# uzh-rpg/dagr

Hardware: AMD Instinct MI355X
Metric: events_per_sec (higher is better)
Workload: dtype f32; 1 GPU; dagr-s + --use_image --img_net resnet50, 640x480 synthetic S-uniform, B=8 windows/step x 100000 events (50 ms each), r=7, K=16, events->graph->GNN(+image fusion)->decoded head outputs->confidence mask + NMS (device); image_branch=in-line, engines=3

## Files before the change

dagr_amd/_lib.py:

```python
import ctypes
import os

_HERE = os.path.dirname(os.path.abspath(__file__))
LIB_PATH = os.path.join(_HERE, "lib", "libdagr_hip.so")

c_void_p = ctypes.c_void_p
c_i32 = ctypes.c_int32
c_i64 = ctypes.c_int64
c_size_t = ctypes.c_size_t
c_float = ctypes.c_float


class PoolDesc(ctypes.Structure):
    _fields_ = [("batch_size", c_i32), ("channels", c_i32), ("gx", c_i32), ("gy", c_i32), ("vx", c_float),
                ("vy", c_float), ("inv_w", c_float), ("inv_h", c_float), ("two_max", c_float), ("r00", c_float),
                ("r02", c_float), ("r11", c_float), ("r12", c_float), ("rx", c_i32), ("ry", c_i32), ("aggr", c_i32),
                ("append_pos", c_i32), ("keep_order", c_i32)]


class GraphDesc(ctypes.Structure):
    _fields_ = [("width", c_i32), ("height", c_i32), ("batch_size", c_i32), ("max_neighbors", c_i32),
                ("queue_size", c_i32), ("radius", c_i32), ("delta_t_us", c_i32), ("time_window", c_i32),
                ("max_events", c_i64)]


class HeadScale(ctypes.Structure):
    _fields_ = [("n_ptr", c_void_p), ("n_max", c_i32), ("pred", c_void_p), ("ld", c_i32), ("pos", c_void_p),
                ("batch", c_void_p), ("vx", c_float), ("vy", c_float), ("stride", c_float), ("Hc", c_i32), ("Wc", c_i32),
                ("cnn", c_void_p * 3), ("cnn_stride", (c_i32 * 4) * 3), ("dense", c_void_p)]


class ConvJob(ctypes.Structure):
    _fields_ = [("n_nodes_ptr", c_void_p), ("n_nodes_max", c_i32), ("rowptr", c_void_p), ("col", c_void_p),
                ("code", c_void_p), ("x", c_void_p), ("ldx", c_i32), ("cin", c_i32), ("xskip", c_void_p),
                ("ldskip", c_i32), ("cskip", c_i32), ("rx", c_i32), ("ry", c_i32), ("den_x", c_float), ("den_y", c_float),
                ("Wq", c_void_p), ("bias", c_void_p), ("C", c_void_p), ("ldc", c_i32), ("N", c_i32), ("relu", c_i32)]


class L0Inputs(ctypes.Structure):
    _fields_ = [("feat", c_void_p), ("pos_nodes", c_void_p), ("batch_nodes", c_void_p), ("x0", c_void_p), ("ldx0", c_i32),
                ("col_feat", c_i32), ("col_pos", c_i32)]


class AsyncUpdateArgs(ctypes.Structure):
    _fields_ = [("gdesc", ctypes.POINTER(GraphDesc)), ("graph_ws", c_void_p), ("n_static", c_i64), ("first_id", c_i64),
                ("app_head", c_void_p), ("app_next", c_void_p), ("app_xytb", c_void_p), ("capacity", c_i64),
                ("pos", c_void_p), ("batch", c_void_p), ("batch_is_int64", c_i32), ("n_new", c_i64),
                ("nbr_src", c_void_p), ("nbr_code", c_void_p), ("deg", c_void_p), ("status", c_void_p),
                ("feat", c_void_p), ("pos_nodes", c_void_p), ("batch_nodes", c_void_p), ("batch_events", c_void_p),
                ("x0", c_void_p), ("ldx0", c_i32), ("col_feat", c_i32), ("col_pos", c_i32),
                ("win_x", c_i32), ("tx", c_i32), ("win_y", c_i32), ("ty", c_i32), ("rx", c_i32), ("ry", c_i32),
                ("den_x", c_float), ("den_y", c_float),
                ("cin1", c_i32), ("w1", c_void_p), ("s1", c_void_p), ("h1", c_void_p), ("ldh1", c_i32),
                ("w2", c_void_p), ("s2", c_void_p), ("hp0", c_void_p), ("ldhp0", c_i32),
                ("pdesc", ctypes.POINTER(PoolDesc)), ("pool_ws", c_void_p), ("xlo", c_void_p), ("ylo", c_void_p),
                ("x_out", c_void_p), ("ldo", c_i32), ("pos_out", c_void_p), ("batch_out", c_void_p), ("n_out", c_void_p),
                ("rowptr_out", c_void_p), ("col_out", c_void_p), ("code_out", c_void_p), ("e_out", c_void_p),
                ("e_cap", c_i32)]


SIGNATURES = {
    "dagr_last_error": (ctypes.c_char_p, []),
    "dagr_version": (ctypes.c_int, []),
    "dagr_device_count": (ctypes.c_int, []),
    "dagr_format_events": (ctypes.c_int, [c_void_p, c_void_p, c_void_p, c_i64, c_i32, c_i32, c_i32,
                                          c_void_p, c_void_p, c_void_p]),
    "dagr_fill_edges": (ctypes.c_int, [c_void_p, c_void_p, c_void_p, c_void_p, c_void_p, c_i32, c_float, c_float, c_void_p,
                                       c_i64, c_i32, c_i64, c_i32, c_i32, c_i32, c_i32, c_void_p]),
    "dagr_insert_in_queue": (ctypes.c_int, [c_void_p, c_void_p, c_void_p, c_i64, c_void_p, c_i32, c_i32, c_i32, c_i32,
                                            c_void_p]),
    "dagr_insert_in_queue_single": (ctypes.c_int, [c_void_p, c_void_p, c_void_p, c_i32, c_i32, c_i32, c_i32, c_void_p]),
    "dagr_graph_workspace_bytes": (c_size_t, [ctypes.POINTER(GraphDesc)]),
    "dagr_graph_workspace_init": (ctypes.c_int, [ctypes.POINTER(GraphDesc), c_void_p, c_size_t, c_void_p]),
    "dagr_graph_build_window": (ctypes.c_int, [ctypes.POINTER(GraphDesc), c_void_p, c_void_p, c_i32, c_void_p,
                                               c_i32, c_i64, c_void_p, c_void_p, c_void_p, c_void_p]),
    "dagr_graph_search_window": (ctypes.c_int, [ctypes.POINTER(GraphDesc), c_void_p, c_i64, c_void_p, c_void_p, c_void_p,
                                                c_void_p]),
    "dagr_graph_status": (ctypes.c_int, [ctypes.POINTER(GraphDesc), c_void_p, ctypes.POINTER(c_i64),
                                         ctypes.POINTER(c_i32), c_void_p]),
    "dagr_graph_counters": (ctypes.c_int, [ctypes.POINTER(GraphDesc), c_void_p, c_void_p, c_void_p]),
    "dagr_scan_scratch_elems": (c_size_t, [c_i64]),
    "dagr_graph_edge_index": (ctypes.c_int, [ctypes.POINTER(GraphDesc), c_void_p, c_void_p, c_void_p, c_i64, c_void_p,
                                             c_void_p, c_void_p, c_i64, c_void_p]),
    "dagr_graph_node_order": (ctypes.c_int, [ctypes.POINTER(GraphDesc), c_void_p, c_i64, c_void_p, c_void_p, c_void_p]),
    "dagr_graph_gather_inputs": (ctypes.c_int, [ctypes.POINTER(GraphDesc), c_void_p, c_void_p, c_void_p, c_i64,
                                                c_void_p, c_void_p, c_void_p, c_i32, c_i32, c_i32, c_void_p]),
    "dagr_spline_conv_l0_tiles": (ctypes.c_int, [c_i32, c_i32, c_i32, c_i32, c_i32, c_i32, c_i32, c_i32, c_i32, c_float,
                                                 c_float, c_i64, c_i32, c_void_p, c_void_p, c_void_p, c_void_p, c_i32,
                                                 c_void_p, c_i32, c_void_p, c_void_p, c_i32, c_void_p, c_i32, c_void_p,
                                                 c_void_p]),
    "dagr_graph_build_window_dev": (ctypes.c_int, [ctypes.POINTER(GraphDesc), c_void_p, c_void_p, c_i32, c_void_p,
                                                   c_i32, c_i64, c_void_p, c_void_p, c_void_p, c_void_p, c_void_p]),
    "dagr_graph_build_window_inputs": (ctypes.c_int, [ctypes.POINTER(GraphDesc), c_void_p, c_void_p, c_void_p, c_i32, c_i64,
                                                      c_void_p, c_void_p, c_void_p, c_void_p, c_void_p, c_void_p]),
    "dagr_graph_node_count_ptr": (c_void_p, [ctypes.POINTER(GraphDesc), c_void_p]),
    "dagr_graph_csr_codes": (ctypes.c_int, [ctypes.POINTER(GraphDesc), c_void_p, c_void_p, c_void_p, c_void_p, c_i64, c_i32,
                                            c_void_p, c_void_p, c_void_p, c_void_p, c_i64, c_void_p]),
    "dagr_stage_window": (ctypes.c_int, [ctypes.POINTER(GraphDesc), c_void_p, c_void_p, c_void_p, c_void_p, c_i32, c_i64,
                                         c_void_p, c_void_p, c_void_p, c_void_p, c_void_p]),
    "dagr_spiral_offsets": (ctypes.c_int, [c_i32, c_void_p, c_void_p]),
    "dagr_spline_tap_window": (ctypes.c_int, [c_i32, c_float, ctypes.POINTER(c_i32), ctypes.POINTER(c_i32)]),
    "dagr_spline_l0_table": (ctypes.c_int, [c_i32, c_i32, c_float, c_float, c_i32, c_i32, c_i32, c_i32, c_void_p,
                                            c_void_p, c_void_p]),
    "dagr_spline_conv_l0": (ctypes.c_int, [c_i32, c_i32, c_i32, c_i64, c_i32, c_i32, c_void_p, c_void_p, c_void_p,
                                           c_void_p, c_i32, c_void_p, c_i32, c_void_p, c_void_p, c_void_p, c_i32,
                                           c_void_p, c_i32, c_void_p]),
    "dagr_spline_tap_aggregate": (ctypes.c_int, [c_void_p, c_i32, c_void_p, c_void_p, c_void_p, c_void_p, c_i32,
                                                 c_i32, c_void_p, c_i32, c_i32, c_i32, c_i32, c_float, c_float,
                                                 c_void_p, c_i32, c_void_p]),
    "dagr_spline_tap_scatter_grad": (ctypes.c_int, [c_void_p, c_i32, c_void_p, c_void_p, c_void_p, c_void_p, c_i32, c_i32,
                                                    c_i32, c_i32, c_float, c_float, c_void_p, c_void_p, c_void_p, c_i32,
                                                    c_void_p]),
    "dagr_spline_tap_scatter_grad_w": (ctypes.c_int, [c_void_p, c_i32, c_void_p, c_void_p, c_void_p, c_void_p, c_i32, c_i32,
                                                      c_void_p, c_i32, c_i32, c_i32, c_i32, c_float, c_float, c_void_p,
                                                      c_void_p, c_void_p, c_i32, c_void_p]),
    "dagr_pool_workspace_bytes": (c_size_t, [ctypes.POINTER(PoolDesc)]),
    "dagr_pool_workspace_init": (ctypes.c_int, [ctypes.POINTER(PoolDesc), c_void_p, c_size_t, c_void_p]),
    "dagr_pool_l0": (ctypes.c_int, [ctypes.POINTER(PoolDesc), c_void_p, ctypes.POINTER(GraphDesc), c_void_p,
                                    c_void_p, c_void_p, c_void_p, c_i32, c_void_p, c_void_p, c_void_p, c_i32, c_i64,
                                    c_void_p, c_void_p,
                                    c_void_p, c_void_p, c_void_p, c_i32, c_i32, c_void_p, c_void_p, c_void_p,
                                    c_void_p, c_void_p, c_void_p, c_void_p, c_i32, c_void_p]),
    "dagr_pool_l0_accumulate": (ctypes.c_int, [ctypes.POINTER(PoolDesc), c_void_p, ctypes.POINTER(GraphDesc), c_void_p,
                                               c_void_p, c_void_p, c_void_p, c_i32, c_void_p, c_i64, c_void_p, c_void_p,
                                               c_void_p, c_void_p]),
    "dagr_pool_csr": (ctypes.c_int, [ctypes.POINTER(PoolDesc), c_void_p, c_void_p, c_i32, c_void_p, c_i32, c_void_p,
                                     c_void_p, c_void_p, c_void_p, c_void_p, c_void_p, c_i32, c_i32, c_void_p,
                                     c_void_p, c_void_p, c_void_p, c_void_p, c_void_p, c_void_p, c_i32, c_void_p]),
    "dagr_pool_recode": (ctypes.c_int, [c_void_p, c_i32, c_void_p, c_void_p, c_void_p, c_float, c_float, c_float, c_float,
                                        c_float, c_i32, c_i32, c_void_p, c_i32, c_void_p, c_void_p]),
    "dagr_pool_status": (ctypes.c_int, [ctypes.POINTER(PoolDesc), c_void_p, ctypes.POINTER(c_i32), c_void_p]),
    "dagr_pool_status_ptr": (c_void_p, [ctypes.POINTER(PoolDesc), c_void_p]),
    "dagr_pool_counters": (ctypes.c_int, [ctypes.POINTER(PoolDesc), c_void_p, c_void_p, c_void_p]),
    "dagr_to_dense": (ctypes.c_int, [c_void_p, c_i32, c_void_p, c_i32, c_i32, c_void_p, c_void_p, c_float, c_float,
                                     c_i32, c_i32, c_i32, c_void_p, c_void_p, c_void_p, c_void_p]),
    "dagr_pool_argmax": (ctypes.c_int, [c_void_p, c_i32, c_void_p, c_i32, c_i32, c_void_p, c_i32, c_i32, c_void_p, c_void_p]),
    "dagr_pool_grad": (ctypes.c_int, [c_void_p, c_i32, c_i32, c_i32, c_void_p, c_void_p, c_void_p, c_i32, c_void_p, c_i32,
                                      c_void_p]),
    "dagr_to_dense_grad": (ctypes.c_int, [c_i32, c_i32, c_void_p, c_void_p, c_float, c_float, c_i32, c_i32, c_i32, c_void_p,
                                          c_void_p, c_i32, c_void_p]),
    "dagr_sample_features": (ctypes.c_int, [c_void_p, c_i32, c_void_p, c_void_p, c_i32, c_void_p, c_i32, c_i32, c_i32,
                                            c_i32, c_i32, c_i32, c_void_p, c_i32, c_i32, c_void_p]),
    "dagr_nms_batched": (ctypes.c_int, [c_void_p, c_void_p, c_void_p, c_void_p, c_i32, c_i32, c_float, c_float, c_void_p,
                                        c_void_p, c_void_p, c_void_p]),
    "dagr_heads_finish": (ctypes.c_int, [ctypes.POINTER(HeadScale), ctypes.POINTER(HeadScale), c_i32, c_i32, c_void_p,
                                         c_void_p, c_void_p]),
    "dagr_heads_finish_detect": (ctypes.c_int, [ctypes.POINTER(HeadScale), ctypes.POINTER(HeadScale), c_i32, c_i32, c_void_p,
                                                c_void_p, c_float, c_float, c_float, c_void_p, c_void_p, c_void_p]),
    "dagr_decode_heads": (ctypes.c_int, [c_void_p, c_i32, c_i32, c_float, c_void_p, c_i32, c_i32, c_float, c_i32, c_i32,
                                         c_void_p, c_void_p]),
    "dagr_postprocess": (ctypes.c_int, [c_void_p, c_i32, c_i32, c_i32, c_float, c_float, c_float, c_void_p, c_void_p,
                                        c_void_p]),
    "dagr_masked_lin": (ctypes.c_int, [c_void_p, c_void_p, c_void_p, c_void_p, c_void_p, c_i32, c_i64, c_i32, c_i32, c_void_p]),
    "dagr_masked_lin_no_bias": (ctypes.c_int, [c_void_p, c_void_p, c_void_p, c_void_p, c_i32, c_i64, c_i32, c_i32, c_void_p]),
    "dagr_masked_isdiff": (ctypes.c_int, [c_void_p, c_void_p, c_void_p, c_float, c_float, c_i64, c_i32, c_void_p]),
    "dagr_masked_inplace_BN": (ctypes.c_int, [c_void_p, c_void_p, c_void_p, c_void_p, c_void_p, c_void_p, c_void_p, c_float,
                                              c_i64, c_i32, c_void_p]),
    "dagr_downsample_events": (ctypes.c_int, [c_void_p, c_void_p, c_void_p, c_i32, c_void_p, c_i32, c_i32, c_void_p,
                                              c_void_p, c_void_p]),
    "dagr_spline_conv_l0_tiles_rows": (ctypes.c_int, [c_i32, c_i32, c_i32, c_i32, c_i32, c_i32, c_i32, c_i32, c_i32, c_float,
                                                      c_float, c_i64, c_i64, c_i32, c_void_p, c_void_p, c_void_p, c_void_p,
                                                      c_i32, c_void_p, c_i32, c_void_p, c_void_p, c_i32, c_void_p, c_i32,
                                                      c_void_p, c_void_p]),
    "dagr_async_graph_append": (ctypes.c_int, [ctypes.POINTER(GraphDesc), c_void_p, c_i64, c_i64, c_void_p, c_void_p,
                                               c_void_p, c_i64, c_void_p, c_i32, c_void_p, c_i32, c_i64, c_void_p, c_void_p,
                                               c_void_p, c_void_p, c_void_p, c_void_p, c_void_p, c_void_p, c_void_p, c_i32,
                                               c_i32, c_i32, c_void_p]),
    "dagr_async_update": (ctypes.c_int, [ctypes.POINTER(AsyncUpdateArgs), c_void_p]),
    "dagr_pool_l0_stream": (ctypes.c_int, [ctypes.POINTER(PoolDesc), c_void_p, c_i32, ctypes.POINTER(GraphDesc), c_void_p,
                                           c_void_p, c_void_p, c_void_p, c_i32, c_void_p, c_void_p, c_i64, c_i64, c_i64,
                                           c_void_p, c_void_p, c_void_p, c_void_p, c_i32, c_i32, c_void_p, c_void_p,
                                           c_void_p, c_void_p, c_void_p, c_void_p, c_void_p, c_i32, c_void_p]),
    "dagr_spline_conv_fused_lds_bytes": (c_size_t, [c_i32, c_i32]),
    "dagr_spline_conv_fused_passes": (c_i32, [c_i32, c_i32]),
    "dagr_spline_conv_fused": (ctypes.c_int, [c_void_p, c_i32, c_void_p, c_void_p, c_void_p, c_void_p, c_i32, c_i32,
                                              c_void_p, c_i32, c_i32, c_i32, c_i32, c_float, c_float, c_void_p,
                                              c_void_p, c_void_p, c_i32, c_i32, c_i32, c_void_p]),
    "dagr_spline_conv_fused_pool": (ctypes.c_int, [c_void_p, c_i32, c_void_p, c_void_p, c_void_p, c_void_p, c_i32, c_i32,
                                                   c_void_p, c_i32, c_i32, c_i32, c_i32, c_float, c_float, c_void_p,
                                                   c_void_p, c_void_p, c_i32, c_i32, c_i32, ctypes.POINTER(PoolDesc),
                                                   c_void_p, c_void_p, c_void_p, c_void_p, c_void_p]),
    "dagr_spline_conv_fused_multi": (ctypes.c_int, [c_void_p, c_i32, c_void_p]),
    "dagr_spline_conv_fused_pair": (ctypes.c_int, [c_void_p, c_i32, c_void_p, c_void_p, c_void_p, c_i32, c_i32, c_i32, c_i32,
                                                   c_float, c_float, c_i32, c_i32, c_void_p, c_void_p, c_void_p, c_void_p,
                                                   c_i32, c_void_p, c_void_p, c_void_p, c_void_p, c_i32, c_void_p]),
    "dagr_gemm_epilogue_workspace_bytes": (c_size_t, []),
    "dagr_gemm_epilogue": (ctypes.c_int, [c_void_p, c_i64, c_i32, c_i64, c_void_p, c_i32, c_void_p, c_void_p, c_i64, c_i32,
                                          c_void_p, c_i64, c_void_p, c_size_t, c_void_p]),
    "dagr_add_relu": (ctypes.c_int, [c_void_p, c_void_p, c_i64, c_void_p]),
    "dagr_bias_relu": (ctypes.c_int, [c_void_p, c_void_p, c_i64, c_i32, c_void_p]),
    "dagr_bias_silu": (ctypes.c_int, [c_void_p, c_void_p, c_i64, c_i32, c_void_p]),
    "dagr_bn_relu_maxpool": (ctypes.c_int, [c_void_p, c_i32, c_i32, c_i32, c_i32, c_void_p, c_void_p, c_void_p, c_void_p]),
    "dagr_gemm_bias_act": (ctypes.c_int, [c_void_p, c_i32, c_void_p, c_i32, c_void_p, c_i32, c_void_p, c_void_p,
                                          c_i32, c_i32, c_i32, c_i32, c_void_p]),
    "dagr_async_flops": (ctypes.c_int, [c_void_p, c_i32, c_void_p, c_void_p, c_void_p, c_void_p, c_void_p, c_i32, c_void_p,
                                        c_void_p]),
    "dagr_viz_workspace_bytes": (c_size_t, [c_i32, c_i32, c_i32]),
    "dagr_viz_render": (ctypes.c_int, [c_void_p, c_i32, c_i32, c_i32, c_void_p, c_i32, c_void_p, c_void_p, c_void_p,
                                       c_void_p, c_i32, c_void_p, c_void_p, c_void_p, c_i32, c_i32, c_void_p, c_i32,
                                       c_void_p, c_void_p, c_void_p, c_size_t, c_void_p]),
    "dagr_augment_workspace_bytes": (c_size_t, [c_i64]),
    "dagr_augment_events": (ctypes.c_int, [c_void_p, c_i32, c_i32, c_i32, c_void_p, c_i32, c_void_p, c_i32, c_void_p, c_i32,
                                           c_void_p, c_i64, c_void_p, c_void_p, c_void_p, c_void_p, c_void_p, c_void_p,
                                           c_void_p, c_size_t, c_void_p]),
    "dagr_augment_status": (ctypes.c_int, [c_void_p, c_void_p]),
    "dagr_augment_frames": (ctypes.c_int, [c_void_p, c_i32, c_i32, c_i32, c_i32, c_i32, c_i32, c_void_p, c_void_p,
                                           c_void_p]),
    "dagr_augment_boxes": (ctypes.c_int, [c_void_p, c_i32, c_i32, c_i32, c_void_p, c_void_p, c_i32, c_i32, c_void_p,
                                          c_void_p]),
}

_lib = None


def lib():
    global _lib
    if _lib is None:
        if not os.path.exists(LIB_PATH):
            raise RuntimeError(
                f"dagr_amd: {LIB_PATH} not found -- build it with `make` (or __graft_entry__.build()). "
                "There is no CPU fallback for the event-graph hot path.")
        handle = ctypes.CDLL(LIB_PATH)
        for name, (res, args) in SIGNATURES.items():
            fn = getattr(handle, name)
            fn.restype = res
            fn.argtypes = args
        _lib = handle
    return _lib


def check(rc, what=""):
    if rc != 0:
        msg = lib().dagr_last_error().decode("utf-8", "replace")
        raise RuntimeError(f"libdagr_hip {what} failed (status {rc}): {msg}")


def ptr(t):
    return None if t is None else c_void_p(t.data_ptr())


def cur_stream(device=None):
    import torch
    return c_void_p(torch.cuda.current_stream(device).cuda_stream)
```

dagr_amd/csrc/pooling.hip:

```cpp
#include <climits>

#include "common.hpp"
#include "pool_common.hpp"

namespace dagr {
namespace {

constexpr int kMaxL0Channels = 512;

__device__ __forceinline__ float div_floor(float a, float b) {
    if (b == 0.0f) return a / b;
    const float mod = fmodf(a, b);
    float div = (a - mod) / b;
    if ((mod != 0.0f) && ((b < 0.0f) != (mod < 0.0f))) div -= 1.0f;
    float floordiv;
    if (div != 0.0f) {
        floordiv = floorf(div);
        if (div - floordiv > 0.5f) floordiv += 1.0f;
    } else {
        floordiv = copysignf(0.0f, a / b);
    }
    return floordiv;
}

__global__ __launch_bounds__(kBlock) void k_pool_accumulate(dagr_pool_desc d, const int32_t *__restrict__ n_ptr,
                                                           int n_max, const float *__restrict__ x, int ldx,
                                                           const float *__restrict__ pos,
                                                           const int32_t *__restrict__ batch,
                                                           const int32_t *__restrict__ rowptr,
                                                           const int32_t *__restrict__ col, PoolWs ws,
                                                           int32_t *__restrict__ cluster_raw_out) {
    const int n_nodes = n_ptr ? min(*n_ptr, n_max) : n_max;
    const int C = d.channels;
    const int64_t gid = (int64_t)blockIdx.x * kBlock + threadIdx.x;
    const int n = (int)(gid / C), ch = (int)(gid % C);
    if (n >= n_nodes) return;
    bool ok;
    const int raw = cluster_raw(pos[3 * n], pos[3 * n + 1], pos[3 * n + 2], batch[n], d, ok);
    if (!ok) {
        if (ch == 0) { atomicOr(&ws.status[0], 1); cluster_raw_out[n] = -1; }
        return;
    }
    const float v = x[(size_t)n * ldx + ch];
    if (d.aggr == 0)
        atomicMax(reinterpret_cast<int *>(ws.xacc + (size_t)raw * C + ch), enc_f(v));
    else
        atomicAdd(reinterpret_cast<unsigned long long *>(ws.xacc + (size_t)raw * C + ch),
                  (unsigned long long)(long long)llrint((double)v * kFeatScale));
    pool_merge_node(d, ws, n, raw, pos, batch, col, rowptr ? rowptr[n] : 0, rowptr ? rowptr[n + 1] : 0, ch, C, cluster_raw_out);
}

constexpr int kPoolL0Block = 1024;

template <int AGGR>
__host__ __device__ inline size_t pool_l0_lds_bytes(int VW, int C, int W, int H, bool ord = false) {
    size_t b = ((size_t)VW * C * (AGGR == 0 ? 4 : 8) + 7) / 8 * 8;
    b += (size_t)VW * (24 + 4 + 4 + 4);
    b += (kPoolL0Block / 64) * 64 * 2;
    b += ((size_t)(W + H) * 2 + 7) / 8 * 8;
    if (ord) b += (size_t)VW * 4;
    return b + 64;
}

template <int AGGR, int VEC, bool ORD>
__device__ __forceinline__ void pool_l0_slots_body(dagr_pool_desc d, int W, int H, int n_cap, int VW,
                                                               const int32_t *__restrict__ n_ptr,
                                                               const int32_t *__restrict__ xlo,
                                                               const int32_t *__restrict__ ylo,
                                                               const int32_t *__restrict__ start, int row_keys,
                                                               const int2 *__restrict__ slot_it,
                                                               const int32_t *__restrict__ slot_xyb,
                                                               const float *__restrict__ x, int ldx,
                                                               const float *__restrict__ pos, PoolWs ws,
                                                               const int16_t *__restrict__ nbr_code,
                                                               const int32_t *__restrict__ nbr_src,
                                                               const int32_t *__restrict__ deg, int K, int r) {
    extern __shared__ __align__(16) unsigned char lds_raw[];
    constexpr int NW = kPoolL0Block / 64;
    const int n = min(*n_ptr, n_cap);
    const int per_block = max(64 * NW, (int)(((long long)n + gridDim.x - 1) / gridDim.x + 63) / 64 * 64);
    const int s_begin = blockIdx.x * per_block;
    if (s_begin >= n) return;
    const int s_end = min(n, s_begin + per_block);
    const int C = d.channels;
    const int lane = threadIdx.x & 63, wv = threadIdx.x >> 6;
    int *l_acc; unsigned long long *l_ps; int *l_cnt, *l_perm; unsigned *l_nbm; short *l_sv; unsigned short *l_xlut, *l_ylut;
    int *l_tmax = nullptr;
    {
        unsigned char *p = lds_raw;
        l_acc = reinterpret_cast<int *>(p); p += ((size_t)VW * C * (AGGR == 0 ? 4 : 8) + 7) / 8 * 8;
        l_ps = reinterpret_cast<unsigned long long *>(p); p += (size_t)VW * 24;
        l_cnt = reinterpret_cast<int *>(p); p += (size_t)VW * 4;
        l_perm = reinterpret_cast<int *>(p); p += (size_t)VW * 4;
        l_nbm = reinterpret_cast<unsigned *>(p); p += (size_t)VW * 4;
        l_sv = reinterpret_cast<short *>(p); p += NW * 64 * 2;
        l_xlut = reinterpret_cast<unsigned short *>(p); p += (size_t)W * 2;
        l_ylut = reinterpret_cast<unsigned short *>(p);
        if (ORD) l_tmax = reinterpret_cast<int *>(l_xlut + ((size_t)(W + H) * 2 + 7) / 8 * 4);
    }
    auto arm_window = [&]() {
        for (int i = threadIdx.x; i < VW * C; i += kPoolL0Block) {
            if (AGGR == 0) l_acc[i] = kEncMin;
            else reinterpret_cast<unsigned long long *>(l_acc)[i] = 0ull;
        }
        for (int i = threadIdx.x; i < VW; i += kPoolL0Block) {
            l_cnt[i] = 0; l_perm[i] = -1; l_nbm[i] = 0u;
            if (ORD) l_tmax[i] = kEncMin;
            l_ps[3 * i] = 0ull; l_ps[3 * i + 1] = 0ull; l_ps[3 * i + 2] = 0ull;
        }
    };
    arm_window();
    for (int c = threadIdx.x; c < d.gx; c += kPoolL0Block)
        for (int px = xlo[c]; px < min(xlo[c + 1], W); px++) l_xlut[px] = (unsigned short)c;
    for (int c = threadIdx.x; c < d.gy; c += kPoolL0Block)
        for (int py = ylo[c]; py < min(ylo[c + 1], H); py++) l_ylut[py] = (unsigned short)c;
    __syncthreads();
    const int cells = d.gx * d.gy;
    const int pair = ws_pair(ws);
    long long *w_possum = ws_possum(ws, pair);
    int32_t *w_cnt = ws_cnt(ws, pair);
    const int side = 2 * r + 1;
    const int side_magic = (65536 + side - 1) / side;
    const int PPN = C / VEC;
    const unsigned ppn_magic = PPN > 1 ? (unsigned)((0x100000000ull + (unsigned)PPN - 1) / (unsigned)PPN) : 0u;
    constexpr int kBig = 1 << 28;
    int n_slow = 0;
    const int T = ws.T;
    const int WB = VW / d.gx;
    for (int seg_begin = s_begin; seg_begin < s_end;) {
    int raw0, seg_end = s_end;
    {
        const int c0 = slot_xyb[seg_begin];
        const int q0 = (int)l_ylut[(c0 >> 12) & 4095] + d.gy * ((c0 >> 24) & 127);
        raw0 = d.gx * q0;
        const int qe = q0 + WB;
        if (qe < d.gy * d.batch_size) {
            const int be = qe / d.gy, cye = qe - be * d.gy;
            seg_end = min(s_end, max(seg_begin + 1, start[row_keys * (min(ylo[cye], H) + H * be)]));
        }
    }
    for (int cs = seg_begin + 64 * wv; cs < seg_end; cs += 64 * NW) {
        const int s = cs + lane;
        const bool live = s < seg_end;
        int c = 0, id = 0, dg = 0;
        float px = 0.f, py = 0.f, pt = 0.f;
        int4 lo4 = make_int4(0, 0, 0, 0), hi4 = lo4;
        if (live) {
            c = slot_xyb[s];
            px = pos[3 * (size_t)s]; py = pos[3 * (size_t)s + 1]; pt = pos[3 * (size_t)s + 2];
            id = slot_it[s].x;
            if (nbr_code) {
                dg = min(deg[s], K);
                if (K == 16) {
                    lo4 = *reinterpret_cast<const int4 *>(nbr_code + (size_t)s * 16);
                    hi4 = *reinterpret_cast<const int4 *>(nbr_code + (size_t)s * 16 + 8);
                }
            }
        }
        const float *xrow = x + (size_t)cs * ldx;
        const int n_live = min(64, seg_end - cs);
        constexpr int U = 4;
        float val[U][VEC];
        int who[U];
        auto request = [&](int f0) {
#pragma unroll
            for (int u = 0; u < U; u++) {
                const int f = f0 + 64 * u + lane;
                who[u] = -1;
                if (f < n_live * PPN) {
                    const int k = PPN > 1 ? (int)__umulhi((unsigned)f, ppn_magic) : f, p = f - k * PPN;
                    who[u] = (k << 16) | p;
                    if constexpr (VEC == 4) {
                        const float4 qv = *reinterpret_cast<const float4 *>(xrow + (size_t)k * ldx + 4 * p);
                        val[u][0] = qv.x; val[u][1] = qv.y; val[u][2] = qv.z; val[u][3] = qv.w;
                    } else {
                        val[u][0] = xrow[(size_t)k * ldx + p];
                    }
                }
            }
        };
        request(0);
        int vloc = -1;
        if (live) {
            const int xp = c & 4095, yp = (c >> 12) & 4095, b = (c >> 24) & 127;
            const int cx = l_xlut[xp], cy = l_ylut[yp];
            const bool leak = pt >= 1.0f;
            const int raw = cx + d.gx * (cy + d.gy * b);
            const int rel = raw - raw0;
            const bool inwin = !leak && rel >= 0 && rel < VW;
            const unsigned long long q0 = (unsigned long long)(long long)llrint((double)px * kPosScale);
            const unsigned long long q1 = (unsigned long long)(long long)llrint((double)py * kPosScale);
            const unsigned long long q2 = (unsigned long long)(long long)llrint((double)pt * kPosScale);
            if (ORD) {
                if (inwin) atomicMax(&l_tmax[rel], enc_f(pt));
                else atomicMax(&ws.tmax[leak ? raw + cells : raw], enc_f(pt));
            }
            unsigned nbm = 0, nbm_up = 0, nbm_low = 0;
            if (nbr_code) {
                int tx[4], ty[4];
#pragma unroll
                for (int k = 0; k < 4; k++) {
                    const int qx = cx - 1 + k, qy = cy - 1 + k;
                    tx[k] = (qx <= 0 ? -kBig : (qx >= d.gx ? kBig : xlo[qx])) - xp + r;
                    ty[k] = (qy <= 0 ? -kBig : (qy >= d.gy ? kBig : ylo[qy])) - yp + r;
                }
                int codes[16];
                if (K == 16) {
                    const int w8[8] = {lo4.x, lo4.y, lo4.z, lo4.w, hi4.x, hi4.y, hi4.z, hi4.w};
#pragma unroll
                    for (int j = 0; j < 8; j++) { codes[2 * j] = (short)(w8[j] & 0xffff); codes[2 * j + 1] = w8[j] >> 16; }
                } else {
#pragma unroll
                    for (int j = 0; j < 16; j++) codes[j] = j < dg ? (int)nbr_code[(size_t)s * K + j] : 0;
                }
#pragma unroll
                for (int j = 0; j < 16; j++) {
                    if (j < dg) {
                        const int code = codes[j];
                        const int ox = (code * side_magic) >> 16, oy = code - ox * side;
                        const int dcx = (ox >= tx[0]) + (ox >= tx[1]) + (ox >= tx[2]) + (ox >= tx[3]);
                        const int dcy = (oy >= ty[0]) + (oy >= ty[1]) + (oy >= ty[2]) + (oy >= ty[3]);
                        const unsigned bit = 1u << (dcy * 5 + dcx);
                        if (!leak) {
                            nbm |= bit;
                        } else {
                            const int src = nbr_src[(size_t)s * K + j];
                            if (pos[3 * (size_t)src + 2] >= 1.0f) nbm_up |= bit;
                            else nbm_low |= bit;
                        }
                    }
                }
                nbm &= ~(1u << 12);
                nbm_up &= ~(1u << 12);
            }
            if (inwin) {
                vloc = rel;
                atomicAdd(&l_cnt[rel], 1);
                atomicMax(&l_perm[rel], id);
                atomicAdd(&l_ps[3 * rel], q0);
                atomicAdd(&l_ps[3 * rel + 1], q1);
                atomicAdd(&l_ps[3 * rel + 2], q2);
                if (nbm) atomicOr(&l_nbm[rel], nbm);
            } else {
                const int rl = leak ? raw + cells : raw;
                n_slow++;
                for (int ch = 0; ch < C; ch++) {
                    const float v = x[(size_t)s * ldx + ch];
                    if (AGGR == 0)
                        atomicMax(reinterpret_cast<int *>(ws.xacc + (size_t)rl * C + ch), enc_f(v));
                    else
                        atomicAdd(reinterpret_cast<unsigned long long *>(ws.xacc + (size_t)rl * C + ch),
                                  (unsigned long long)(long long)llrint((double)v * kFeatScale));
                }
                ws.occupied[rl] = 1;
                atomicAdd(&w_cnt[rl], 1);
                atomicMax(&ws.perm[rl], id);
                atomicAdd(reinterpret_cast<unsigned long long *>(w_possum + (size_t)rl * 3 + 0), q0);
                atomicAdd(reinterpret_cast<unsigned long long *>(w_possum + (size_t)rl * 3 + 1), q1);
                atomicAdd(reinterpret_cast<unsigned long long *>(w_possum + (size_t)rl * 3 + 2), q2);
                if (!leak) {
                    if (nbm) atomicOr(&ws.nbmask[rl], (unsigned long long)nbm);
                } else if (nbm_up | nbm_low) {
                    atomicOr(&ws.nbmask[rl], ((unsigned long long)nbm_low << 32) | nbm_up);
                }
            }
        }
        l_sv[wv * 64 + lane] = (short)vloc;
        __builtin_amdgcn_wave_barrier();
        for (int f0 = 0; f0 < n_live * PPN; f0 += 64 * U) {
            float cur[U][VEC];
            int tgt[U];
#pragma unroll
            for (int u = 0; u < U; u++) {
                tgt[u] = -1;
                if (who[u] >= 0) {
                    const int v = l_sv[wv * 64 + (who[u] >> 16)];
                    if (v >= 0) tgt[u] = v * C + (who[u] & 0xffff) * VEC;
                }
#pragma unroll
                for (int j = 0; j < VEC; j++) cur[u][j] = val[u][j];
            }
            if (f0 + 64 * U < n_live * PPN) request(f0 + 64 * U);
#pragma unroll
            for (int u = 0; u < U; u++) {
                if (tgt[u] >= 0) {
#pragma unroll
                    for (int j = 0; j < VEC; j++) {
                        if (AGGR == 0)
                            atomicMax(&l_acc[tgt[u] + j], enc_f(cur[u][j]));
                        else
                            atomicAdd(reinterpret_cast<unsigned long long *>(l_acc) + tgt[u] + j,
                                      (unsigned long long)(long long)llrint((double)cur[u][j] * kFeatScale));
                    }
                }
            }
        }
        __builtin_amdgcn_wave_barrier();
    }
    __syncthreads();
    for (int i = threadIdx.x; i < VW * C; i += kPoolL0Block) {
        const int v = i / C;
        if (l_cnt[v] > 0 && raw0 + v < T) {
            const size_t o = (size_t)(raw0 + v) * C + (i - v * C);
            if (AGGR == 0) atomicMax(reinterpret_cast<int *>(ws.xacc + o), l_acc[i]);
            else atomicAdd(reinterpret_cast<unsigned long long *>(ws.xacc + o),
                           reinterpret_cast<unsigned long long *>(l_acc)[i]);
        }
    }
    for (int v = threadIdx.x; v < VW; v += kPoolL0Block) {
        const int cn = l_cnt[v];
        if (cn > 0 && raw0 + v < T) {
            const int raw = raw0 + v;
            ws.occupied[raw] = 1;
            atomicAdd(&w_cnt[raw], cn);
            atomicMax(&ws.perm[raw], l_perm[v]);
            atomicAdd(reinterpret_cast<unsigned long long *>(w_possum + (size_t)raw * 3 + 0), l_ps[3 * v]);
            atomicAdd(reinterpret_cast<unsigned long long *>(w_possum + (size_t)raw * 3 + 1), l_ps[3 * v + 1]);
            atomicAdd(reinterpret_cast<unsigned long long *>(w_possum + (size_t)raw * 3 + 2), l_ps[3 * v + 2]);
            if (l_nbm[v]) atomicOr(&ws.nbmask[raw], (unsigned long long)l_nbm[v]);
            if (ORD) atomicMax(&ws.tmax[raw], l_tmax[v]);
        }
    }
    seg_begin = seg_end;
    if (seg_begin < s_end) {
        __syncthreads();
        arm_window();
        __syncthreads();
    }
    }
    {
        int tot = n_slow;
#pragma unroll
        for (int off = 1; off < 64; off <<= 1) tot += __shfl_xor(tot, off, 64);
        if (lane == 0 && tot) atomicAdd(&ws.status[5], tot);
    }
}

#define DAGR_POOL_L0_SLOTS_KERNEL(NAME, ORD)                                                                          \
    template <int AGGR, int VEC>                                                                                       \
    __global__ __launch_bounds__(kPoolL0Block) void NAME(                                                              \
        dagr_pool_desc d, int W, int H, int n_cap, int VW, const int32_t *__restrict__ n_ptr,                          \
        const int32_t *__restrict__ xlo, const int32_t *__restrict__ ylo, const int32_t *__restrict__ start, int row_keys, \
        const int2 *__restrict__ slot_it, const int32_t *__restrict__ slot_xyb, const float *__restrict__ x, int ldx,   \
        const float *__restrict__ pos, PoolWs ws, const int16_t *__restrict__ nbr_code,                                \
        const int32_t *__restrict__ nbr_src, const int32_t *__restrict__ deg, int K, int r) {                          \
        pool_l0_slots_body<AGGR, VEC, ORD>(d, W, H, n_cap, VW, n_ptr, xlo, ylo, start, row_keys, slot_it, slot_xyb, x, \
                                           ldx, pos, ws, nbr_code, nbr_src, deg, K, r);                                \
    }
DAGR_POOL_L0_SLOTS_KERNEL(k_pool_l0_slots, false)
DAGR_POOL_L0_SLOTS_KERNEL(k_pool_l0_slots_ord, true)
#undef DAGR_POOL_L0_SLOTS_KERNEL

__global__ __launch_bounds__(kBlock) void k_pool_l0_event_cluster(dagr_pool_desc d, int N,
                                                                 const float *__restrict__ pos,
                                                                 const int32_t *__restrict__ batch32,
                                                                 const int64_t *__restrict__ batch64,
                                                                 int32_t *__restrict__ cluster_raw_out,
                                                                 int32_t *__restrict__ status) {
    const int n = blockIdx.x * kBlock + threadIdx.x;
    if (n >= N) return;
    bool ok;
    const int b = batch32 ? batch32[n] : (int)batch64[n];
    const int raw = cluster_raw(pos[3 * (size_t)n], pos[3 * (size_t)n + 1], pos[3 * (size_t)n + 2], b, d, ok);
    if (!ok) atomicOr(status, 1);
    cluster_raw_out[n] = ok ? raw : -1;
}

__device__ __forceinline__ void cluster_pos(const PoolWs &ws, int pair, int raw, int cnt, const dagr_pool_desc &d,
                                            float (&p)[3]) {
    const long long *ps = ws_possum(ws, pair) + (size_t)raw * 3;
#pragma unroll
    for (int k = 0; k < 3; k++) p[k] = (float)(((double)ps[k] / kPosScale) / (double)cnt);
    p[0] = div_floor(p[0] + 1e-5f, d.inv_w) * d.inv_w;
    p[1] = div_floor(p[1] + 1e-5f, d.inv_h) * d.inv_h;
}

__global__ __launch_bounds__(kBlock) void k_pool_finalize(dagr_pool_desc d, PoolWs ws,
                                                         const int32_t *__restrict__ batch32,
                                                         const int64_t *__restrict__ batch64,
                                                         float *__restrict__ x_out, int ldo, int xoff,
                                                         float *__restrict__ pos_out, int32_t *__restrict__ batch_out,
                                                         int32_t *__restrict__ n_out) {
    const int T = d.gx * d.gy * (d.batch_size + 1);
    const int C = d.channels;
    const int64_t gid = (int64_t)blockIdx.x * kBlock + threadIdx.x;
    const int raw = (int)(gid / C), ch = (int)(gid % C);
    if (raw >= T) return;
    if (gid == 0) *n_out = ws.newid[T];
    const int pair = ws_pair(ws);
    const int cnt = ws_cnt(ws, pair)[raw];
    long long *acc = ws.xacc + (size_t)raw * C + ch;
    if (cnt > 0) {
        const int c = ws.newid[raw];
        float v;
        if (d.aggr == 0) v = dec_f((int)(*acc));
        else v = (float)(((double)(*acc) / kFeatScale) / (double)cnt);
        x_out[(size_t)c * ldo + xoff + ch] = v;
        if (ch == 0) {
            float p[3];
            cluster_pos(ws, pair, raw, cnt, d, p);
            pos_out[3 * c] = p[0]; pos_out[3 * c + 1] = p[1]; pos_out[3 * c + 2] = p[2];
            const int pm = ws.perm[raw];
            batch_out[c] = batch32 ? batch32[pm] : (int)batch64[pm];
            if (d.append_pos) {
                x_out[(size_t)c * ldo + xoff + C] = p[0];
                x_out[(size_t)c * ldo + xoff + C + 1] = p[1];
            }
        }
    }
    *acc = 0ll;
    if (d.aggr == 0) *reinterpret_cast<int *>(acc) = kEncMin;
    if (ch == 0) {
        long long *ps = ws_possum(ws, pair) + (size_t)raw * 3;
        ps[0] = 0; ps[1] = 0; ps[2] = 0;
    }
}

__global__ void k_fill_enc_min(long long *p, size_t n) {
    const size_t i = (size_t)blockIdx.x * blockDim.x + threadIdx.x;
    if (i < n) { p[i] = 0ll; *reinterpret_cast<int *>(p + i) = kEncMin; }
}

__global__ __launch_bounds__(kBlock) void k_pool_rearm(int T, PoolWs ws) {
    const int raw = blockIdx.x * kBlock + threadIdx.x;
    if (raw >= T) return;
    ws_cnt(ws, ws_pair(ws))[raw] = 0;
    ws.perm[raw] = -1;
    ws.nbmask[raw] = 0ull;
    if (ws.tmax) ws.tmax[raw] = kEncMin;
}

__global__ __launch_bounds__(kBlock) void k_coarse_edges_ell(int N, int K, const int32_t *__restrict__ nbr_src,
                                                            const int32_t *__restrict__ deg,
                                                            const int32_t *__restrict__ cluster_raw_in,
                                                            const int32_t *__restrict__ newid, int32_t *rows,
                                                            int32_t *status, const int32_t *__restrict__ tmax) {
    __shared__ unsigned long long seen[256];
    seen[threadIdx.x] = ~0ull;
    __syncthreads();
    const int lane = threadIdx.x & 63;
    const int per_iter = kBlock / K;
    const int G = gridDim.x, nx = (G % 8 == 0) ? 8 : 1;
    const int xcd = blockIdx.x % nx, lb = blockIdx.x / nx, bpx = G / nx;
    const int chunk = (N + nx - 1) / nx;
    const int per_block = (chunk + bpx - 1) / bpx;
    const int n_begin = xcd * chunk + lb * per_block;
    const int n_end = min(min(N, (xcd + 1) * chunk), n_begin + per_block);
    const int sub = threadIdx.x / K, j = threadIdx.x % K;
    for (int n0 = n_begin; n0 < n_end; n0 += per_iter) {
        const int n = n0 + sub;
        int rd = -1, rs = -1;
        if (sub < per_iter && n < n_end && j < deg[n]) {
            rd = cluster_raw_in[n];
            rs = cluster_raw_in[nbr_src[(size_t)n * K + j]];
        }
        bool has = (rd != rs) && rd >= 0 && rs >= 0;
        if (tmax && has && !(tmax[rs] < tmax[rd])) has = false;
        const unsigned long long key = ((unsigned long long)(unsigned)rd << 32) | (unsigned)rs;
        const unsigned h = (unsigned)((key * 0x9E3779B97F4A7C15ull) >> 56);
        if (has && seen[h] == key) has = false;
        unsigned long long pending = __ballot(has);
        while (pending) {
            const int leader = __ffsll((long long)pending) - 1;
            const int prd = __shfl(rd, leader, 64), prs = __shfl(rs, leader, 64);
            if (lane == leader) {
                row_insert(rows, newid[prd], newid[prs], status);
                seen[h] = key;
            }
            const bool same = has && rd == prd && rs == prs;
            pending &= ~__ballot(same);
            if (same) has = false;
        }
    }
}

__global__ __launch_bounds__(kBlock) void k_rows_sort(int T, const int32_t *__restrict__ newid, int32_t *rows,
                                                     int32_t *__restrict__ rowcnt) {
    const int lane = threadIdx.x & 63;
    const int c = blockIdx.x * (kBlock / 64) + (threadIdx.x >> 6);
    if (c > T) return;
    const int nc = newid[T];
    if (c >= nc) {
        if (lane == 0 && c <= T) rowcnt[c] = 0;
        return;
    }
    int32_t *row = rows + (size_t)c * kRowSlots;
    const int v = row[lane];
    const bool valid = v >= 0;
    int rank = 0;
    for (int k = 0; k < 64; k++) {
        const int o = __shfl(v, k, 64);
        rank += (o >= 0 && o < v) ? 1 : 0;
    }
    const int count = __popcll(__ballot(valid));
    row[lane] = -1;
    __builtin_amdgcn_wave_barrier();
    if (valid) row[rank] = v;
    if (lane == 0) rowcnt[c] = count;
}

__global__ __launch_bounds__(kBlock) void k_rows_emit(dagr_pool_desc d, int T, const int32_t *__restrict__ newid,
                                                     int32_t *rows, const int32_t *__restrict__ rowptr,
                                                     const float *__restrict__ pos_out, int32_t *__restrict__ col,
                                                     int32_t *__restrict__ code, int32_t *__restrict__ e_out,
// ... 222 lines not shown
        for (int k = 0; k < 64; k++) {
            const int o = __shfl(v, k, 64);
            rank += (o >= 0 && o < v) ? 1 : 0;
        }
    }
    if (v < 0) return;
    const int o = rowptr_out[c] + rank;
    if (o >= e_cap) { atomicOr(ws.status, 4); return; }
    float q[3];
    cluster_pos(ws, pair, v, ws_cnt(ws, pair)[v], d, q);
    const float ax = (q[0] - p[0]) / d.two_max + 0.5f;
    const float ay = (q[1] - p[1]) / d.two_max + 0.5f;
    const int ix = (int)((ax * d.r00 + d.r02) + 1e-3f);
    const int iy = (int)((ay * d.r11 + d.r12) + 1e-3f);
    if (ix < 0 || ix > 2 * d.rx || iy < 0 || iy > 2 * d.ry) atomicOr(ws.status, 8);
    col[o] = ws.newid[v];
    code[o] = (ix & 0xffff) | (iy << 16);
}

template <bool KEEP>
__global__ __launch_bounds__(kBlock) void k_pool_order_masks(dagr_pool_desc d, PoolWs ws) {
    const int raw = blockIdx.x * kBlock + threadIdx.x;
    if (raw >= ws.T) return;
    const unsigned long long m = ws.nbmask[raw];
    unsigned long long f = 0ull;
    if (m) {
        if (!KEEP) ws.nbmask[raw] = 0ull;
        const int td = ws.tmax[raw];
        const int cells = d.gx * d.gy;
        for (unsigned long long r = m; r; r &= r - 1ull) {
            const int bit = __ffsll((long long)r) - 1;
            const int k = bit & 31;
            const int v = raw + (k % 5 - 2) + d.gx * (k / 5 - 2) - (bit >= 32 ? cells : 0);
            if (v >= 0 && v < ws.T && ws.tmax[v] < td) f |= 1ull << bit;
        }
    }
    ws.nbmask_f[raw] = f;
}

__global__ __launch_bounds__(kBlock) void k_pool_order_rows(PoolWs ws) {
    const int lane = threadIdx.x & 63;
    const int raw = blockIdx.x * (kBlock / 64) + (threadIdx.x >> 6);
    if (raw >= ws.T || ws.rowcnt[raw] == 0) return;
    int32_t *row = ws.rows + (size_t)raw * kRowSlots;
    const int v = row[lane];
    bool keep = v >= 0;
    if (keep && !(ws.tmax[v] < ws.tmax[raw])) {
        row[lane] = -1;
        keep = false;
    }
    const int n = __popcll(__ballot(keep));
    if (lane == 0) ws.rowcnt[raw] = n;
}

__global__ __launch_bounds__(kBlock) void k_pool_l0_add_rows(dagr_pool_desc d, int W, int H, int first_row, int n_rows,
                                                            const int32_t *__restrict__ xlo,
                                                            const int32_t *__restrict__ ylo,
                                                            const float *__restrict__ x, int ldx,
                                                            const float *__restrict__ pos,
                                                            const int32_t *__restrict__ batch_events, PoolWs ws,
                                                            const int16_t *__restrict__ nbr_code,
                                                            const int32_t *__restrict__ nbr_src,
                                                            const int32_t *__restrict__ deg, int K, int r) {
    const int l = threadIdx.x & 15;
    const int i = (blockIdx.x * kBlock + threadIdx.x) >> 4;
    if (i >= n_rows) return;
    const int s = first_row + i;
    const float px = pos[3 * (size_t)s], py = pos[3 * (size_t)s + 1], pt = pos[3 * (size_t)s + 2];
    const int b = batch_events[s];
    bool ok;
    const int raw = cluster_raw(px, py, pt, b, d, ok);
    if (!ok) {
        if (l == 0) atomicOr(&ws.status[0], 1);
        return;
    }
    const bool leak = pt >= 1.0f;
    const int cells = d.gx * d.gy;
    const int C = d.channels;
    const int pair = ws_pair(ws);
    for (int ch = l; ch < C; ch += 16) {
        const float v = x[(size_t)s * ldx + ch];
        if (d.aggr == 0) atomicMax(reinterpret_cast<int *>(ws.xacc + (size_t)raw * C + ch), enc_f(v));
        else atomicAdd(reinterpret_cast<unsigned long long *>(ws.xacc + (size_t)raw * C + ch),
                       (unsigned long long)(long long)llrint((double)v * kFeatScale));
    }
    if (l == 0) {
        ws.occupied[raw] = 1;
        atomicAdd(&ws_cnt(ws, pair)[raw], 1);
        atomicMax(&ws.perm[raw], ((b + 1) << 26) | s);
        if (ws.tmax) atomicMax(&ws.tmax[raw], enc_f(pt));
        atomicAdd(reinterpret_cast<unsigned long long *>(ws_possum(ws, pair) + (size_t)raw * 3 + 0),
                  (unsigned long long)(long long)llrint((double)px * kPosScale));
        atomicAdd(reinterpret_cast<unsigned long long *>(ws_possum(ws, pair) + (size_t)raw * 3 + 1),
                  (unsigned long long)(long long)llrint((double)py * kPosScale));
        atomicAdd(reinterpret_cast<unsigned long long *>(ws_possum(ws, pair) + (size_t)raw * 3 + 2),
                  (unsigned long long)(long long)llrint((double)pt * kPosScale));
    }
    if (nbr_code && l < deg[s]) {
        const int xpix = (int)((float)W * px + 1e-3f), ypix = (int)((float)H * py + 1e-3f);
        const int cx = (raw % cells) % d.gx, cy = (raw % cells) / d.gx;
        const int side = 2 * r + 1;
        const int code = nbr_code[(size_t)s * K + l];
        const int ox = code / side, oy = code - ox * side;
        const int xs = xpix + ox - r, ys = ypix + oy - r;
        int dcx = 0, dcy = 0;
#pragma unroll
        for (int q = 0; q < 4; q++) {
            const int qx = cx - 1 + q, qy = cy - 1 + q;
            const int bxq = qx <= 0 ? INT_MIN : (qx >= d.gx ? INT_MAX : xlo[qx]);
            const int byq = qy <= 0 ? INT_MIN : (qy >= d.gy ? INT_MAX : ylo[qy]);
            dcx += xs >= bxq;
            dcy += ys >= byq;
        }
        const int bit = dcy * 5 + dcx;
        if (!leak) {
            if (bit != 12) atomicOr(&ws.nbmask[raw], 1ull << bit);
        } else {
            const int src = nbr_src[(size_t)s * K + l];
            if (pos[3 * (size_t)src + 2] >= 1.0f) {
                if (bit != 12) atomicOr(&ws.nbmask[raw], 1ull << bit);
            } else {
                atomicOr(&ws.nbmask[raw], 1ull << (32 + bit));
            }
        }
    }
}

__global__ __launch_bounds__(kBlock) void k_pool_perm_keys(int T, const int32_t *__restrict__ batch_events, PoolWs ws) {
    const int raw = blockIdx.x * kBlock + threadIdx.x;
    if (raw >= T) return;
    const int pm = ws.perm[raw];
    if (pm >= 0) ws.perm[raw] = ((batch_events[pm] + 1) << 26) | pm;
}

}
}

using namespace dagr;

namespace {
int validate_pool(const dagr_pool_desc *d) {
    DAGR_CHECK_ARG(d != nullptr, "desc is NULL");
    DAGR_CHECK_ARG(d->gx > 0 && d->gy > 0 && d->batch_size > 0 && d->channels > 0, "bad sizes");
    DAGR_CHECK_ARG((int64_t)d->gx * d->gy * (d->batch_size + 1) < (1 << 22), "voxel table too large");
    DAGR_CHECK_ARG(d->keep_order == 0 || d->keep_order == 1, "keep_order must be 0 or 1");
    DAGR_CHECK_ARG(d->aggr == 0 || d->aggr == 1, "aggr must be 0 (max) or 1 (mean)");
    DAGR_CHECK_ARG(d->vx > 0 && d->vy > 0 && d->two_max > 0, "bad voxel size / cartesian max");
    return DAGR_OK;
}

int launch_pool_l0_slots(const dagr_pool_desc *desc, const dagr_graph_desc *gdesc, void *graph_ws, const int32_t *xlo,
                         const int32_t *ylo, const float *x, int ldx, const float *pos, const PoolWs &ws,
                         const int16_t *nbr_code, const int32_t *nbr_src, const int32_t *deg, int64_t n_cap,
                         hipStream_t stream) {
    PixelIndex ix;
    graph_ws_index(gdesc, graph_ws, &ix);
    const int32_t *start = ix.start; const int2 *slot_it = ix.slot_it;
    const int32_t *slot_xyb = ix.slot_xyb;
    const int32_t *n_ptr = ix.n_nodes;
    const int row_keys = ix.W;
    const int C = desc->channels, W = gdesc->width, H = gdesc->height, K = gdesc->max_neighbors;
    const bool vec4 = C % 4 == 0 && ldx % 4 == 0 && ((uintptr_t)x & 15) == 0;
    const bool ord = desc->keep_order != 0;
    const size_t per_slot = (size_t)C * (desc->aggr == 0 ? 4 : 8) + 36 + (ord ? 4 : 0);
    const size_t budget = (size_t)60 * 1024 - (size_t)(W + H) * 2 - 2048 - 1024;
    int VW = (int)std::min<size_t>(1024, budget / per_slot);
    VW = std::max(VW, desc->gx) / 2 * 2 + 2;
    const size_t lds = desc->aggr == 0 ? pool_l0_lds_bytes<0>(VW, C, W, H, ord) : pool_l0_lds_bytes<1>(VW, C, W, H, ord);
    DAGR_CHECK_ARG(lds <= 64 * 1024, "level-0 pooling: one voxel row of accumulators does not fit the LDS window");
    DAGR_CHECK_ARG(desc->gx < 65536 && desc->gy < 65536 && VW < 32768, "voxel grid too large for the level-0 pooling kernel");
    const int gmult = C > 32 ? 2 : 1;
    const unsigned grid = (unsigned)std::max<int64_t>(1, std::min<int64_t>((int64_t)gmult * device_cu_count(),
                                                                          ceil_div(n_cap, kPoolL0Block)));
#define DAGR_POOL_L0_LAUNCH(AG, VEC)                                                                                  \
    if (ord) DAGR_POOL_L0_LAUNCH_ORD(k_pool_l0_slots_ord, AG, VEC); else DAGR_POOL_L0_LAUNCH_ORD(k_pool_l0_slots, AG, VEC)
#define DAGR_POOL_L0_LAUNCH_ORD(KERNEL, AG, VEC)                                                                      \
    KERNEL<AG, VEC><<<grid, kPoolL0Block, lds, stream>>>(*desc, W, H, (int)n_cap, VW, n_ptr, xlo, ylo, start, row_keys, slot_it, \
                                                                   slot_xyb, x, ldx, pos, ws, nbr_code, nbr_src, deg, K, \
                                                                   gdesc->radius)
    if (desc->aggr == 0) { if (vec4) DAGR_POOL_L0_LAUNCH(0, 4); else DAGR_POOL_L0_LAUNCH(0, 1); }
    else                 { if (vec4) DAGR_POOL_L0_LAUNCH(1, 4); else DAGR_POOL_L0_LAUNCH(1, 1); }
#undef DAGR_POOL_L0_LAUNCH
#undef DAGR_POOL_L0_LAUNCH_ORD
    DAGR_CHECK_LAUNCH();
    return DAGR_OK;
}
template <bool KEEP>
int pool_order_masks(const dagr_pool_desc *d, const PoolWs &ws, PoolWs *view, hipStream_t stream) {
    *view = ws;
    if (!d->keep_order) return DAGR_OK;
    k_pool_order_masks<KEEP><<<(unsigned)ceil_div(ws.T, kBlock), kBlock, 0, stream>>>(*d, ws);
    DAGR_CHECK_LAUNCH();
    view->nbmask = ws.nbmask_f;
    return DAGR_OK;
}
}

extern "C" {

size_t dagr_pool_workspace_bytes(const dagr_pool_desc *desc) {
    if (validate_pool(desc) != DAGR_OK) return 0;
    return pool_carve(*desc, nullptr, nullptr);
}

int dagr_pool_workspace_init(const dagr_pool_desc *desc, void *workspace, size_t bytes, void *stream_) {
    int rc = validate_pool(desc);
    if (rc != DAGR_OK) return rc;
    DAGR_CHECK_ARG(workspace, "workspace is NULL");
    PoolWs ws;
    if (pool_carve(*desc, (char *)workspace, &ws) > bytes) {
        set_error("dagr_pool_workspace_init: workspace too small");
        return DAGR_ERR_WORKSPACE;
    }
    hipStream_t stream = (hipStream_t)stream_;
    const int64_t T = (int64_t)desc->gx * desc->gy * (desc->batch_size + 1);
    DAGR_CHECK_HIP(hipMemsetAsync(ws.occupied, 0, (T + 32) * 4, stream));
    DAGR_CHECK_HIP(hipMemsetAsync(ws.newid, 0, (T + 32) * 4, stream));
    DAGR_CHECK_HIP(hipMemsetAsync(ws.possum, 0, 2 * T * 3 * 8, stream));
    DAGR_CHECK_HIP(hipMemsetAsync(ws.cnt, 0, 2 * T * 4, stream));
    DAGR_CHECK_HIP(hipMemsetAsync(ws.perm, 0xff, T * 4, stream));
    DAGR_CHECK_HIP(hipMemsetAsync(ws.rows, 0xff, T * (size_t)kRowSlots * 4, stream));
    DAGR_CHECK_HIP(hipMemsetAsync(ws.rowcnt, 0, (T + 32) * 4, stream));
    DAGR_CHECK_HIP(hipMemsetAsync(ws.status, 0, 32, stream));
    DAGR_CHECK_HIP(hipMemsetAsync(ws.tile_state, 0, ((T + 1 + kPoolScanTile - 1) / kPoolScanTile + 8) * 8, stream));
    DAGR_CHECK_HIP(hipMemsetAsync(ws.nbmask, 0, (T + 9) * 8, stream));
    if (desc->keep_order) {
        DAGR_CHECK_HIP(hipMemsetD32Async((hipDeviceptr_t)ws.tmax, kEncMin, (size_t)T + 32, stream));
        DAGR_CHECK_HIP(hipMemsetAsync(ws.nbmask_f, 0, (T + 9) * 8, stream));
    }
    {
        const size_t n = T * (size_t)desc->channels;
        if (desc->aggr == 0) {
            k_fill_enc_min<<<(unsigned)ceil_div(n, 256), 256, 0, stream>>>(ws.xacc, n);
            DAGR_CHECK_LAUNCH();
        } else {
            DAGR_CHECK_HIP(hipMemsetAsync(ws.xacc, 0, n * 8, stream));
        }
    }
    return DAGR_OK;
}


#define DAGR_POOL_SCAN(MASKS, KEEP, WS)                                                                               \
    k_pool_scan_chained<MASKS, KEEP><<<(unsigned)ceil_div(T + 1, kPoolScanTile), kBlock, 0, stream>>>(WS, n_out, rowptr_out, e_out)


static int pool_tail(const dagr_pool_desc *d, PoolWs &ws, const int32_t *batch32, const int64_t *batch64,
                     float *x_out, int ldo, int xoff, float *pos_out, int32_t *batch_out, int32_t *n_out,
                     int32_t *rowptr_out, int32_t *col_out, int32_t *code_out, int32_t *e_out, int e_cap,
                     hipStream_t stream) {
    const int T = d->gx * d->gy * (d->batch_size + 1);
    const int wpb = kBlock / 64;
    k_rows_sort<<<(unsigned)ceil_div(T + 1, wpb), kBlock, 0, stream>>>(T, ws.newid, ws.rows, ws.rowcnt);
    DAGR_CHECK_LAUNCH();
    DAGR_CHECK_HIP(exclusive_scan_i32(ws.rowcnt, rowptr_out, T + 1, ws.scan_tmp, false, stream));
    k_rows_emit<<<(unsigned)ceil_div(T, wpb), kBlock, 0, stream>>>(*d, T, ws.newid, ws.rows, rowptr_out, pos_out,
                                                                  col_out, code_out, e_out, e_cap, ws.status);
    DAGR_CHECK_LAUNCH();
    k_pool_rearm<<<(unsigned)ceil_div(T, kBlock), kBlock, 0, stream>>>(T, ws);
    DAGR_CHECK_LAUNCH();
    (void)batch32; (void)batch64; (void)x_out; (void)ldo; (void)xoff; (void)batch_out; (void)n_out;
    return DAGR_OK;
}

int dagr_pool_l0(const dagr_pool_desc *desc, void *pool_ws, const dagr_graph_desc *gdesc, void *graph_ws,
                 const int32_t *xlo, const int32_t *ylo, const float *x, int32_t ldx, const float *pos,
                 const int32_t *batch_nodes, const void *batch, int32_t batch_is_int64, int64_t N,
                 const int32_t *nbr_src, const int16_t *nbr_code, const int32_t *deg,
                 int32_t *cluster_scratch, float *x_out, int32_t ldo, int32_t xoff, float *pos_out,
                 int32_t *batch_out, int32_t *n_out, int32_t *rowptr_out, int32_t *col_out, int32_t *code_out,
                 int32_t *e_out, int32_t e_cap, void *stream_) {
    int rc = validate_pool(desc);
    if (rc != DAGR_OK) return rc;
    DAGR_CHECK_ARG(pool_ws && gdesc && graph_ws, "NULL workspace/desc");
    DAGR_CHECK_ARG(desc->channels <= kMaxL0Channels, "too many channels for the level-0 pooling kernel");
    DAGR_CHECK_ARG(desc->batch_size == gdesc->batch_size, "batch_size mismatch");
    DAGR_CHECK_ARG(n_out && rowptr_out && e_out, "NULL output");
    hipStream_t stream = (hipStream_t)stream_;
    PoolWs ws;
    pool_carve(*desc, (char *)pool_ws, &ws);
    const int T = desc->gx * desc->gy * (desc->batch_size + 1);
    const int32_t *b32 = batch_is_int64 ? nullptr : (const int32_t *)batch;
    const int64_t *b64 = batch_is_int64 ? (const int64_t *)batch : nullptr;
    const int K = gdesc->max_neighbors;
    const int cell_w = (int)floorf(desc->vx * (float)gdesc->width), cell_h = (int)floorf(desc->vy * (float)gdesc->height);
    const bool fast_edges = nbr_code != nullptr && K <= 16 && gdesc->radius <= 2 * std::min(cell_w, cell_h) &&
                            gdesc->width <= 4096;
    if (N > 0) {
        DAGR_CHECK_ARG(xlo && ylo && x && pos && batch_nodes && batch && nbr_src && deg && cluster_scratch, "NULL input");
        rc = launch_pool_l0_slots(desc, gdesc, graph_ws, xlo, ylo, x, ldx, pos, ws, fast_edges ? nbr_code : nullptr, nbr_src,
                                  deg, N, stream);
        if (rc != DAGR_OK) return rc;
    }
    if (fast_edges) {
        PoolWs wv;
        rc = pool_order_masks<false>(desc, ws, &wv, stream);
        if (rc != DAGR_OK) return rc;
        DAGR_POOL_SCAN(true, false, wv);
        DAGR_CHECK_LAUNCH();
        k_pool_emit<true><<<(unsigned)ceil_div(T, kBlock / 64), kBlock, 0, stream>>>(
            *desc, wv, b32, b64, x_out, ldo, xoff, pos_out, batch_out, rowptr_out, col_out, code_out, e_cap);
        DAGR_CHECK_LAUNCH();
        return DAGR_OK;
    }
    DAGR_CHECK_HIP(exclusive_scan_i32(ws.occupied, ws.newid, T + 1, ws.scan_tmp, true, stream));
    k_pool_finalize<<<(unsigned)ceil_div((int64_t)T * desc->channels, kBlock), kBlock, 0, stream>>>(
        *desc, ws, b32, b64, x_out, ldo, xoff, pos_out, batch_out, n_out);
    DAGR_CHECK_LAUNCH();
    if (N > 0) {
        k_pool_l0_event_cluster<<<(unsigned)ceil_div(N, kBlock), kBlock, 0, stream>>>(
            *desc, (int)N, pos, batch_nodes, nullptr, cluster_scratch, ws.status);
        DAGR_CHECK_LAUNCH();
        DAGR_CHECK_ARG(K <= kBlock, "max_neighbors too large");
        const unsigned gE = round_grid8(std::min<int64_t>(ceil_div(N, kBlock / K), 256 * 8));
        k_coarse_edges_ell<<<gE, kBlock, 0, stream>>>((int)N, K, nbr_src, deg, cluster_scratch, ws.newid, ws.rows,
                                                      ws.status, ws.tmax);
        DAGR_CHECK_LAUNCH();
    }
    return pool_tail(desc, ws, b32, b64, x_out, ldo, xoff, pos_out, batch_out, n_out, rowptr_out, col_out, code_out,
                     e_out, e_cap, stream);
}

int dagr_pool_l0_accumulate(const dagr_pool_desc *desc, void *pool_ws, const dagr_graph_desc *gdesc, void *graph_ws,
                            const int32_t *xlo, const int32_t *ylo, const float *x, int32_t ldx, const float *pos,
                            int64_t N, const int32_t *nbr_src, const int16_t *nbr_code, const int32_t *deg,
                            void *stream_) {
    int rc = validate_pool(desc);
    if (rc != DAGR_OK) return rc;
    DAGR_CHECK_ARG(pool_ws && gdesc && graph_ws && xlo && ylo && x && pos && nbr_src && deg && N > 0, "bad arguments");
    DAGR_CHECK_ARG(desc->channels <= kMaxL0Channels && desc->batch_size == gdesc->batch_size, "bad descriptors");
    PoolWs ws;
    pool_carve(*desc, (char *)pool_ws, &ws);
    const int K = gdesc->max_neighbors;
    const int cell_w = (int)floorf(desc->vx * (float)gdesc->width), cell_h = (int)floorf(desc->vy * (float)gdesc->height);
    const bool fast_edges = nbr_code != nullptr && K <= 16 && gdesc->radius <= 2 * std::min(cell_w, cell_h) &&
                            gdesc->width <= 4096;
    return launch_pool_l0_slots(desc, gdesc, graph_ws, xlo, ylo, x, ldx, pos, ws, fast_edges ? nbr_code : nullptr, nbr_src,
                                deg, N, (hipStream_t)stream_);
}

int dagr_pool_l0_stream(const dagr_pool_desc *desc, void *pool_ws, int32_t rebuild, const dagr_graph_desc *gdesc,
                        void *graph_ws, const int32_t *xlo, const int32_t *ylo, const float *x, int32_t ldx, const float *pos,
                        const int32_t *batch_events, int64_t n_window, int64_t first_row, int64_t n_rows,
                        const int32_t *nbr_src, const int16_t *nbr_code, const int32_t *deg, float *x_out, int32_t ldo,
                        int32_t xoff, float *pos_out, int32_t *batch_out, int32_t *n_out, int32_t *rowptr_out,
                        int32_t *col_out, int32_t *code_out, int32_t *e_out, int32_t e_cap, void *stream_) {
    int rc = validate_pool(desc);
    if (rc != DAGR_OK) return rc;
    DAGR_CHECK_ARG(pool_ws && gdesc && graph_ws, "NULL workspace/desc");
    DAGR_CHECK_ARG(desc->channels <= kMaxL0Channels, "too many channels for the level-0 pooling kernel");
    DAGR_CHECK_ARG(desc->batch_size == gdesc->batch_size, "batch_size mismatch");
    DAGR_CHECK_ARG(n_out && rowptr_out && e_out && xlo && ylo && x && pos && batch_events && nbr_src && nbr_code && deg,
                   "NULL pointer");
    DAGR_CHECK_ARG(n_window >= 0 && first_row >= n_window && n_rows >= 0 && first_row + n_rows < (1 << 26) &&
                       desc->batch_size < 30, "bad row ranges");
    hipStream_t stream = (hipStream_t)stream_;
    PoolWs ws;
    pool_carve(*desc, (char *)pool_ws, &ws);
    const int T = desc->gx * desc->gy * (desc->batch_size + 1);
    const int K = gdesc->max_neighbors;
    const int cell_w = (int)floorf(desc->vx * (float)gdesc->width), cell_h = (int)floorf(desc->vy * (float)gdesc->height);
    DAGR_CHECK_ARG(K <= 16 && gdesc->radius <= 2 * std::min(cell_w, cell_h) && gdesc->width <= 4096,
                   "asynchronous pooling keeps its coarse edges as cell bitmaps: the search radius must span at most two cells");
    if (rebuild) {
        rc = dagr_pool_workspace_init(desc, pool_ws, pool_carve(*desc, nullptr, nullptr), stream_);
        if (rc != DAGR_OK) return rc;
        if (n_window > 0) {
            rc = launch_pool_l0_slots(desc, gdesc, graph_ws, xlo, ylo, x, ldx, pos, ws, nbr_code, nbr_src, deg, n_window,
                                      stream);
            if (rc != DAGR_OK) return rc;
            k_pool_perm_keys<<<(unsigned)ceil_div(T, kBlock), kBlock, 0, stream>>>(T, batch_events, ws);
            DAGR_CHECK_LAUNCH();
        }
    }
    if (n_rows > 0) {
        k_pool_l0_add_rows<<<(unsigned)ceil_div(n_rows * 16, kBlock), kBlock, 0, stream>>>(
            *desc, gdesc->width, gdesc->height, (int)first_row, (int)n_rows, xlo, ylo, x, ldx, pos, batch_events, ws, nbr_code,
            nbr_src, deg, K, gdesc->radius);
        DAGR_CHECK_LAUNCH();
    }
    PoolWs wv;
    rc = pool_order_masks<true>(desc, ws, &wv, stream);
    if (rc != DAGR_OK) return rc;
    DAGR_POOL_SCAN(true, true, wv);
    DAGR_CHECK_LAUNCH();
    k_pool_emit<true, true><<<(unsigned)ceil_div(T, kBlock / 64), kBlock, 0, stream>>>(
        *desc, wv, batch_events, nullptr, x_out, ldo, xoff, pos_out, batch_out, rowptr_out, col_out, code_out, e_cap);
    DAGR_CHECK_LAUNCH();
    return DAGR_OK;
}

int dagr_pool_csr(const dagr_pool_desc *desc, void *pool_ws, const int32_t *n_ptr, int32_t n_max, const float *x,
                  int32_t ldx, const float *pos, const int32_t *batch, const int32_t *rowptr, const int32_t *col,
                  int32_t *cluster_scratch, float *x_out, int32_t ldo, int32_t xoff, float *pos_out,
                  int32_t *batch_out, int32_t *n_out, int32_t *rowptr_out, int32_t *col_out, int32_t *code_out,
                  int32_t *e_out, int32_t e_cap, void *stream_) {
    int rc = validate_pool(desc);
    if (rc != DAGR_OK) return rc;
    DAGR_CHECK_ARG(pool_ws, "NULL workspace");
    DAGR_CHECK_ARG(n_out && rowptr_out && e_out, "NULL output");
    hipStream_t stream = (hipStream_t)stream_;
    PoolWs ws;
    pool_carve(*desc, (char *)pool_ws, &ws);
    const int T = desc->gx * desc->gy * (desc->batch_size + 1);
    if (n_max > 0) {
        DAGR_CHECK_ARG(x && pos && batch && rowptr && col && cluster_scratch, "NULL input");
        k_pool_accumulate<<<(unsigned)ceil_div((int64_t)n_max * desc->channels, kBlock), kBlock, 0, stream>>>(
            *desc, n_ptr, n_max, x, ldx, pos, batch, rowptr, col, ws, cluster_scratch);
        DAGR_CHECK_LAUNCH();
    }
    if (desc->keep_order) {
        k_pool_order_rows<<<(unsigned)ceil_div(T, kBlock / 64), kBlock, 0, stream>>>(ws);
        DAGR_CHECK_LAUNCH();
    }
    DAGR_POOL_SCAN(false, false, ws);
    DAGR_CHECK_LAUNCH();
    k_pool_emit<false><<<(unsigned)ceil_div(T, kBlock / 64), kBlock, 0, stream>>>(
        *desc, ws, batch, nullptr, x_out, ldo, xoff, pos_out, batch_out, rowptr_out, col_out, code_out, e_cap);
    DAGR_CHECK_LAUNCH();
    return DAGR_OK;
}

int dagr_pool_status(const dagr_pool_desc *desc, void *pool_ws, int32_t *flags_host, void *stream) {
    int rc = validate_pool(desc);
    if (rc != DAGR_OK) return rc;
    DAGR_CHECK_ARG(pool_ws && flags_host, "NULL pointer");
    PoolWs ws;
    pool_carve(*desc, (char *)pool_ws, &ws);
    DAGR_CHECK_HIP(hipMemcpyAsync(flags_host, ws.status, 4, hipMemcpyDeviceToHost, (hipStream_t)stream));
    DAGR_CHECK_HIP(hipStreamSynchronize((hipStream_t)stream));
    return DAGR_OK;
}

const int32_t *dagr_pool_status_ptr(const dagr_pool_desc *desc, void *pool_ws) {
    if (validate_pool(desc) != DAGR_OK || !pool_ws) return nullptr;
    PoolWs ws;
    pool_carve(*desc, (char *)pool_ws, &ws);
    return ws.status;
}

int dagr_pool_counters(const dagr_pool_desc *desc, void *pool_ws, int32_t *out8_host, void *stream) {
    int rc = validate_pool(desc);
    if (rc != DAGR_OK) return rc;
    DAGR_CHECK_ARG(pool_ws && out8_host, "NULL pointer");
    PoolWs ws;
    pool_carve(*desc, (char *)pool_ws, &ws);
    DAGR_CHECK_HIP(hipMemcpyAsync(out8_host, ws.status, 32, hipMemcpyDeviceToHost, (hipStream_t)stream));
    DAGR_CHECK_HIP(hipStreamSynchronize((hipStream_t)stream));
    return DAGR_OK;
}

int dagr_pool_recode(const int32_t *n_ptr, int32_t n_max, const int32_t *rowptr, const int32_t *col, const float *pos,
                     float two_max, float r00, float r02, float r11, float r12, int32_t rx, int32_t ry,
                     int32_t *code_out, int32_t e_cap, int32_t *status, void *stream) {
    DAGR_CHECK_ARG(n_max >= 0 && e_cap >= 0, "bad sizes");
    if (n_max == 0) return DAGR_OK;
    DAGR_CHECK_ARG(n_ptr && rowptr && col && pos && code_out && status, "NULL pointer");
    DAGR_CHECK_ARG(two_max > 0 && rx >= 0 && ry >= 0, "bad domain");
    k_recode<<<(unsigned)ceil_div(n_max, kBlock / 64), kBlock, 0, (hipStream_t)stream>>>(
        n_ptr, n_max, rowptr, col, pos, two_max, r00, r02, r11, r12, rx, ry, code_out, e_cap, status);
    DAGR_CHECK_LAUNCH();
    return DAGR_OK;
}

}
```

dagr_amd/csrc/sample.hip:

```cpp
#include "common.hpp"

namespace dagr {
namespace {

template <typename BatchT, int V, bool ALIGNED>
__global__ __launch_bounds__(kBlock) void k_sample_features(const int32_t *__restrict__ n_ptr, int n_max,
                                                           const float *__restrict__ pos,
                                                           const BatchT *__restrict__ batch,
                                                           const float *__restrict__ feat, int B, int h, int w,
                                                           int C, float fW, float fH, float fWm1, float fHm1,
                                                           float fBm1, float *__restrict__ out, int ldo, int coff) {
    const int n_nodes = n_ptr ? min(*n_ptr, n_max) : n_max;
    const int CV = C / V;
    const int64_t gid = (int64_t)blockIdx.x * kBlock + threadIdx.x;
    const int n = (int)(gid / CV), c = (int)(gid % CV) * V;
    if (n >= n_nodes) return;
    float gx = pos[3 * (size_t)n] * fW;
    float gy = pos[3 * (size_t)n + 1] * fH;
    float gb = (float)batch[n];
    gx = (2.0f * gx) / fWm1 - 1.0f;
    gy = (2.0f * gy) / fHm1 - 1.0f;
    gb = (2.0f * gb) / fBm1 - 1.0f;
    const float ix = ((gx + 1.0f) / 2.0f) * (float)(w - 1);
    const float iy = ((gy + 1.0f) / 2.0f) * (float)(h - 1);
    const float iz = ((gb + 1.0f) / 2.0f) * (float)(B - 1);
    const float x0f = floorf(ix), y0f = floorf(iy), z0f = floorf(iz);
    const int x0 = (int)x0f, y0 = (int)y0f, z0 = (int)z0f;
    const int x1 = x0 + 1, y1 = y0 + 1, z1 = z0 + 1;
    const float wx0 = (x0f + 1.0f) - ix, wx1 = ix - x0f;
    const float wy0 = (y0f + 1.0f) - iy, wy1 = iy - y0f;
    const float wz0 = (z0f + 1.0f) - iz, wz1 = iz - z0f;
    float acc[V];
#pragma unroll
    for (int v = 0; v < V; v++) acc[v] = 0.0f;
    auto tap = [&](int z, int y, int x, float wgt) {
        if (wgt == 0.0f || z < 0 || z >= B || y < 0 || y >= h || x < 0 || x >= w) return;
        const float *src = feat + (((size_t)z * h + y) * w + x) * C + c;
        if (V == 4 && ALIGNED) {
            const float4 f = *reinterpret_cast<const float4 *>(src);
            acc[0] += f.x * wgt; acc[1 % V] += f.y * wgt; acc[2 % V] += f.z * wgt; acc[3 % V] += f.w * wgt;
        } else {
#pragma unroll
            for (int v = 0; v < V; v++) acc[v] += src[v] * wgt;
        }
    };
    tap(z0, y0, x0, (wx0 * wy0) * wz0);
    tap(z0, y0, x1, (wx1 * wy0) * wz0);
    tap(z0, y1, x0, (wx0 * wy1) * wz0);
    tap(z0, y1, x1, (wx1 * wy1) * wz0);
    tap(z1, y0, x0, (wx0 * wy0) * wz1);
    tap(z1, y0, x1, (wx1 * wy0) * wz1);
    tap(z1, y1, x0, (wx0 * wy1) * wz1);
    tap(z1, y1, x1, (wx1 * wy1) * wz1);
    float *dst = out + (size_t)n * ldo + coff + c;
    if (V == 4 && ALIGNED) {
        *reinterpret_cast<float4 *>(dst) = make_float4(acc[0], acc[1 % V], acc[2 % V], acc[3 % V]);
    } else {
#pragma unroll
        for (int v = 0; v < V; v++) dst[v] = acc[v];
    }
}

}
}

using namespace dagr;

extern "C" int dagr_sample_features(const int32_t *n_ptr, int32_t n_max, const float *pos, const void *batch,
                                    int32_t batch_is_int64, const float *feat_nhwc, int32_t B, int32_t h, int32_t w,
                                    int32_t C, int32_t width, int32_t height, float *out, int32_t ldo, int32_t coff,
                                    void *stream_) {
    DAGR_CHECK_ARG(n_max >= 0 && B >= 1 && h >= 1 && w >= 1 && C >= 1 && width > 1 && height > 1, "bad sizes");
    if (n_max == 0) return DAGR_OK;
    DAGR_CHECK_ARG(pos && batch && feat_nhwc && out, "NULL pointer");
    hipStream_t stream = (hipStream_t)stream_;
    const float fBm1 = (float)((B > 1 ? B : 2) - 1);
    const bool four = (C % 4 == 0) && ((uintptr_t)feat_nhwc % 16 == 0);
    const bool aligned = four && (ldo % 4 == 0) && (coff % 4 == 0) && ((uintptr_t)out % 16 == 0);
    const unsigned grid = (unsigned)ceil_div((int64_t)n_max * (four ? C / 4 : C), kBlock);
#define DAGR_SAMPLE(BT, V, A)                                                                                           \
    k_sample_features<BT, V, A><<<grid, kBlock, 0, stream>>>(n_ptr, n_max, pos, (const BT *)batch, feat_nhwc, B, h, w, C, \
                                                             (float)width, (float)height, (float)(width - 1),          \
                                                             (float)(height - 1), fBm1, out, ldo, coff)
#define DAGR_SAMPLE_BT(BT)                                 \
    do {                                                   \
        if (aligned) DAGR_SAMPLE(BT, 4, true);             \
        else if (four) DAGR_SAMPLE(BT, 4, false);          \
        else DAGR_SAMPLE(BT, 1, false);                    \
    } while (0)
    if (batch_is_int64) DAGR_SAMPLE_BT(int64_t);
    else DAGR_SAMPLE_BT(int32_t);
#undef DAGR_SAMPLE_BT
#undef DAGR_SAMPLE
    DAGR_CHECK_LAUNCH();
    return DAGR_OK;
}
```

dagr_amd/engine.py:

```python
import contextlib
import ctypes
import gc
import types

import numpy as np
import torch

from . import _lib
from .graph.ev_graph import WindowGraphBuilder

FUSED_PASSES_MAX_NODES = 1600


def _f32(v):
    return float(torch.as_tensor(v, dtype=torch.float32))


def _same_domain(a, b):
    return (a["rx"], a["ry"], a["den_x"], a["den_y"]) == (b["rx"], b["ry"], b["den_x"], b["den_y"]) \
        and torch.equal(a["remap"], b["remap"])


def _bn_affine(bn):
    m = bn.module
# ... 137 lines not shown
    if y.is_cuda and y.dtype == torch.float32 and z.dtype == torch.float32 and y.shape == z.shape \
            and y.stride() == z.stride() and y.data_ptr() % 16 == 0 and z.data_ptr() % 16 == 0 \
            and (y.is_contiguous() or y.is_contiguous(memory_format=torch.channels_last)):
        _lib.check(_lib.lib().dagr_add_relu(_lib.ptr(y), _lib.ptr(z), y.numel(), _lib.cur_stream(y.device)), "add_relu")
        return y
    return torch.relu_(y.add_(z))


def _bias_relu_(y, bias):
    C = y.shape[1]
    if y.is_cuda and y.dtype == torch.float32 and C % 4 == 0 and y.is_contiguous(memory_format=torch.channels_last) \
            and y.data_ptr() % 16 == 0 and bias.data_ptr() % 16 == 0:
        _lib.check(_lib.lib().dagr_bias_relu(_lib.ptr(y), _lib.ptr(bias), y.numel(), C, _lib.cur_stream(y.device)),
                   "bias_relu")
        return y
    return torch.relu_(y.add_(bias.view(1, -1, 1, 1)))


def _baseconv_forward(m, x):
    y = m.conv(x)
    b = m._bias
    C = y.shape[1]
    if y.is_cuda and y.dtype == torch.float32 and C % 4 == 0 and y.is_contiguous(memory_format=torch.channels_last) \
            and y.data_ptr() % 16 == 0 and b.data_ptr() % 16 == 0:
        _lib.check(_lib.lib().dagr_bias_silu(_lib.ptr(y), _lib.ptr(b), y.numel(), C, _lib.cur_stream(y.device)),
                   "bias_silu")
        return y
    return torch.nn.functional.silu(y.add_(b.view(1, -1, 1, 1)), inplace=True)


def _conv_bias_relu(blk, name, x):
    conv = getattr(blk, name)
    b = getattr(blk, "_" + name + "_bias", None)
    out = conv(x)
    if b is not None:
        return _bias_relu_(out, b)
    if getattr(conv, "relu", False):
        return out
    return blk.relu(out)


def _bottleneck_forward(blk, x):
    identity = x if blk.downsample is None else blk.downsample(x)
    out = _conv_bias_relu(blk, "conv1", x)
    out = _conv_bias_relu(blk, "conv2", out)
    if isinstance(blk.conv3, _Conv1x1Gemm):
        return blk.conv3(out, residual=identity)
    return _add_relu_(blk.conv3(out), identity)


def _resnet_features_forward(net, x, emit=None):
    emit = emit or (lambda name, t: None)
    c1 = net.conv1(x)
    emit("conv1", c1)
    mp = net.maxpool
    ok = (c1.is_cuda and c1.dtype == torch.float32 and c1.is_contiguous(memory_format=torch.channels_last)
          and c1.shape[1] % 4 == 0 and mp.kernel_size == 3 and mp.stride == 2 and mp.padding == 1
          and mp.dilation == 1 and not mp.ceil_mode)
    if ok:
        B, C, H, W = c1.shape
        scale, shift = net._stem_affine
        y = torch.empty((B, C, (H - 1) // 2 + 1, (W - 1) // 2 + 1), dtype=c1.dtype, device=c1.device,
                        memory_format=torch.channels_last)
        _lib.check(_lib.lib().dagr_bn_relu_maxpool(_lib.ptr(c1), B, H, W, C, _lib.ptr(scale), _lib.ptr(shift), _lib.ptr(y),
                                                   _lib.cur_stream(c1.device)), "bn_relu_maxpool")
    else:
        y = net.maxpool(net.relu(net.bn1(c1)))
    l1 = net.layer1(y)
    emit("layer1", l1)
    l2 = net.layer2(l1)
    emit("layer2", l2)
    l3 = net.layer3(l2)
    emit("layer3", l3)
    l4 = net.layer4(l3)
    emit("layer4", l4)
    return dict(conv1=c1, layer1=l1, layer2=l2, layer3=l3, layer4=l4)


def _basicblock_forward(blk, x):
    identity = x if blk.downsample is None else blk.downsample(x)
    out = _conv_bias_relu(blk, "conv1", x)
    return _add_relu_(blk.conv2(out), identity)


class _Level:

    def __init__(self, T, cin, cout, device, cf_next=0):
        self.T = T
        self.e_cap = T * 64
        i32 = dict(dtype=torch.int32, device=device)
        f32 = dict(dtype=torch.float32, device=device)
        self.x = torch.zeros((T, (cin + 3) // 4 * 4), **f32)
        self.pos = torch.zeros((T, 3), **f32)
        self.batch = torch.zeros((T,), **i32)
        self.rowptr = torch.zeros((T + 2,), **i32)
        self.col = torch.zeros((self.e_cap,), **i32)
        self.code = torch.zeros((self.e_cap,), **i32)
        self.counts = torch.zeros((2,), **i32)
        self.cluster = torch.zeros((T,), **i32)
        self.h1 = torch.zeros((T, cout), **f32)
        self.hp = torch.zeros((T, cout + cf_next), **f32)
        self.cout = cout


class WindowEngine:
    def __init__(self, model, max_events=1 << 17, device="cuda"):
        self.model = model
        self.device = torch.device(device)
        args = model.args
        bb, head = model.backbone, model.head
        self.args = args
        self.B = int(args.batch_size)
        self.W, self.H = int(model.width), int(model.height)
        self.time_window = int(getattr(args, "time_window_us", 1000000))
        self.num_classes = bb.num_classes
        self.num_scales = int(args.num_scales)
        self.use_image = bool(args.use_image)
        self.no_events = bool(getattr(args, "no_events", False))
        self.feat_ch = list(bb.net.feature_channels) if self.use_image else [0] * 5
        if self.use_image:
            bb.net.to(memory_format=torch.channels_last)
            head.cnn_head.to(memory_format=torch.channels_last)
        if bb.conv_block1.conv_block1.conv.lut_domain is None:
            model.cache_luts(width=self.W, height=self.H, radius=args.radius)
            model._engine = self
        self.L = _lib.lib()
        if self.L.dagr_device_count() < 1:
            raise RuntimeError("dagr_amd: no HIP device visible; the event-graph path has no CPU fallback")
        self._keep = []
        self._cnn_out = None
        self._img_stream = None
        self._feat_ready = None
        self._post_key = None
        self._det = self._n_keep = None
        self._wg_post = self._graph_post = (None, None)
        self._post_fresh = False
        self._cnn_ready = None
        self._net_f = self._cnn_f = None
        self._tail_jobs = None
        self._inputs_gathered = False
        self.fast_coarse_edges = True
        self._pool_accumulated = [False] * 4
        self.set_low_latency(True)
        self._head_stream = self._head_join = self._graph = self._graph_out = None
        self._graph_warm = 0
        self._wg = self._wg_out = None
        self._wg_warm = 0
        self._dev_mode = False
        self.in_image = None
        self._async_on = False
        self._app = None
        self._n_rows = 0
        self._N = 0
        self._prepare(bb, head)
        self.max_events = 0
        self._alloc_events(int(max_events))

    def _prepare(self, bb, head):
        dev = self.device
        L = self.L
        stream = _lib.cur_stream(dev)
        layers = [bb.conv_block1, bb.layer2, bb.layer3, bb.layer4, bb.layer5]
        pools = [bb.pool1, bb.pool2, bb.pool3, bb.pool4]
        self.dom = [layer.conv_block1.conv.lut_domain for layer in layers]
        d0 = self.dom[0]
        if d0["rx"] != d0["ry"]:
            raise NotImplementedError("level 0 expects a square search radius (ev_tgn.py:29 derives it from the width)")
        win = []
        for r, den in ((d0["rx"], d0["den_x"]), (d0["ry"], d0["den_y"])):
            lo, cnt = ctypes.c_int32(0), ctypes.c_int32(0)
            _lib.check(L.dagr_spline_tap_window(r, den, ctypes.byref(lo), ctypes.byref(cnt)), "tap_window")
            if cnt.value <= 3:
                win += [min(lo.value, 2), 3]
            else:
                win += [0, 5]
        self.win0 = tuple(win)
        self.ntaps0 = win[1] * win[3]
        ntp = (self.ntaps0 + 3) // 4 * 4
        self.ncodes0 = (2 * d0["rx"] + 1) * (2 * d0["ry"] + 1)
        self.tab0 = torch.zeros((self.ncodes0, ntp), dtype=torch.float32, device=dev)
        bad = torch.zeros((1,), dtype=torch.int32, device=dev)
        _lib.check(L.dagr_spline_l0_table(d0["rx"], d0["ry"], d0["den_x"], d0["den_y"], win[0], win[1], win[2], win[3],
                                          _lib.ptr(self.tab0), _lib.ptr(bad), stream), "l0_table")
        if int(bad.item()) != 0:
            raise RuntimeError("level-0 offset table: an offset needs a kernel tap outside the chosen window")
        l0 = layers[0]
        c0 = 1 + self.feat_ch[0] + 2
        self.l0_tiles = ((win[1], win[3]) in ((3, 3), (3, 5), (5, 3)) and int(self.args.max_neighbors) == 16
                         and self.feat_ch[0] in (0, 16))
        if self.l0_tiles:
            nf = self.feat_ch[0]
            self.x0_cols = list(range(1, 1 + nf)) + [0, 1 + nf, 2 + nf]
            self.x0_ld = (c0 + 3) // 4 * 4
            self.x0_feat_col, self.x0_img_col, self.x0_pos_col = nf, 0, nf + 1
        else:
            self.x0_cols = list(range(c0))
            self.x0_ld = c0
            self.x0_feat_col, self.x0_img_col, self.x0_pos_col = 0, 1, c0 - 2
        self.l0_conv1 = _pack_l0(l0.conv_block1.conv, l0.conv_block1.norm, self.win0, device=dev, cols_in=self.x0_cols)
        self.l0_conv2 = _pack_l0(l0.conv_block2.conv, l0.conv_block2.norm, self.win0,
                                 skip=(l0.conv_block2.lin, l0.conv_block2.norm_skip), device=dev,
                                 cols_skip=self.x0_cols)
        self.packs = []
        for layer in layers[1:]:
            c1 = _pack_generic([layer.conv_block1.conv], [layer.conv_block1.norm], device=dev)
            c2 = _pack_generic([layer.conv_block2.conv], [layer.conv_block2.norm],
                               skip=(layer.conv_block2.lin, layer.conv_block2.norm_skip), device=dev)
            self.packs.append((c1, c2))
        self.pool_desc, self.pool_ws, self.levels = [], [], []
        B = self.B
        chans = [l.out_channel for l in layers]
        fch = self.feat_ch
        for k, pool in enumerate(pools):
            vs = pool.voxel_size.detach().float().cpu()
            end = torch.Tensor([0.9999999, 0.9999999])
            g = ((end - 0) / vs[:2]).to(torch.int64) + 1
            nd = self.dom[k + 1]
            remap = nd["remap"]
            desc = _lib.PoolDesc(batch_size=B, channels=chans[k] + fch[k + 1], gx=int(g[0]), gy=int(g[1]), vx=float(vs[0]),
                                 vy=float(vs[1]), inv_w=float(pool.wh_inv[0, 0]), inv_h=float(pool.wh_inv[0, 1]),
                                 two_max=_f32(2 * pool.transform.max), r00=float(remap[0, 0]),
                                 r02=float(remap[0, 2]), r11=float(remap[1, 1]), r12=float(remap[1, 2]),
                                 rx=nd["rx"], ry=nd["ry"], aggr=0 if pool.aggr == "max" else 1, append_pos=1,
                                 keep_order=1 if getattr(pool, "keep_temporal_ordering", False) else 0)
            nbytes = L.dagr_pool_workspace_bytes(ctypes.byref(desc))
            if nbytes == 0:
                raise RuntimeError("libdagr_hip: " + L.dagr_last_error().decode())
            ws = torch.empty(nbytes, dtype=torch.uint8, device=dev)
            _lib.check(L.dagr_pool_workspace_init(ctypes.byref(desc), _lib.ptr(ws), nbytes, stream), "pool_ws_init")
            self.pool_desc.append(desc)
            self.pool_ws.append(ws)
            T = int(g[0]) * int(g[1]) * (B + 1)
            self.levels.append(_Level(T, chans[k] + fch[k + 1] + 2, chans[k + 1], dev,
                                      cf_next=fch[k + 2] if k + 2 < 5 else 0))
        vs = pools[0].voxel_size.detach().float().cpu()
        d = self.pool_desc[0]
        cellx = ((torch.arange(self.W).float() / self.W) / vs[0]).to(torch.int64)
        celly = ((torch.arange(self.H).float() / self.H) / vs[1]).to(torch.int64)
        self.xlo = torch.searchsorted(cellx, torch.arange(d.gx + 1)).to(torch.int32).to(dev)
        self.ylo = torch.searchsorted(celly, torch.arange(d.gy + 1)).to(torch.int32).to(dev)
        self.head_packs, self.head_dom = [], []
        first_level = 5 - self.num_scales
        self.head_levels = list(range(first_level, 5))
        for s in range(1, self.num_scales + 1):
            g = lambda n: getattr(head, n + str(s))
            stem = _pack_generic([g("stem").conv], [g("stem").norm], device=dev)
            cr = _pack_generic([g("cls_conv").conv, g("reg_conv").conv], [g("cls_conv").norm, g("reg_conv").norm],
                               device=dev)
            cls = _pack_generic([g("cls_pred")], [None], relu=False, device=dev)
            ro = _pack_generic([g("reg_pred"), g("obj_pred")], [None, None], relu=False, device=dev)
            self.head_packs.append((stem, cr, cls, ro))
            hd = g("stem").conv.lut_domain
            for n in ("cls_conv", "reg_conv"):
                assert _same_domain(getattr(head, n + str(s)).conv.lut_domain, hd)
            for n in ("cls_pred", "reg_pred", "obj_pred"):
                assert _same_domain(getattr(head, n + str(s)).lut_domain, hd)
            self.head_dom.append(hd)
        self.n_reg = head.stem1.conv.out_channels
        osz = bb.get_output_sizes()[-self.num_scales:]
        self.out_sizes = osz
        self.strides = list(bb.strides)
        self.head_vox = [pools[2].voxel_size[:2].detach().float().cpu(), pools[3].voxel_size[:2].detach().float().cpu()][-self.num_scales:]
        lda_max = 0
        for k, (c1, c2) in enumerate(self.packs):
            lda_max = max(lda_max, self.levels[k].T * (max(c1.K, c2.K) + 3))
        for i, lvl in enumerate(self.head_levels):
            for p in self.head_packs[i]:
                lda_max = max(lda_max, self.levels[lvl - 1].T * (p.K + 3))
        self.A = torch.zeros((lda_max,), dtype=torch.float32, device=dev)
        lda2 = max([self.levels[self.head_levels[0] - 1].T * (p.K + 3) for p in self.head_packs[0]])
        self.A2 = torch.zeros((lda2 if self.num_scales > 1 else 1,), dtype=torch.float32, device=dev)
        self.head_buf = []
        for i, lvl in enumerate(self.head_levels):
            T = self.levels[lvl - 1].T
            Hc, Wc = self.out_sizes[i]
            self.head_buf.append(dict(
                stem=torch.zeros((T, self.n_reg), dtype=torch.float32, device=dev),
                cr=torch.zeros((T, 2 * self.n_reg), dtype=torch.float32, device=dev),
                pred=torch.zeros((T, 5 + self.num_classes), dtype=torch.float32, device=dev),
                dense=torch.zeros((self.B, 5 + self.num_classes, Hc, Wc), dtype=torch.float32, device=dev)))
        self.status = torch.zeros((4,), dtype=torch.int32, device=dev)
        self.head_code = []
        for i, lvl in enumerate(self.head_levels):
            same = _same_domain(self.head_dom[i], self.dom[lvl])
            self.head_code.append(None if same else torch.zeros_like(self.levels[lvl - 1].code))
        grids, strides = [], []
        for (hs, ws_), stride in zip(self.out_sizes, self.strides):
            yv, xv = torch.meshgrid(torch.arange(hs), torch.arange(ws_), indexing="ij")
            grid = torch.stack((xv, yv), 2).view(1, -1, 2)
            grids.append(grid)
            strides.append(torch.full((1, grid.shape[1], 1), stride))
        self.grid_cache = torch.cat(grids, dim=1).float().to(dev)
        self.stride_cache = torch.cat(strides, dim=1).float().to(dev)

    def set_low_latency(self, on):
        self.overlap_heads = self.tail_graph = bool(on)
        self.window_graph = bool(on)
        return self

    def _alloc_events(self, n):
        if n <= self.max_events:
            return
        dev = self.device
        n = max(n, 1024)
        self.max_events = n
        bb = self.model.backbone
        tgn = bb.events_to_graph
        self.graph = tgn.window_builder(self.W, self.H, self.time_window, self.B, dev, max_events=n)
        K = self.graph.K
        self.nbr_src = torch.zeros((n, K), dtype=torch.int32, device=dev)
        self.nbr_code = torch.zeros((n, K), dtype=torch.int16, device=dev)
        self.deg = torch.zeros((n,), dtype=torch.int32, device=dev)
        self.h1 = torch.zeros((n, 16), dtype=torch.float32, device=dev)
        self.hp0 = torch.zeros((n, 16 + self.feat_ch[1]), dtype=torch.float32, device=dev)
        self.x0buf = torch.zeros((n, self.x0_ld), dtype=torch.float32, device=dev)
        self.cluster0 = torch.zeros((n,), dtype=torch.int32, device=dev)
        self.pos_n = torch.zeros((n, 3), dtype=torch.float32, device=dev)
        self.batch_n = torch.zeros((n,), dtype=torch.int32, device=dev)
        self.in_pos = torch.zeros((n, 3), dtype=torch.float32, device=dev)
        self.in_feat = torch.zeros((n,), dtype=torch.float32, device=dev)
        self.in_batch = torch.zeros((n,), dtype=torch.int32, device=dev)
        self.n_dev = torch.zeros((1,), dtype=torch.int32, device=dev)
        self._wg = self._wg_out = None
        self._wg_warm = 0
        self.rows_cap = n
        self._async_on = False
        self._app = None

    _ROW_ARRAYS = ("nbr_src", "nbr_code", "deg", "h1", "hp0", "x0buf", "cluster0", "pos_n", "batch_n")

    def _grow_rows(self, rows):
        if rows <= self.rows_cap:
            return
        cap = max(rows, self.rows_cap + self.rows_cap // 2)
        for name in self._ROW_ARRAYS:
            old = getattr(self, name)
            new = torch.zeros((cap,) + tuple(old.shape[1:]), dtype=old.dtype, device=old.device)
            new[:old.shape[0]] = old
            setattr(self, name, new)
        if self._app is not None:
            for name in ("next", "xytb", "batch_ev"):
                old = self._app[name]
                new = torch.zeros((cap,) + tuple(old.shape[1:]), dtype=old.dtype, device=old.device)
                new[:old.shape[0]] = old
                self._app[name] = new
        self.rows_cap = cap

    def can_append(self):
        if not self.l0_tiles or self.no_events or self._N <= 0 or self.B >= 30:
            return False
        d, g = self.pool_desc[0], self.graph.params
        cell_w, cell_h = int(np.floor(np.float32(d.vx) * np.float32(g["width"]))), int(np.floor(np.float32(d.vy) * np.float32(g["height"])))
        return g["max_neighbors"] <= 16 and g["radius"] <= 2 * min(cell_w, cell_h) and g["width"] <= 4096

    def async_begin(self):
        L, P = self.L, _lib.ptr
        dev = self.device
        n0 = self._N
        if n0 == 0:
            raise RuntimeError("asynchronous update without a window: call forward_raw (reset=True) first")
        self._grow_rows(n0 + max(4096, n0 // 4))
        npix = self.B * self.H * self.W
        if self._app is None or self._app["head"].shape[0] != npix:
            nbytes = L.dagr_pool_workspace_bytes(ctypes.byref(self.pool_desc[0]))
            self._app = dict(head=torch.empty((npix,), dtype=torch.int32, device=dev),
                             next=torch.zeros((self.rows_cap,), dtype=torch.int32, device=dev),
                             xytb=torch.zeros((self.rows_cap, 4), dtype=torch.int32, device=dev),
                             batch_ev=torch.zeros((self.rows_cap,), dtype=torch.int32, device=dev),
                             status=torch.zeros((4,), dtype=torch.int32, device=dev),
                             pool_ws=torch.empty(nbytes, dtype=torch.uint8, device=dev))
        a = self._app
        for name in ("next", "xytb", "batch_ev"):
            if a[name].shape[0] < self.rows_cap:
                a[name] = torch.zeros((self.rows_cap,) + tuple(a[name].shape[1:]), dtype=a[name].dtype, device=dev)
        a.pop("args", None)
        a["head"].fill_(-1)
        a["status"].zero_()
        a["batch_ev"][:n0] = self._batch.to(torch.int32)
        self._n_rows = n0
        self._async_on = True
        self._pool1_stream(rebuild=True, first=n0, n=0)

    def _pool1_stream(self, rebuild, first, n):
        L, P = self.L, _lib.ptr
        g, a, l1, d = self.graph, self._app, self.levels[0], self.pool_desc[0]
        _lib.check(L.dagr_pool_l0_stream(ctypes.byref(d), P(a["pool_ws"]), 1 if rebuild else 0, ctypes.byref(g.desc),
                                         P(g.workspace), P(self.xlo), P(self.ylo), P(self.hp0), self.hp0.shape[1],
                                         P(self.pos_n), P(a["batch_ev"]), self._N, first, n, P(self.nbr_src),
                                         P(self.nbr_code), P(self.deg), P(l1.x), l1.x.shape[1], 0, P(l1.pos), P(l1.batch),
                                         P(l1.counts), P(l1.rowptr), P(l1.col), P(l1.code),
                                         ctypes.c_void_p(l1.counts.data_ptr() + 4), l1.e_cap,
                                         _lib.cur_stream(self.device)), "pool_l0_stream")

    def _conv_l0_rows(self, pack, first, n, x, ldx, xskip, ldskip, out, ldo):
        L, P = self.L, _lib.ptr
        cin, cskip, w, s = pack
        d0 = self.dom[0]
        wx, tx, wy, ty = self.win0
        cm = 16 if cin >= 16 else 0
        _lib.check(L.dagr_spline_conv_l0_tiles_rows(cm, cin - cm, cskip, wx, tx, wy, ty, d0["rx"], d0["ry"], d0["den_x"],
                                                    d0["den_y"], first, n, self.graph.K, P(self.nbr_src), P(self.nbr_code),
                                                    P(self.deg), x, ldx, xskip, ldskip, P(w), P(s), 1, out, ldo, None,
                                                    _lib.cur_stream(self.device)), "conv_l0_tiles_rows")

    def _async_call(self, a, first, n, pos, feat, batch, stream):
        P = lambda t: None if t is None else t.data_ptr()
        u = a.get("args")
        g, l1, d0 = self.graph, self.levels[0], self.dom[0]
        if u is None or a.get("args_rows_cap") != self.rows_cap:
            u = _lib.AsyncUpdateArgs()
            u.gdesc, u.graph_ws = ctypes.pointer(g.desc), P(g.workspace)
            u.app_head, u.app_next, u.app_xytb = P(a["head"]), P(a["next"]), P(a["xytb"])
            u.capacity = a["next"].shape[0]
            u.nbr_src, u.nbr_code, u.deg, u.status = P(self.nbr_src), P(self.nbr_code), P(self.deg), P(a["status"])
            u.pos_nodes, u.batch_nodes, u.batch_events = P(self.pos_n), P(self.batch_n), P(a["batch_ev"])
            u.x0, u.ldx0, u.col_feat, u.col_pos = P(self.x0buf), self.x0_ld, self.x0_feat_col, self.x0_pos_col
            u.win_x, u.tx, u.win_y, u.ty = self.win0
            u.rx, u.ry, u.den_x, u.den_y = d0["rx"], d0["ry"], d0["den_x"], d0["den_y"]
            cin1, _, w1, s1 = self.l0_conv1
            _, _, w2, s2 = self.l0_conv2
            u.cin1, u.w1, u.s1, u.h1, u.ldh1 = cin1, P(w1), P(s1), P(self.h1), 16
            u.w2, u.s2, u.hp0, u.ldhp0 = P(w2), P(s2), P(self.hp0), self.hp0.shape[1]
            u.pdesc, u.pool_ws, u.xlo, u.ylo = ctypes.pointer(self.pool_desc[0]), P(a["pool_ws"]), P(self.xlo), P(self.ylo)
            u.x_out, u.ldo, u.pos_out, u.batch_out = P(l1.x), l1.x.shape[1], P(l1.pos), P(l1.batch)
            u.n_out, u.rowptr_out, u.col_out, u.code_out = P(l1.counts), P(l1.rowptr), P(l1.col), P(l1.code)
            u.e_out, u.e_cap = l1.counts.data_ptr() + 4, l1.e_cap
            a["args"], a["args_rows_cap"] = u, self.rows_cap
        u.n_static, u.first_id, u.n_new = self._N, first, n
        u.pos, u.feat, u.batch = P(pos), P(feat), P(batch)
        u.batch_is_int64 = 1 if (batch is not None and batch.dtype == torch.int64) else 0
        _lib.check(self.L.dagr_async_update(ctypes.byref(u), stream), "async_update")

    def forward_append(self, pos, feat, batch, static_out=False):
        if not self.l0_tiles:
            raise NotImplementedError("asynchronous updates run on the tiled level-0 conv (16 neighbours, 3x3/3x5 tap window)")
        L, P = self.L, _lib.ptr
        if not self._async_on:
            self.async_begin()
        n = int(pos.shape[0])
        a = self._app
        first = self._n_rows
        stream = _lib.cur_stream(self.device)
        if n:
            self._grow_rows(first + n)
            a = self._app
            pos = pos.float().contiguous()
            feat = feat.float().reshape(-1).contiguous()
            batch = batch.contiguous()
        if not self.use_image:
            self._async_call(a, first, n, pos if n else None, feat if n else None, batch if n else None, stream)
            self._n_rows = first + n
        else:
            if n:
                b64 = 1 if batch.dtype == torch.int64 else 0
                g = self.graph
                _lib.check(L.dagr_async_graph_append(ctypes.byref(g.desc), P(g.workspace), self._N, first, P(a["head"]),
                                                     P(a["next"]), P(a["xytb"]), a["next"].shape[0], P(pos), 0, P(batch), b64,
                                                     n, P(self.nbr_src), P(self.nbr_code), P(self.deg), P(a["status"]), P(feat),
                                                     P(self.pos_n), P(self.batch_n), P(a["batch_ev"]), P(self.x0buf),
                                                     self.x0_ld, self.x0_feat_col, self.x0_pos_col, stream),
                           "async_graph_append")
                rows = slice(first, first + n)
                self._sample(None, n, self.pos_n[rows], self.batch_n[rows], 0, self._img_feats[0], self.x0buf[rows],
                             self.x0_img_col)
                self._conv_l0_rows(self.l0_conv1, first, n, P(self.x0buf), self.x0_ld, None, 0, P(self.h1), 16)
                self._conv_l0_rows(self.l0_conv2, first, n, P(self.h1), 16, P(self.x0buf), self.x0_ld, P(self.hp0),
                                   self.hp0.shape[1])
                self._sample(None, n, self.pos_n[rows], self.batch_n[rows], 0, self._img_feats[1], self.hp0[rows], 16)
                self._n_rows = first + n
            self._pool1_stream(rebuild=False, first=first, n=n)
        if self.tail_graph and not self.use_image:
            return self._replay_tail(static_out)
        return self._tail_and_head()

    def _conv_generic(self, lvl, pack, x, ldx, xskip, ldskip, out, ldo, dom, stream, code=None, scratch=None):
        L = self.L
        P = _lib.ptr
        code = lvl.code if code is None else code
        scratch = self.A if scratch is None else scratch
        passes = L.dagr_spline_conv_fused_passes(pack.cin, pack.cskip)
        if passes == 1 or (passes > 1 and lvl.T <= FUSED_PASSES_MAX_NODES):
            _lib.check(L.dagr_spline_conv_fused(P(lvl.counts), lvl.T, P(lvl.rowptr), P(lvl.col), P(code), x, ldx,
                                                pack.cin, xskip, ldskip, pack.cskip, dom["rx"], dom["ry"], dom["den_x"],
                                                dom["den_y"], P(pack.Wq), P(pack.bias), out, ldo, pack.N,
                                                1 if pack.relu else 0, stream), "spline_conv_fused")
            return
        lda = (pack.K + 3) // 4 * 4
        _lib.check(L.dagr_spline_tap_aggregate(P(lvl.counts), lvl.T, P(lvl.rowptr), P(lvl.col), P(code),
                                               x, ldx, pack.cin, xskip, ldskip, pack.cskip, dom["rx"], dom["ry"],
                                               dom["den_x"], dom["den_y"], P(scratch), lda, stream), "tap_aggregate")
        _lib.check(L.dagr_gemm_bias_act(P(lvl.counts), lvl.T, P(scratch), lda, P(pack.Wm), pack.ldw, P(pack.bias),
                                        out, ldo, pack.K, pack.N, 1 if pack.relu else 0, stream), "gemm")

    def stage_graph(self, pos, batch, feat=None):
        N = int(pos.shape[0])
        self._alloc_events(N)
        self._N = N
        self._pos, self._batch = pos, batch
        self._nbr = (self.nbr_src[:N], self.nbr_code[:N], self.deg[:N])
        inputs = None
        if feat is not None and pos.dtype == torch.float32:
            self._feat_flat = feat.float().reshape(-1).contiguous()
            inputs = _lib.L0Inputs(feat=self._feat_flat.data_ptr(), pos_nodes=self.pos_n.data_ptr(),
                                   batch_nodes=self.batch_n.data_ptr(), x0=self.x0buf.data_ptr(), ldx0=self.x0_ld,
                                   col_feat=self.x0_feat_col, col_pos=self.x0_pos_col)
        self.graph.build(pos, batch, out=self._nbr, n_dev=self.n_dev if self._dev_mode else None, inputs=inputs)
        self._inputs_gathered = inputs is not None
        self._n_rows = N
        self._async_on = False

    def _nptr(self):
        return self.graph.node_count_ptr() if self._dev_mode else None

    def _sample(self, n_ptr, n_max, pos, batch, b64, fmap, out, coff):
        if self._feat_ready is not None:
            ready = self._feat_ready.get(id(fmap))
            if ready is None:
                raise RuntimeError("pipelined window: a sampled feature map has no ready-event (the image branch did not "
                                   "announce it) -- reading it would race with the image stream")
            torch.cuda.current_stream(self.device).wait_event(ready)
        Bf, C, h, w = fmap.shape
        nhwc = fmap.permute(0, 2, 3, 1)
        if not nhwc.is_contiguous():
            nhwc = nhwc.contiguous()
        self._keep.append(nhwc)
        _lib.check(self.L.dagr_sample_features(n_ptr, n_max, _lib.ptr(pos), _lib.ptr(batch), b64, _lib.ptr(nhwc), Bf, h,
                                               w, C, self.W, self.H, _lib.ptr(out), out.shape[1], coff,
                                               _lib.cur_stream(self.device)), "sample_features")

    def _fold_image_branch(self):
        import copy
        from torch.nn.utils.fusion import fuse_conv_bn_eval
        bb, head = self.model.backbone, self.model.head
        net = copy.deepcopy(bb.net).eval()
        cnn = copy.deepcopy(head.cnn_head).eval()

        def fold_block(blk):
            for ci, bi in (("conv1", "bn1"), ("conv2", "bn2"), ("conv3", "bn3")):
                if hasattr(blk, ci):
                    setattr(blk, ci, fuse_conv_bn_eval(getattr(blk, ci), getattr(blk, bi)))
                    setattr(blk, bi, torch.nn.Identity())
            if blk.downsample is not None:
                blk.downsample = torch.nn.Sequential(fuse_conv_bn_eval(blk.downsample[0], blk.downsample[1]))
        for name in ("layer1", "layer2", "layer3", "layer4"):
            for blk in getattr(net.module, name):
                fold_block(blk)
        for m in cnn.modules():
            if hasattr(m, "conv") and hasattr(m, "bn") and isinstance(m.bn, torch.nn.BatchNorm2d):
                m.conv = fuse_conv_bn_eval(m.conv, m.bn)
                m.bn = torch.nn.Identity()
                if isinstance(getattr(m, "act", None), torch.nn.SiLU) and m.conv.bias is not None:
                    m._bias = m.conv.bias.detach().clone().contiguous()
                    m.conv.bias = None
                    m.forward = types.MethodType(_baseconv_forward, m)
        net = net.to(memory_format=torch.channels_last)
        cnn = cnn.to(memory_format=torch.channels_last)
        for blkname in ("layer1", "layer2", "layer3", "layer4"):
            _gemmify_1x1(getattr(net.module, blkname))
            for blk in getattr(net.module, blkname):
                relu_convs = ("conv1", "conv2") if hasattr(blk, "conv3") else ("conv1",)
                for cname in relu_convs:
                    conv = getattr(blk, cname)
                    if isinstance(conv, _Conv1x1Gemm):
                        conv.relu = True
                    elif isinstance(conv, torch.nn.Conv2d) and conv.bias is not None:
                        setattr(blk, "_" + cname + "_bias", conv.bias.detach().clone().contiguous())
                        conv.bias = None
                blk.forward = types.MethodType(_bottleneck_forward if hasattr(blk, "conv3") else _basicblock_forward,
                                               blk)
        bn = net.module.bn1
        scale = (bn.weight.detach().float() / torch.sqrt(bn.running_var.detach().float() + bn.eps)).contiguous()
        shift = (bn.bias.detach().float() - bn.running_mean.detach().float() * scale).contiguous()
        net.module._stem_affine = (scale, shift)
        net.module.forward_features = types.MethodType(_resnet_features_forward, net.module)
        _gemmify_1x1(net.feature_dconv)
        _gemmify_1x1(net.output_dconv)
        self._net_f, self._cnn_f = net, cnn

    def _image_branch(self, image, on_feature=None):
        if self._net_f is None:
            self._fold_image_branch()
        bb, head = types.SimpleNamespace(net=self._net_f), types.SimpleNamespace(cnn_head=self._cnn_f)
        x = image.contiguous(memory_format=torch.channels_last)
        net = self._net_f
        if on_feature is not None:
            feats = [None] * len(net.feature_layers)

            def emit(name, t):
                if name in net.feature_layers:
                    j = net.feature_layers.index(name)
                    feats[j] = net.feature_dconv[j](t) if len(net.feature_dconv) > 0 else t
                    on_feature(j, feats[j])
            d = _resnet_features_forward(net.module, x, emit)
            outs = [d[l] for l in net.output_layers]
            if len(net.output_dconv) > 0:
                outs = [dconv(o) for o, dconv in zip(outs, net.output_dconv)]
        else:
            feats, outs = bb.net(x)
        outs = outs[-self.num_scales:]
        resized = [torch.nn.functional.interpolate(f, o) for f, o in zip(outs, self.out_sizes)]
        return feats, head.cnn_head(resized)

    def stage_image(self, image):
        self._keep = []
        self._img_feats, self._cnn_out = self._image_branch(image)

    def image_async(self, image, stream=None):
        cur = torch.cuda.current_stream(self.device)
        if stream is not None:
            self._img_stream = stream
        if self._img_stream is None:
            self._img_stream = torch.cuda.Stream(self.device)
        s = self._img_stream
        s.wait_stream(cur)
        with torch.cuda.stream(s):
            feats, cnn_out = self._image_branch(image)
            ev = torch.cuda.Event()
            ev.record(s)
        return feats, cnn_out, ev

    def _consume_image_handle(self, handle):
        feats, cnn_out, ev = handle
        cur = torch.cuda.current_stream(self.device)
        cur.wait_event(ev)
        for t in list(feats) + [o for v in cnn_out.values() for o in v]:
            t.record_stream(cur)
        self._keep = []
        self._img_feats, self._cnn_out = feats, cnn_out

    def stage_l0_input(self, feat):
        N = self._N
        x0 = self.x0buf[:N]
        g = self.graph
        if not self._inputs_gathered:
            f = feat.float().reshape(-1).contiguous()
            _lib.check(self.L.dagr_graph_gather_inputs(ctypes.byref(g.desc), _lib.ptr(g.workspace), _lib.ptr(self._pos),
                                                       _lib.ptr(f), N, _lib.ptr(self.pos_n), _lib.ptr(self.batch_n),
                                                       _lib.ptr(x0), self.x0_ld, self.x0_feat_col, self.x0_pos_col,
                                                       _lib.cur_stream(self.device)), "graph_gather_inputs")
        if self.use_image:
            self._sample(self._nptr(), N, self.pos_n, self.batch_n, 0, self._img_feats[0], x0, self.x0_img_col)
        self._x0 = x0

    def _conv_l0(self, pack, x, ldx, xskip, ldskip, out, ldo):
        L, P = self.L, _lib.ptr
        nbr_src, nbr_code, deg = self._nbr
        cin, cskip, w, s = pack
        d0 = self.dom[0]
        wx, tx, wy, ty = self.win0
        stream = _lib.cur_stream(self.device)
        if self.l0_tiles:
            cm = 16 if cin >= 16 else 0
            _lib.check(L.dagr_spline_conv_l0_tiles(cm, cin - cm, cskip, wx, tx, wy, ty, d0["rx"], d0["ry"], d0["den_x"],
                                                   d0["den_y"], self._N, self.graph.K, P(nbr_src), P(nbr_code), P(deg),
                                                   x, ldx, xskip, ldskip, P(w), P(s), 1, out, ldo, self._nptr(), stream),
                       "conv_l0_tiles")
        else:
            _lib.check(L.dagr_spline_conv_l0(cin, cskip, self.ntaps0, self._N, self.graph.K, self.ncodes0, P(nbr_src),
                                             P(nbr_code), P(deg), x, ldx, xskip, ldskip, P(self.tab0), P(w), P(s), 1,
                                             out, ldo, stream), "conv_l0")

    def stage_l0_conv1(self):
        P = _lib.ptr
        assert self.l0_conv1[0] == len(self.x0_cols)
        self._conv_l0(self.l0_conv1, P(self._x0), self.x0_ld, None, 0, P(self.h1), 16)

    def stage_l0_conv2(self, sample=True):
        P = _lib.ptr
        self._conv_l0(self.l0_conv2, P(self.h1), 16, P(self._x0), self.x0_ld, P(self.hp0), self.hp0.shape[1])
        if self.use_image and sample:
            self._sample(self._nptr(), self._N, self.pos_n, self.batch_n, 0, self._img_feats[1], self.hp0[:self._N], 16)

    def stage_l0_sample1(self):
        self._sample(None, self._N, self.pos_n, self.batch_n, 0, self._img_feats[1], self.hp0[:self._N], 16)

    def stage_pool1(self):
        L, P = self.L, _lib.ptr
        g = self.graph
        nbr_src, nbr_code, deg = self._nbr
        l1 = self.levels[0]
        d = self.pool_desc[0]
        b64 = 1 if self._batch.dtype == torch.int64 else 0
        _lib.check(L.dagr_pool_l0(ctypes.byref(d), P(self.pool_ws[0]), ctypes.byref(g.desc), P(g.workspace),
                                  P(self.xlo), P(self.ylo), P(self.hp0), self.hp0.shape[1], P(self.pos_n),
                                  P(self.batch_n), P(self._batch), b64, self._N, P(nbr_src),
                                  P(nbr_code) if self.fast_coarse_edges else None, P(deg), P(self.cluster0), P(l1.x),
                                  l1.x.shape[1], 0, P(l1.pos), P(l1.batch), P(l1.counts), P(l1.rowptr), P(l1.col),
                                  P(l1.code), ctypes.c_void_p(l1.counts.data_ptr() + 4), l1.e_cap,
                                  _lib.cur_stream(self.device)), "pool_l0")

    def pool1_accumulate_again(self):
        L, P = self.L, _lib.ptr
        g = self.graph
        nbr_src, nbr_code, deg = self._nbr
        _lib.check(L.dagr_pool_l0_accumulate(ctypes.byref(self.pool_desc[0]), P(self.pool_ws[0]), ctypes.byref(g.desc),
                                             P(g.workspace), P(self.xlo), P(self.ylo), P(self.hp0), self.hp0.shape[1],
                                             P(self.pos_n), self._N, P(nbr_src),
                                             P(nbr_code) if self.fast_coarse_edges else None, P(deg),
                                             _lib.cur_stream(self.device)), "pool_l0_accumulate")

    def _stage_level(self, k, trace=None):
        L, P = self.L, _lib.ptr
        stream = _lib.cur_stream(self.device)
        lvl = self.levels[k]
        c1, c2 = self.packs[k]
        dom = self.dom[k + 1]
        ldx = lvl.x.shape[1]
        self._conv_generic(lvl, c1, P(lvl.x), ldx, None, 0, P(lvl.h1), c1.N, dom, stream)
        ldh = lvl.hp.shape[1]
        fuse_pool = (k < 3 and not self.use_image and L.dagr_spline_conv_fused_passes(c2.cin, c2.cskip) == 1
                     and self.pool_desc[k + 1].channels == c2.N)
        self._pool_accumulated[k] = fuse_pool
        if fuse_pool:
            d = self.pool_desc[k + 1]
            _lib.check(L.dagr_spline_conv_fused_pool(P(lvl.counts), lvl.T, P(lvl.rowptr), P(lvl.col), P(lvl.code), P(lvl.h1),
                                                     c1.N, c2.cin, P(lvl.x), ldx, c2.cskip, dom["rx"], dom["ry"],
                                                     dom["den_x"], dom["den_y"], P(c2.Wq), P(c2.bias), P(lvl.hp), ldh, c2.N,
                                                     1 if c2.relu else 0, ctypes.byref(d), P(self.pool_ws[k + 1]), P(lvl.pos),
                                                     P(lvl.batch), P(lvl.cluster), stream), "spline_conv_fused_pool")
        else:
            self._conv_generic(lvl, c2, P(lvl.h1), c1.N, P(lvl.x), ldx, P(lvl.hp), ldh, dom, stream)
        if trace is not None:
            trace[f"pool{k + 1}"] = self._level_snapshot(lvl, lvl.x)
            trace[f"layer{k + 2}"] = self._level_snapshot(lvl, lvl.hp[:, :lvl.cout])

    def _stage_pool(self, k):
        L, P = self.L, _lib.ptr
        stream = _lib.cur_stream(self.device)
        lvl, nxt = self.levels[k], self.levels[k + 1]
        ldh = lvl.hp.shape[1]
        if self.use_image:
            self._sample(P(lvl.counts), lvl.T, lvl.pos, lvl.batch, 0, self._img_feats[k + 2], lvl.hp, lvl.cout)
        d = self.pool_desc[k + 1]
        _lib.check(L.dagr_pool_csr(ctypes.byref(d), P(self.pool_ws[k + 1]), P(lvl.counts),
                                   0 if self._pool_accumulated[k] else lvl.T, P(lvl.hp),
                                   ldh, P(lvl.pos), P(lvl.batch), P(lvl.rowptr), P(lvl.col),
                                   P(lvl.cluster), P(nxt.x), nxt.x.shape[1], 0, P(nxt.pos), P(nxt.batch),
                                   P(nxt.counts), P(nxt.rowptr), P(nxt.col), P(nxt.code),
                                   ctypes.c_void_p(nxt.counts.data_ptr() + 4), nxt.e_cap, stream), "pool_csr")

    def stage_tail(self, trace=None):
        for k in range(4):
            self._stage_level(k, trace)
            if k < 3:
                self._stage_pool(k)

    def _head_recode(self, i):
        code = self.head_code[i]
        if code is None:
            return
        L, P = self.L, _lib.ptr
        lvln = self.head_levels[i]
        lvl = self.levels[lvln - 1]
        dom = self.head_dom[i]
        rm = dom["remap"]
        _lib.check(L.dagr_pool_recode(P(lvl.counts), lvl.T, P(lvl.rowptr), P(lvl.col), P(lvl.pos),
                                      self.pool_desc[lvln - 1].two_max, float(rm[0, 0]), float(rm[0, 2]),
                                      float(rm[1, 1]), float(rm[1, 2]), dom["rx"], dom["ry"], P(code),
                                      lvl.e_cap, ctypes.c_void_p(self.status.data_ptr() + 4), _lib.cur_stream(self.device)),
                   "pool_recode")

    def _conv_job(self, lvl, pack, x, ldx, xskip, ldskip, out, ldo, dom, code=None):
        code = lvl.code if code is None else code
        return _lib.ConvJob(n_nodes_ptr=lvl.counts.data_ptr(), n_nodes_max=lvl.T, rowptr=lvl.rowptr.data_ptr(),
                            col=lvl.col.data_ptr(), code=code.data_ptr(), x=x, ldx=ldx, cin=pack.cin, xskip=xskip,
                            ldskip=ldskip, cskip=pack.cskip, rx=dom["rx"], ry=dom["ry"], den_x=dom["den_x"],
                            den_y=dom["den_y"], Wq=pack.Wq.data_ptr(), bias=pack.bias.data_ptr(), C=out, ldc=ldo, N=pack.N,
                            relu=1 if pack.relu else 0)

    def _build_tail_jobs(self):
        L = self.L
        if not (len(self.head_levels) == 2 and self.head_levels[0] == 3):
            return None
        c1, c2 = self.packs[3]
        packs = [c1, c2] + [p for hp in self.head_packs for p in hp]
        if any(L.dagr_spline_conv_fused_passes(p.cin, p.cskip) != 1 for p in packs):
            return None
        nr = self.n_reg
        lvl4 = self.levels[3]
        dom4 = self.dom[4]
        ldx4, ldh4 = lvl4.x.shape[1], lvl4.hp.shape[1]
        layer5 = [self._conv_job(lvl4, c1, lvl4.x.data_ptr(), ldx4, None, 0, lvl4.h1.data_ptr(), c1.N, dom4),
                  self._conv_job(lvl4, c2, lvl4.h1.data_ptr(), c1.N, lvl4.x.data_ptr(), ldx4, lvl4.hp.data_ptr(), ldh4, dom4)]
        heads = []
        for i in range(2):
            lvl = self.levels[self.head_levels[i] - 1]
            stem, cr, cls, ro = self.head_packs[i]
            hb, dom, code = self.head_buf[i], self.head_dom[i], self.head_code[i]
            pred = hb["pred"]
            npred = pred.shape[1]
            heads.append([
                [self._conv_job(lvl, stem, lvl.hp.data_ptr(), lvl.hp.shape[1], None, 0, hb["stem"].data_ptr(), nr, dom, code)],
                [self._conv_job(lvl, cr, hb["stem"].data_ptr(), nr, None, 0, hb["cr"].data_ptr(), 2 * nr, dom, code)],
                [self._conv_job(lvl, ro, hb["cr"].data_ptr() + 4 * nr, 2 * nr, None, 0, pred.data_ptr(), npred, dom, code),
                 self._conv_job(lvl, cls, hb["cr"].data_ptr(), 2 * nr, None, 0, pred.data_ptr() + 4 * 5, npred, dom, code)]])
        plan = [[layer5[0]] + heads[0][0], [layer5[1]] + heads[0][1], heads[1][0] + heads[0][2], heads[1][1], heads[1][2]]
        return [((_lib.ConvJob * len(jobs))(*jobs), len(jobs)) for jobs in plan]

    def _stage_level5_and_heads(self):
        stream = _lib.cur_stream(self.device)
        self._pool_accumulated[3] = False
        for i in range(2):
            self._head_recode(i)
        for arr, count in self._tail_jobs:
            _lib.check(self.L.dagr_spline_conv_fused_multi(arr, count, stream), "spline_conv_fused_multi")

    def _stage_head_scale(self, i, scratch=None):
        L, P = self.L, _lib.ptr
        stream = _lib.cur_stream(self.device)
        lvln = self.head_levels[i]
        lvl = self.levels[lvln - 1]
        stem, cr, cls, ro = self.head_packs[i]
        hb = self.head_buf[i]
        dom = self.head_dom[i]
        code = self.head_code[i]
        self._head_recode(i)
        nr = self.n_reg
        self._conv_generic(lvl, stem, P(lvl.hp), lvl.hp.shape[1], None, 0, P(hb["stem"]), nr, dom, stream, code, scratch)
        self._conv_generic(lvl, cr, P(hb["stem"]), nr, None, 0, P(hb["cr"]), 2 * nr, dom, stream, code, scratch)
        pred = hb["pred"]
        npred = pred.shape[1]
        x_reg, x_cls = ctypes.c_void_p(hb["cr"].data_ptr() + 4 * nr), P(hb["cr"])
        o_reg, o_cls = P(pred), ctypes.c_void_p(pred.data_ptr() + 4 * 5)
        if L.dagr_spline_conv_fused_passes(ro.cin, 0) >= 1 and \
                (L.dagr_spline_conv_fused_passes(ro.cin, 0) == 1 or lvl.T <= FUSED_PASSES_MAX_NODES):
            kcode = lvl.code if code is None else code
            _lib.check(L.dagr_spline_conv_fused_pair(P(lvl.counts), lvl.T, P(lvl.rowptr), P(lvl.col), P(kcode), 2 * nr, ro.cin,
                                                     dom["rx"], dom["ry"], dom["den_x"], dom["den_y"], npred, 0, x_reg,
                                                     P(ro.Wq), P(ro.bias), o_reg, ro.N, x_cls, P(cls.Wq), P(cls.bias), o_cls,
                                                     cls.N, stream), "spline_conv_fused_pair")
        else:
            self._conv_generic(lvl, ro, x_reg, 2 * nr, None, 0, o_reg, npred, dom, stream, code, scratch)
            self._conv_generic(lvl, cls, x_cls, 2 * nr, None, 0, o_cls, npred, dom, stream, code, scratch)
        return pred

    def _heads_finish(self):
        P = _lib.ptr
        if self._cnn_ready is not None:
            torch.cuda.current_stream(self.device).wait_event(self._cnn_ready)
            self._cnn_ready = None
            self._feat_ready = None
        scales = []
        for i, lvln in enumerate(self.head_levels):
            lvl, hb = self.levels[lvln - 1], self.head_buf[i]
            Hc, Wc = self.out_sizes[i]
            vox = self.head_vox[i]
            hs = _lib.HeadScale(n_ptr=lvl.counts.data_ptr(), n_max=lvl.T, pred=hb["pred"].data_ptr(), ld=hb["pred"].shape[1],
                                pos=lvl.pos.data_ptr(), batch=lvl.batch.data_ptr(), vx=float(vox[0]), vy=float(vox[1]),
                                stride=float(self.strides[i]), Hc=int(Hc), Wc=int(Wc), dense=hb["dense"].data_ptr())
            if self._cnn_out is not None:
                for k, name in enumerate(("reg_output", "obj_output", "cls_output")):
                    t = self._cnn_out[name][i]
                    hs.cnn[k] = t.data_ptr()
                    for j in range(4):
                        hs.cnn_stride[k][j] = int(t.stride(j))
            scales.append(hs)
        A = sum(int(h) * int(w) for h, w in self.out_sizes)
        CH = 5 + self.num_classes
        out = torch.empty((self.B, A, CH), dtype=torch.float32, device=self.device)
        s0, s1 = ctypes.byref(scales[0]), ctypes.byref(scales[1]) if len(scales) > 1 else None
        if self._post_key is not None:
            self._det = torch.empty((self.B, A, 6), dtype=torch.float32, device=self.device)
            self._n_keep = torch.empty((self.B,), dtype=torch.int32, device=self.device)
            conf, nms = self._post_key
            _lib.check(self.L.dagr_heads_finish_detect(s0, s1, self.B, CH, P(out), P(self.status), conf, nms,
                                                       float(max(self.W, self.H) + 1), P(self._det), P(self._n_keep),
                                                       _lib.cur_stream(self.device)), "heads_finish_detect")
            self._post_fresh = True
        else:
            _lib.check(self.L.dagr_heads_finish(s0, s1, self.B, CH, P(out), P(self.status), _lib.cur_stream(self.device)),
                       "heads_finish")
        self._fused_dense = [hb["dense"] for hb in self.head_buf]
        return out

    def stage_head(self):
        for i in range(len(self.head_levels)):
            self._stage_head_scale(i)
        return self._heads_finish()

    def _tail_and_head(self, trace=None):
        first = self.head_levels[0]
        if trace is None:
            if self._tail_jobs is None:
                self._tail_jobs = self._build_tail_jobs() or False
            if self._tail_jobs:
                for k in range(3):
                    self._stage_level(k)
                    self._stage_pool(k)
                self._stage_level5_and_heads()
                return self._heads_finish()
        done = [False] * len(self.head_levels)
        cur = torch.cuda.current_stream(self.device)
        forked = False
        for k in range(4):
            self._stage_level(k, trace)
            if k + 1 == first and first == 3 and trace is None and self.overlap_heads:
                if self._head_stream is None:
                    self._head_stream = torch.cuda.Stream(self.device)
                ev = torch.cuda.Event()
                ev.record(cur)
                self._head_stream.wait_event(ev)
                with torch.cuda.stream(self._head_stream):
                    self._stage_head_scale(0, scratch=self.A2)
                    done[0] = True
                    self._head_join = torch.cuda.Event()
                    self._head_join.record(self._head_stream)
                forked = True
            if k < 3:
                self._stage_pool(k)
        for i in range(len(self.head_levels)):
            if not done[i]:
                self._stage_head_scale(i)
        if forked:
            cur.wait_event(self._head_join)
        return self._heads_finish()

    def _post_launch(self, out):
        if self._post_key is None or self._post_fresh:
            return
        B, A, C = out.shape
        self._det = torch.empty((B, A, 6), dtype=torch.float32, device=self.device)
        self._n_keep = torch.empty((B,), dtype=torch.int32, device=self.device)
        conf, nms = self._post_key
        _lib.check(self.L.dagr_postprocess(_lib.ptr(out), B, A, int(self.num_classes), conf, nms,
                                           float(max(self.W, self.H) + 1), _lib.ptr(self._det), _lib.ptr(self._n_keep),
                                           _lib.cur_stream(self.device)), "postprocess")
        self._post_fresh = True

    def forward_detections(self, pos, feat, batch, image=None, append=False):
        from .model.utils import postprocess_device
        key = (float(self.model.conf_threshold), float(self.model.nms_threshold))
        if key != self._post_key:
            self._post_key = key
            self._wg = None
            self._wg_warm = 0
            self._graph = None
            self._graph_warm = 0
        self._post_fresh = False
        if append:
            out = self.forward_append(pos, feat, batch, static_out=True)
        else:
            out = self.forward_raw(pos, feat, batch, image=image, static_out=True)
        if self._post_fresh:
            return self._det, self._n_keep
        return postprocess_device(out, self.num_classes, key[0], key[1], self.H, self.W)

    def forward_raw(self, pos, feat, batch, image=None, trace=None, image_handle=None, static_out=False):
        if trace is None and image_handle is None and self.window_graph and self.l0_tiles and not self.no_events \
                and (image is not None or not self.use_image):
            return self._forward_window_graph(pos, feat, batch, image, static_out)
        self._cnn_out = None
        if self.use_image:
            if image_handle is not None:
                self._consume_image_handle(image_handle)
            elif image is None:
                raise RuntimeError("model was built with --use_image: an image batch is required")
            else:
                self.stage_image(image)
        if self.no_events:
            c = self._cnn_out
            return self._decode_maps([torch.cat([c["reg_output"][k], c["obj_output"][k], c["cls_output"][k]], 1)
                                      for k in range(self.num_scales)])
        self.stage_graph(pos.contiguous(), batch.contiguous(), feat)
        self.stage_l0_input(feat)
        self.stage_l0_conv1()
        self.stage_l0_conv2()
        if trace is not None:
            trace["nbr"] = tuple(t.clone() for t in self._nbr)
            _, ev_slot = self.graph.node_order(self._N)
            ev_slot = ev_slot.long()
            trace["layer1"] = self.hp0[:self._N, :16][ev_slot].clone()
            if self.use_image:
                back = [self.x0_cols.index(k) for k in range(len(self.x0_cols))]
                trace["x0"] = self._x0[ev_slot][:, back].clone()
        self.stage_pool1()
        if trace is None and self.tail_graph and not self.use_image:
            return self._replay_tail(static_out)
        out = self._tail_and_head(trace)
        if trace is not None:
            trace["head_dense"] = [o.clone() for o in self._fused_dense]
        return out

    def _forward_static(self):
        self._dev_mode = True
        try:
            self._cnn_out = None
            if self.use_image:
                cur = torch.cuda.current_stream(self.device)
                if self._head_stream is None:
                    self._head_stream = torch.cuda.Stream(self.device)
                fork = torch.cuda.Event()
                fork.record(cur)
                self._head_stream.wait_event(fork)
                with torch.cuda.stream(self._head_stream):
                    self.stage_graph(self.in_pos, self.in_batch, self.in_feat)
                    join = torch.cuda.Event()
                    join.record(self._head_stream)
                if self._img_stream is None:
                    self._img_stream = torch.cuda.Stream(self.device)
                s_img = self._img_stream
                s_img.wait_event(fork)
                self._feat_ready = {}
                self._keep = []
                with torch.cuda.stream(s_img):
                    def on_feature(j, fmap):
                        ev = torch.cuda.Event()
                        ev.record(s_img)
                        self._feat_ready[id(fmap)] = ev
                        fmap.record_stream(cur)
                    self._img_feats, self._cnn_out = self._image_branch(self.in_image, on_feature)
                    for v in self._cnn_out.values():
                        for o in v:
                            o.record_stream(cur)
                    self._cnn_ready = torch.cuda.Event()
                    self._cnn_ready.record(s_img)
                cur.wait_event(join)
            else:
                self.stage_graph(self.in_pos, self.in_batch, self.in_feat)
            self.stage_l0_input(self.in_feat)
            self.stage_l0_conv1()
            self.stage_l0_conv2()
            self.stage_pool1()
            out = self._tail_and_head()
            self._post_launch(out)
            return out
        finally:
            self._dev_mode = False

    def _forward_window_graph(self, pos, feat, batch, image, static_out=False):
        L, P = self.L, _lib.ptr
        N = int(pos.shape[0])
        if N > self.max_events:
            self._alloc_events(max(N, 2 * self.max_events))
        pos = pos.float().contiguous()
        feat = feat.float().reshape(-1).contiguous()
        batch = batch.contiguous()
        g = self.graph
        _lib.check(L.dagr_stage_window(ctypes.byref(g.desc), P(g.workspace), P(pos), P(feat), P(batch),
                                       1 if batch.dtype == torch.int64 else 0, N, P(self.in_pos), P(self.in_feat),
                                       P(self.in_batch), P(self.n_dev), _lib.cur_stream(self.device)), "stage_window")
        if self.use_image:
            if self.in_image is None or self.in_image.shape != image.shape:
                self.in_image = torch.empty(tuple(image.shape), dtype=torch.float32, device=self.device)
                self._wg = None
                self._wg_warm = 0
            self.in_image.copy_(image)
        if self._wg is None:
            if self._wg_warm < 2:
                self._wg_warm += 1
                out = self._forward_static()
            else:
                g = torch.cuda.CUDAGraph()
                with _capture(g):
                    out = self._forward_static()
                self._wg, self._wg_out, self._wg_post = g, out, (self._det, self._n_keep)
                g.replay()
        else:
            self._wg.replay()
            out = self._wg_out
            self._det, self._n_keep = self._wg_post
            self._post_fresh = self._post_key is not None
        self._N = N
        self._n_rows = N
        self._async_on = False
        self._pos, self._batch = self.in_pos[:N], self.in_batch[:N]
        self._nbr = (self.nbr_src[:N], self.nbr_code[:N], self.deg[:N])
        self._x0 = self.x0buf[:N]
        return out if static_out else out.clone()

    def _replay_tail(self, static_out=False):
        if self._graph is None:
            if self._graph_warm < 2:
                self._graph_warm += 1
                out = self._tail_and_head()
                self._post_launch(out)
                return out
            g = torch.cuda.CUDAGraph()
            with _capture(g):
                out = self._tail_and_head()
                self._post_launch(out)
            self._graph, self._graph_out, self._graph_post = g, out, (self._det, self._n_keep)
        self._graph.replay()
        self._det, self._n_keep = self._graph_post
        self._post_fresh = self._post_key is not None
        return self._graph_out if static_out else self._graph_out.clone()

    def _decode_maps(self, dense_maps):
        P = _lib.ptr
        d = [m.contiguous() for m in dense_maps]
        self._keep_maps = d
        CH = d[0].shape[1]
        A = sum(m.shape[2] * m.shape[3] for m in d)
        out = torch.empty((self.B, A, CH), dtype=torch.float32, device=self.device)
        second = d[1] if len(d) > 1 else None
        _lib.check(self.L.dagr_decode_heads(P(d[0]), d[0].shape[2], d[0].shape[3], float(self.strides[0]), P(second),
                                            second.shape[2] if second is not None else 0,
                                            second.shape[3] if second is not None else 0,
                                            float(self.strides[1]) if second is not None else 0.0, self.B, CH, P(out),
                                            _lib.cur_stream(self.device)), "decode_heads")
        return out

    def _level_snapshot(self, lvl, x):
        n, e = [int(v) for v in lvl.counts.tolist()]
        return dict(x=x[:n].clone(), pos=lvl.pos[:n].clone(), batch=lvl.batch[:n].clone(),
                    rowptr=lvl.rowptr[:n + 1].clone(), col=lvl.col[:e].clone(), code=lvl.code[:e].clone())

    def l0_kernel_names(self):
        c0 = 3 + self.feat_ch[0]
        nt = self.ntaps0
        if self.l0_tiles:
            tx, ty = self.win0[1], self.win0[3]
            cm = 16 if c0 >= 16 else 0
            return {"l0_conv1": f"k_conv_l0_tiles<{cm}, {c0 - cm}, 0, {tx}, {ty}>",
                    "l0_conv2": f"k_conv_l0_tiles<16, 0, {c0}, {tx}, {ty}>"}
        return {"l0_conv1": f"k_conv_l0<{c0}, 0, {nt}>", "l0_conv2": f"k_conv_l0<16, {c0}, {nt}>"}

    def check_status(self):
        ne, fl = self.graph.status()
        if fl:
            raise RuntimeError(f"graph builder flagged {fl:#x} (events outside the sensor / batch range)")
        for k, (d, ws) in enumerate(zip(self.pool_desc, self.pool_ws)):
            f = ctypes.c_int32(0)
            _lib.check(self.L.dagr_pool_status(ctypes.byref(d), _lib.ptr(ws), ctypes.byref(f),
                                               _lib.cur_stream(self.device)), "pool_status")
            if f.value:
                raise RuntimeError(f"pool{k + 1} flagged {f.value:#x}")
        if self._async_on:
            if int(self._app["status"][0]):
                raise RuntimeError("asynchronous update: event outside the sensor / batch range")
            f = ctypes.c_int32(0)
            _lib.check(self.L.dagr_pool_status(ctypes.byref(self.pool_desc[0]), _lib.ptr(self._app["pool_ws"]),
                                               ctypes.byref(f), _lib.cur_stream(self.device)), "pool_status")
            if f.value:
                raise RuntimeError(f"pool1 (asynchronous accumulators) flagged {f.value:#x}")
        st = self.status.tolist()
        if st[0]:
            raise RuntimeError("to_dense: node outside the output map")
        if st[1]:
            raise RuntimeError("head: LUT coordinate outside the head's table (dagr_pool_recode)")

    def check_batch(self, data):
        ng = getattr(data, "num_graphs", None)
        if ng is not None and int(ng) > self.B:
            raise RuntimeError(f"batch of {int(ng)} windows, but the model was built with batch_size = {self.B}")
        geo = getattr(data, "_geometry", None)
        for k, (name, want) in enumerate((("width", self.W), ("height", self.H), ("time_window", self.time_window))):
            v = geo[k] if geo is not None else getattr(data, name, None)
            if v is not None and not (torch.is_tensor(v) and v.is_cuda):
                v = int(v[0]) if hasattr(v, "__len__") else int(v)
                if v != want:
                    raise RuntimeError(f"data.{name} = {v}, but the model was built for {want}")

    def forward_detections_data(self, data):
        batch = data.batch if getattr(data, "batch", None) is not None else \
            torch.zeros(data.pos.shape[0], dtype=torch.int64, device=data.pos.device)
        self.check_batch(data)
        return self.forward_detections(data.pos.float(), data.x.float(), batch, image=getattr(data, "image", None))

    def forward_data(self, data, static_out=False):
        batch = data.batch if getattr(data, "batch", None) is not None else \
            torch.zeros(data.pos.shape[0], dtype=torch.int64, device=data.pos.device)
        self.check_batch(data)
        return self.forward_raw(data.pos.float(), data.x.float(), batch, image=getattr(data, "image", None),
                                static_out=static_out)
```

include/dagr_hip.h:

```cpp
#ifndef DAGR_HIP_H
#define DAGR_HIP_H

#include <stddef.h>
#include <stdint.h>

#ifdef __cplusplus
extern "C" {
#endif

typedef enum {
    DAGR_OK = 0,
    DAGR_ERR_INVALID_ARG = -1,
    DAGR_ERR_HIP = -2,
    DAGR_ERR_WORKSPACE = -3,
    DAGR_ERR_UNSUPPORTED = -4
} dagr_status;

const char *dagr_last_error(void);
int dagr_version(void);
int dagr_device_count(void);

int dagr_format_events(const int16_t *xy , const int32_t *t , const int8_t *p ,
                       int64_t N, int32_t width, int32_t height, int32_t time_window,
                       float *pos_out , float *feat_out , void *stream);
// ... 6 lines not shown
int dagr_insert_in_queue(const int32_t *indices , const int32_t *unique_coords ,
                         const int32_t *cumsum_counts , int64_t num_pixels, int32_t *queue,
                         int32_t B, int32_t Q, int32_t H, int32_t W, void *stream);
int dagr_insert_in_queue_single(const int32_t *indices , const int32_t *event_xy ,
                                int32_t *queue, int32_t B, int32_t Q, int32_t H, int32_t W, void *stream);

typedef struct {
    int32_t width;
    int32_t height;
    int32_t batch_size;
    int32_t max_neighbors;
    int32_t queue_size;
    int32_t radius;
    int32_t delta_t_us;
    int32_t time_window;
    int64_t max_events;
} dagr_graph_desc;

size_t dagr_graph_workspace_bytes(const dagr_graph_desc *desc);
int dagr_graph_workspace_init(const dagr_graph_desc *desc, void *workspace, size_t workspace_bytes, void *stream);

int dagr_graph_build_window(const dagr_graph_desc *desc, void *workspace,
                            const void *pos, int32_t pos_is_int32,
                            const void *batch, int32_t batch_is_int64, int64_t N,
                            int32_t *nbr_src, int16_t *nbr_code, int32_t *deg, void *stream);

int dagr_graph_build_window_dev(const dagr_graph_desc *desc, void *workspace, const void *pos, int32_t pos_is_int32,
                                const void *batch, int32_t batch_is_int64, int64_t n_cap, const int32_t *n_dev,
                                int32_t *nbr_src, int16_t *nbr_code, int32_t *deg, void *stream);
const int32_t *dagr_graph_node_count_ptr(const dagr_graph_desc *desc, void *workspace);
int dagr_stage_window(const dagr_graph_desc *desc, void *workspace, const float *pos, const float *feat, const void *batch,
                      int32_t batch_is_int64, int64_t N, float *pos_out, float *feat_out, int32_t *batch_out,
                      int32_t *n_dev, void *stream);

int dagr_graph_search_window(const dagr_graph_desc *desc, void *workspace, int64_t N,
                             int32_t *nbr_src, int16_t *nbr_code, int32_t *deg, void *stream);

int dagr_graph_status(const dagr_graph_desc *desc, void *workspace, int64_t *num_edges ,
                      int32_t *flags , void *stream);
int dagr_graph_counters(const dagr_graph_desc *desc, void *workspace, int32_t *out8_host, void *stream);

size_t dagr_scan_scratch_elems(int64_t n);
int dagr_graph_edge_index(const dagr_graph_desc *desc, void *workspace, const int32_t *nbr_src, const int32_t *deg,
                          int64_t N, int32_t *rowptr, int32_t *scan_scratch,
                          int64_t *edge_index, int64_t row_stride, void *stream);
int dagr_graph_csr_codes(const dagr_graph_desc *desc, void *workspace, const int32_t *nbr_src, const int16_t *nbr_code,
                         const int32_t *deg, int64_t N, int32_t code_bias, int32_t *rowptr, int32_t *scan_scratch,
                         int32_t *col, int32_t *code, int64_t e_cap, void *stream);
int dagr_graph_node_order(const dagr_graph_desc *desc, void *workspace, int64_t N, int32_t *slot_event,
                          int32_t *event_slot, void *stream);
int dagr_graph_gather_inputs(const dagr_graph_desc *desc, void *workspace, const float *pos, const float *feat,
                             int64_t N, float *pos_nodes, int32_t *batch_nodes, float *x0, int32_t ldx0,
                             int32_t col_feat, int32_t col_pos, void *stream);

typedef struct dagr_l0_inputs {
    const float *feat;
    float *pos_nodes;
    int32_t *batch_nodes;
    float *x0;
    int32_t ldx0, col_feat, col_pos;
} dagr_l0_inputs;
int dagr_graph_build_window_inputs(const dagr_graph_desc *desc, void *workspace, const float *pos, const void *batch,
                                   int32_t batch_is_int64, int64_t N, const int32_t *n_dev, int32_t *nbr_src,
                                   int16_t *nbr_code, int32_t *deg, const dagr_l0_inputs *inputs, void *stream);

int dagr_spline_tap_window(int32_t r, float den, int32_t *first_tap_host, int32_t *num_taps_host);
int dagr_spline_l0_table(int32_t rx, int32_t ry, float den_x, float den_y, int32_t win_x, int32_t tx,
                         int32_t win_y, int32_t ty, float *tab, int32_t *bad_flag, void *stream);
int dagr_spline_conv_l0(int32_t cin, int32_t cskip, int32_t ntaps ,
                        int64_t N, int32_t K, int32_t ncodes,
                        const int32_t *nbr_src, const int16_t *nbr_code, const int32_t *deg,
                        const float *x, int32_t ldx, const float *xskip, int32_t ldskip,
                        const float *tab, const float *wpack, const float *shift, int32_t relu,
                        float *out, int32_t ldo, void *stream);
int dagr_spline_conv_l0_tiles(int32_t cmain, int32_t cextra, int32_t cskip, int32_t win_x, int32_t tx, int32_t win_y,
                              int32_t ty, int32_t rx, int32_t ry, float den_x, float den_y, int64_t N, int32_t K,
                              const int32_t *nbr_src, const int16_t *nbr_code, const int32_t *deg, const float *x,
                              int32_t ldx, const float *xskip, int32_t ldskip, const float *wpack, const float *shift,
                              int32_t relu, float *out, int32_t ldo, const int32_t *n_ptr, void *stream);
int dagr_spline_conv_l0_tiles_rows(int32_t cmain, int32_t cextra, int32_t cskip, int32_t win_x, int32_t tx, int32_t win_y,
                                   int32_t ty, int32_t rx, int32_t ry, float den_x, float den_y, int64_t first_node,
                                   int64_t N, int32_t K, const int32_t *nbr_src, const int16_t *nbr_code,
                                   const int32_t *deg, const float *x, int32_t ldx, const float *xskip, int32_t ldskip,
                                   const float *wpack, const float *shift, int32_t relu, float *out, int32_t ldo,
                                   const int32_t *n_ptr, void *stream);
int dagr_spline_tap_aggregate(const int32_t *n_nodes_ptr, int32_t n_nodes_max, const int32_t *rowptr,
                              const int32_t *col, const int32_t *code, const float *x, int32_t ldx,
                              int32_t cin, const float *xskip, int32_t ldskip, int32_t cskip,
                              int32_t rx, int32_t ry, float den_x, float den_y,
                              float *A, int32_t lda, void *stream);
int dagr_spline_tap_scatter_grad(const int32_t *n_nodes_ptr, int32_t n_nodes_max, const int32_t *rowptr,
                                 const int32_t *col, const int32_t *code, const float *grad_A, int32_t lda, int32_t cin,
                                 int32_t rx, int32_t ry, float den_x, float den_y, const float *grad_A_absmax,
                                 int64_t *acc, float *grad_x, int32_t ldg, void *stream);
int dagr_spline_tap_scatter_grad_w(const int32_t *n_nodes_ptr, int32_t n_nodes_max, const int32_t *rowptr,
                                   const int32_t *col, const int32_t *code, const float *grad_out, int32_t ldg, int32_t cout,
                                   const float *Wm, int32_t ldw, int32_t cin, int32_t rx, int32_t ry, float den_x,
                                   float den_y, const float *grad_A_bound, int64_t *acc, float *grad_x, int32_t ldgx,
                                   void *stream);
size_t dagr_spline_conv_fused_lds_bytes(int32_t cin, int32_t cskip);
int32_t dagr_spline_conv_fused_passes(int32_t cin, int32_t cskip);
int dagr_spline_conv_fused(const int32_t *n_nodes_ptr, int32_t n_nodes_max, const int32_t *rowptr,
                           const int32_t *col, const int32_t *code, const float *x, int32_t ldx, int32_t cin,
                           const float *xskip, int32_t ldskip, int32_t cskip, int32_t rx, int32_t ry,
                           float den_x, float den_y, const float *Wq, const float *bias, float *C, int32_t ldc,
                           int32_t N, int32_t relu, void *stream);
int dagr_spline_conv_fused_pair(const int32_t *n_nodes_ptr, int32_t n_nodes_max, const int32_t *rowptr,
                                const int32_t *col, const int32_t *code, int32_t ldx, int32_t cin, int32_t rx, int32_t ry,
                                float den_x, float den_y, int32_t ldc, int32_t relu, const float *x_a, const float *Wq_a,
                                const float *bias_a, float *C_a, int32_t N_a, const float *x_b, const float *Wq_b,
                                const float *bias_b, float *C_b, int32_t N_b, void *stream);
typedef struct dagr_conv_job {
    const int32_t *n_nodes_ptr;
    int32_t n_nodes_max;
    const int32_t *rowptr, *col, *code;
    const float *x;
    int32_t ldx, cin;
    const float *xskip;
    int32_t ldskip, cskip, rx, ry;
    float den_x, den_y;
    const float *Wq, *bias;
    float *C;
    int32_t ldc, N, relu;
} dagr_conv_job;
int dagr_spline_conv_fused_multi(const dagr_conv_job *jobs, int32_t count, void *stream);
int dagr_gemm_bias_act(const int32_t *m_ptr, int32_t m_max, const float *A, int32_t lda,
                       const float *Wm, int32_t ldw, const float *bias, float *C, int32_t ldc,
                       int32_t K, int32_t N, int32_t relu, void *stream);

typedef struct {
    int32_t batch_size;
    int32_t channels;
    int32_t gx, gy;
    float vx, vy;
    float inv_w, inv_h;
    float two_max;
    float r00, r02, r11, r12;
    int32_t rx, ry;
    int32_t aggr;
    int32_t append_pos;
    int32_t keep_order;
} dagr_pool_desc;

size_t dagr_pool_workspace_bytes(const dagr_pool_desc *desc);
int dagr_pool_workspace_init(const dagr_pool_desc *desc, void *workspace, size_t workspace_bytes, void *stream);
int dagr_pool_l0(const dagr_pool_desc *desc, void *pool_ws, const dagr_graph_desc *gdesc, void *graph_ws,
                 const int32_t *xlo, const int32_t *ylo, const float *x, int32_t ldx,
                 const float *pos_nodes, const int32_t *batch_nodes ,
                 const void *batch, int32_t batch_is_int64 , int64_t N,
                 const int32_t *nbr_src, const int16_t *nbr_code , const int32_t *deg,
                 int32_t *cluster_scratch , float *x_out, int32_t ldo, int32_t xoff, float *pos_out,
                 int32_t *batch_out, int32_t *n_out, int32_t *rowptr_out, int32_t *col_out, int32_t *code_out,
                 int32_t *e_out, int32_t e_cap, void *stream);
int dagr_async_graph_append(const dagr_graph_desc *desc, void *graph_ws, int64_t n_static, int64_t first_id,
                            int32_t *app_head, int32_t *app_next, int32_t *app_xytb, int64_t capacity,
                            const void *pos , int32_t pos_is_int32,
                            const void *batch, int32_t batch_is_int64, int64_t n_new,
                            int32_t *nbr_src, int16_t *nbr_code, int32_t *deg ,
                            int32_t *status,
                            const float *feat, float *pos_nodes, int32_t *batch_nodes, int32_t *batch_events, float *x0,
                            int32_t ldx0, int32_t col_feat, int32_t col_pos, void *stream);
typedef struct dagr_async_update_args {
    const dagr_graph_desc *gdesc; void *graph_ws; int64_t n_static, first_id;
    int32_t *app_head, *app_next, *app_xytb; int64_t capacity;
    const float *pos; const void *batch; int32_t batch_is_int64; int64_t n_new;
    int32_t *nbr_src; int16_t *nbr_code; int32_t *deg; int32_t *status;
    const float *feat; float *pos_nodes; int32_t *batch_nodes, *batch_events; float *x0; int32_t ldx0, col_feat, col_pos;
    int32_t win_x, tx, win_y, ty, rx, ry; float den_x, den_y;
    int32_t cin1; const float *w1, *s1; float *h1; int32_t ldh1;
    const float *w2, *s2; float *hp0; int32_t ldhp0;
    const dagr_pool_desc *pdesc; void *pool_ws; const int32_t *xlo, *ylo;
    float *x_out; int32_t ldo; float *pos_out; int32_t *batch_out, *n_out, *rowptr_out, *col_out, *code_out, *e_out;
    int32_t e_cap;
} dagr_async_update_args;
int dagr_async_update(const dagr_async_update_args *args, void *stream);
int dagr_pool_l0_accumulate(const dagr_pool_desc *desc, void *pool_ws, const dagr_graph_desc *gdesc, void *graph_ws,
                            const int32_t *xlo, const int32_t *ylo, const float *x, int32_t ldx, const float *pos,
                            int64_t N, const int32_t *nbr_src, const int16_t *nbr_code, const int32_t *deg, void *stream);
int dagr_pool_l0_stream(const dagr_pool_desc *desc, void *pool_ws, int32_t rebuild, const dagr_graph_desc *gdesc,
                        void *graph_ws, const int32_t *xlo, const int32_t *ylo, const float *x, int32_t ldx, const float *pos,
                        const int32_t *batch_events, int64_t n_window, int64_t first_row, int64_t n_rows,
                        const int32_t *nbr_src, const int16_t *nbr_code, const int32_t *deg, float *x_out, int32_t ldo,
                        int32_t xoff, float *pos_out, int32_t *batch_out, int32_t *n_out, int32_t *rowptr_out,
                        int32_t *col_out, int32_t *code_out, int32_t *e_out, int32_t e_cap, void *stream);

int dagr_spline_conv_fused_pool(const int32_t *n_nodes_ptr, int32_t n_nodes_max, const int32_t *rowptr,
                                const int32_t *col, const int32_t *code, const float *x, int32_t ldx, int32_t cin,
                                const float *xskip, int32_t ldskip, int32_t cskip, int32_t rx, int32_t ry,
                                float den_x, float den_y, const float *Wq, const float *bias, float *C,
                                int32_t ldc, int32_t N, int32_t relu, const dagr_pool_desc *pdesc, void *pool_ws,
                                const float *pos, const int32_t *batch, int32_t *cluster_scratch, void *stream);
int dagr_pool_csr(const dagr_pool_desc *desc, void *pool_ws, const int32_t *n_ptr, int32_t n_max, const float *x,
                  int32_t ldx, const float *pos, const int32_t *batch, const int32_t *rowptr, const int32_t *col,
                  int32_t *cluster_scratch , float *x_out, int32_t ldo, int32_t xoff, float *pos_out,
                  int32_t *batch_out, int32_t *n_out, int32_t *rowptr_out, int32_t *col_out, int32_t *code_out,
                  int32_t *e_out, int32_t e_cap, void *stream);
int dagr_pool_recode(const int32_t *n_ptr, int32_t n_max, const int32_t *rowptr, const int32_t *col, const float *pos,
                     float two_max, float r00, float r02, float r11, float r12, int32_t rx, int32_t ry,
                     int32_t *code_out, int32_t e_cap, int32_t *status, void *stream);
int dagr_pool_status(const dagr_pool_desc *desc, void *pool_ws, int32_t *flags_host, void *stream);
const int32_t *dagr_pool_status_ptr(const dagr_pool_desc *desc, void *pool_ws);
int dagr_pool_counters(const dagr_pool_desc *desc, void *pool_ws, int32_t *out8_host, void *stream);

int dagr_to_dense(const int32_t *n_ptr, int32_t n_max, const float *x, int32_t ldx, int32_t channels,
                  const float *pos, const int32_t *batch, float vx, float vy, int32_t batch_size,
                  int32_t Hc, int32_t Wc, int32_t *winner_scratch, float *dense, int32_t *status, void *stream);

int dagr_pool_argmax(const int32_t *cluster, int32_t n, const float *x, int32_t ldx, int32_t channels,
                     const float *x_pooled, int32_t ldp, int32_t n_clusters, int32_t *arg, void *stream);
int dagr_pool_grad(const int32_t *cluster, int32_t n, int32_t channels, int32_t aggr, const int32_t *arg,
                   const int32_t *count, const float *grad_pooled, int32_t ldg, float *grad_x, int32_t ldgx,
                   void *stream);
int dagr_to_dense_grad(int32_t n, int32_t channels, const float *pos, const int32_t *batch, float vx, float vy,
                       int32_t batch_size, int32_t Hc, int32_t Wc, const float *grad_dense,
                       float *grad_x, int32_t ldgx, void *stream);

int dagr_add_relu(float *y, const float *z, int64_t n, void *stream);
int dagr_bias_relu(float *y_nhwc, const float *bias, int64_t n, int32_t C, void *stream);
int dagr_bias_silu(float *y_nhwc, const float *bias, int64_t n, int32_t C, void *stream);
int dagr_bn_relu_maxpool(const float *x_nhwc, int32_t B, int32_t H, int32_t W, int32_t C, const float *scale,
                         const float *shift, float *y_nhwc, void *stream);

int dagr_sample_features(const int32_t *n_ptr, int32_t n_max, const float *pos, const void *batch,
                         int32_t batch_is_int64, const float *feat_nhwc, int32_t B, int32_t h, int32_t w, int32_t C,
                         int32_t width, int32_t height, float *out, int32_t ldo, int32_t coff, void *stream);

int dagr_nms_batched(const float *boxes, const float *scores, const int32_t *cls, const uint8_t *valid,
                     int32_t B, int32_t A, float iou_threshold, float class_offset,
                     int32_t *order_out, int32_t *keep_out, int32_t *n_keep, void *stream);

typedef struct dagr_head_scale {
    const int32_t *n_ptr; int32_t n_max;
    const float *pred; int32_t ld;
    const float *pos; const int32_t *batch;
    float vx, vy, stride; int32_t Hc, Wc;
    const float *cnn[3]; int32_t cnn_stride[3][4];
    float *dense;
} dagr_head_scale;
int dagr_heads_finish(const dagr_head_scale *scale0, const dagr_head_scale *scale1, int32_t batch_size, int32_t channels,
                      float *out, int32_t *status, void *stream);
int dagr_heads_finish_detect(const dagr_head_scale *scale0, const dagr_head_scale *scale1, int32_t batch_size,
                             int32_t channels, float *out, int32_t *status, float conf_threshold, float iou_threshold,
                             float class_offset, float *det, int32_t *n_keep, void *stream);
int dagr_decode_heads(const float *dense0, int32_t H0, int32_t W0, float stride0, const float *dense1, int32_t H1,
                      int32_t W1, float stride1, int32_t B, int32_t channels, float *out, void *stream);

int dagr_postprocess(const float *pred, int32_t B, int32_t A, int32_t num_classes, float conf_threshold,
                     float iou_threshold, float class_offset, float *det, int32_t *n_keep, void *stream);

int dagr_masked_lin(const int64_t *indices, const float *x_in, float *x_out, const float *weight, const float *bias,
                    int32_t add, int64_t K, int32_t Cin, int32_t Cout, void *stream);
int dagr_masked_lin_no_bias(const int64_t *indices, const float *x_in, float *x_out, const float *weight, int32_t add,
                            int64_t K, int32_t Cin, int32_t Cout, void *stream);
int dagr_masked_isdiff(int64_t *indices, const float *x_old, const float *x_new, float atol, float rtol, int64_t K,
                       int32_t C, void *stream);
int dagr_masked_inplace_BN(const int64_t *indices, const float *x, float *x_out, const float *running_mean,
                           const float *running_var, const float *weight, const float *bias, float eps, int64_t K,
                           int32_t C, void *stream);

int dagr_downsample_events(const int32_t *order, const int32_t *run_cell, const int32_t *run_end, int32_t n_runs,
                           const int8_t *polarity, int32_t fx, int32_t fy, float *change_map, uint8_t *keep,
                           void *stream);

size_t dagr_gemm_epilogue_workspace_bytes(void);
int dagr_gemm_epilogue(const float *A, int64_t M, int32_t K, int64_t lda, const float *Wt, int32_t N, const float *bias,
                       const float *R, int64_t ldr, int32_t act, float *D, int64_t ldd, void *workspace,
                       size_t workspace_bytes, void *stream);

enum { DAGR_FLOPS_ZERO = 0, DAGR_FLOPS_CONV = 1, DAGR_FLOPS_LINEAR = 2, DAGR_FLOPS_POOL = 3, DAGR_FLOPS_CARTESIAN = 4 };
typedef struct dagr_flops_module {
    int32_t kind, level, cin, cout, root, bias;
} dagr_flops_module;
int dagr_async_flops(const int32_t *deg, int32_t n_events, const int32_t *counts1, const int32_t *counts2,
                     const int32_t *counts3, const int32_t *counts4, const dagr_flops_module *mods, int32_t n_mods,
                     int64_t *out, void *stream);

size_t dagr_viz_workspace_bytes(int32_t F, int32_t H, int32_t W);
int dagr_viz_render(const uint8_t *images, int32_t n_images, int32_t H, int32_t W, const int32_t *frame_image, int32_t F,
                    const int32_t *ev_x, const int32_t *ev_y, const int8_t *ev_p, const int32_t *ev_ptr, int32_t n_events,
                    const double *alpha, const int32_t *boxes, const int32_t *box_ptr, int32_t n_boxes, int32_t linewidth,
                    const uint8_t *colors, int32_t n_colors, uint8_t *out, int32_t *status, void *workspace,
                    size_t workspace_bytes, void *stream);

typedef struct dagr_aug_params {
    int32_t flip, crop_on;
    int32_t crop_lo[2], crop_hi[2];
    float zoom;
    int32_t move[2];
} dagr_aug_params;
size_t dagr_augment_workspace_bytes(int64_t N);
int dagr_augment_events(const dagr_aug_params *params, int32_t B, int32_t W, int32_t H, const void *pos, int32_t pos_width,
                        const void *t, int32_t t_width, const void *p, int32_t p_width, const int32_t *sample_ptr, int64_t N,
                        int16_t *out_pos, void *out_t, void *out_p, int64_t *out_batch, int32_t *out_ptr,
                        int32_t *status, void *workspace, size_t workspace_bytes, void *stream);
int dagr_augment_status(const int32_t *status, void *stream);
int dagr_augment_frames(const dagr_aug_params *params, int32_t B, int32_t C, int32_t H, int32_t W, int32_t elem_bytes,
                        int32_t reference_crop, const void *in, void *out, void *stream);
int dagr_augment_boxes(const dagr_aug_params *params, int32_t B, int32_t W, int32_t H, const float *boxes,
                       const int64_t *box_batch, int32_t M, int32_t ld, float *out, void *stream);

int dagr_spiral_offsets(int32_t n, int32_t *dx_host, int32_t *dy_host);

#ifdef __cplusplus
}
#endif
#endif
```

Measured before the change: 148.3 million events/s.

## Fuse image-feature sampling into level-0 pooling kernel instead of writing hp0

Result: slower. 146.8 million events/s (-1.1%).

```diff
diff --git a/dagr_amd/_lib.py b/dagr_amd/_lib.py
--- a/dagr_amd/_lib.py
+++ b/dagr_amd/_lib.py
@@ -124,6 +124,16 @@
     "dagr_pool_l0_accumulate": (ctypes.c_int, [ctypes.POINTER(PoolDesc), c_void_p, ctypes.POINTER(GraphDesc), c_void_p,
                                                c_void_p, c_void_p, c_void_p, c_i32, c_void_p, c_i64, c_void_p, c_void_p,
                                                c_void_p, c_void_p]),
+    "dagr_pool_l0_sampled": (ctypes.c_int, [ctypes.POINTER(PoolDesc), c_void_p, ctypes.POINTER(GraphDesc), c_void_p,
+                                            c_void_p, c_void_p, c_void_p, c_i32, c_void_p, c_void_p, c_void_p, c_i32, c_i64,
+                                            c_void_p, c_void_p,
+                                            c_void_p, c_void_p, c_void_p, c_i32, c_i32, c_void_p, c_void_p, c_void_p,
+                                            c_void_p, c_void_p, c_void_p, c_void_p, c_i32,
+                                            c_void_p, c_i32, c_i32, c_i32, c_i32, c_i32, c_void_p]),
+    "dagr_pool_l0_accumulate_sampled": (ctypes.c_int, [ctypes.POINTER(PoolDesc), c_void_p, ctypes.POINTER(GraphDesc),
+                                                       c_void_p, c_void_p, c_void_p, c_void_p, c_i32, c_void_p, c_void_p,
+                                                       c_i64, c_void_p, c_void_p, c_void_p,
+                                                       c_void_p, c_i32, c_i32, c_i32, c_i32, c_i32, c_void_p]),
     "dagr_pool_csr": (ctypes.c_int, [ctypes.POINTER(PoolDesc), c_void_p, c_void_p, c_i32, c_void_p, c_i32, c_void_p,
                                      c_void_p, c_void_p, c_void_p, c_void_p, c_void_p, c_i32, c_i32, c_void_p,
                                      c_void_p, c_void_p, c_void_p, c_void_p, c_void_p, c_void_p, c_i32, c_void_p]),
diff --git a/dagr_amd/csrc/pooling.hip b/dagr_amd/csrc/pooling.hip
--- a/dagr_amd/csrc/pooling.hip
+++ b/dagr_amd/csrc/pooling.hip
@@ -2,6 +2,7 @@
 
 #include "common.hpp"
 #include "pool_common.hpp"
+#include "sample_common.hpp"
 
 namespace dagr {
 namespace {
@@ -52,6 +53,13 @@
 
 constexpr int kPoolL0Block = 1024;
 
+struct L0Sample {
+    const float *feat;
+    const int32_t *batch;
+    SampleGeom g;
+    int coff, Cf;
+};
+
 template <int AGGR>
 __host__ __device__ inline size_t pool_l0_lds_bytes(int VW, int C, int W, int H, bool ord = false) {
     size_t b = ((size_t)VW * C * (AGGR == 0 ? 4 : 8) + 7) / 8 * 8;
@@ -62,7 +70,7 @@
     return b + 64;
 }
 
-template <int AGGR, int VEC, bool ORD>
+template <int AGGR, int VEC, bool ORD, bool SAMP>
 __device__ __forceinline__ void pool_l0_slots_body(dagr_pool_desc d, int W, int H, int n_cap, int VW,
                                                                const int32_t *__restrict__ n_ptr,
                                                                const int32_t *__restrict__ xlo,
@@ -74,7 +82,9 @@
                                                                const float *__restrict__ pos, PoolWs ws,
                                                                const int16_t *__restrict__ nbr_code,
                                                                const int32_t *__restrict__ nbr_src,
-                                                               const int32_t *__restrict__ deg, int K, int r) {
+                                                               const int32_t *__restrict__ deg, int K, int r,
+                                                               const L0Sample &sm) {
+    static_assert(!SAMP || VEC == 4, "sampled columns are merged as 16-byte pieces");
     extern __shared__ __align__(16) unsigned char lds_raw[];
     constexpr int NW = kPoolL0Block / 64;
     const int n = min(*n_ptr, n_cap);
@@ -142,11 +152,12 @@
     for (int cs = seg_begin + 64 * wv; cs < seg_end; cs += 64 * NW) {
         const int s = cs + lane;
         const bool live = s < seg_end;
-        int c = 0, id = 0, dg = 0;
+        int c = 0, id = 0, dg = 0, sb = 0;
         float px = 0.f, py = 0.f, pt = 0.f;
         int4 lo4 = make_int4(0, 0, 0, 0), hi4 = lo4;
         if (live) {
             c = slot_xyb[s];
+            if constexpr (SAMP) sb = sm.batch[s];
             px = pos[3 * (size_t)s]; py = pos[3 * (size_t)s + 1]; pt = pos[3 * (size_t)s + 2];
             id = slot_it[s].x;
             if (nbr_code) {
@@ -179,7 +190,43 @@
                 }
             }
         };
-        request(0);
+        SampleCoord sc{0.f, 0.f, 0.f};
+        if constexpr (SAMP) sc = sample_coord(px, py, (float)sb, sm.g);
+        struct Piece {
+            int who;
+            unsigned on;
+            int colp;
+            SampleCoord sk;
+            float f[4][4];
+        };
+        auto piece_begin = [&](int f, Piece &pc) {
+            const bool act = f < n_live * PPN;
+            const int fc = act ? f : 0;
+            const int k = PPN > 1 ? (int)__umulhi((unsigned)fc, ppn_magic) : fc, p = fc - k * PPN;
+            pc.sk.ix = __shfl(sc.ix, k, 64); pc.sk.iy = __shfl(sc.iy, k, 64); pc.sk.iz = __shfl(sc.iz, k, 64);
+            const int colp = 4 * p - sm.coff;
+            const bool smp = act && colp >= 0 && colp < sm.Cf;
+            pc.colp = smp ? colp : 0;
+            pc.who = act ? (k << 16) | p : -1;
+            pc.on = sample_plane_load<4, true>(pc.sk, sm.feat, sm.g, pc.colp, 0, smp, pc.f,
+                                               xrow + (size_t)k * ldx + (smp ? 0 : 4 * p)) | (smp ? 16u : 0u);
+        };
+        auto piece_end = [&](const Piece &pc, int u) {
+            who[u] = pc.who;
+            if (pc.on & 16u) {
+                float a[4] = {0.f, 0.f, 0.f, 0.f};
+                sample_plane_sum<4>(pc.sk, 0, pc.on & 15u, pc.f, a);
+                float f1[4][4];
+                const unsigned on1 = sample_plane_load<4, true>(pc.sk, sm.feat, sm.g, pc.colp, 1, true, f1);
+                sample_plane_sum<4>(pc.sk, 1, on1, f1, a);
+#pragma unroll
+                for (int j = 0; j < 4; j++) val[u][j % VEC] = a[j];
+            } else {
+#pragma unroll
+                for (int j = 0; j < 4; j++) val[u][j % VEC] = pc.f[0][j];
+            }
+        };
+        if constexpr (!SAMP) request(0);
         int vloc = -1;
         if (live) {
             const int xp = c & 4095, yp = (c >> 12) & 4095, b = (c >> 24) & 127;
@@ -244,13 +291,28 @@
             } else {
                 const int rl = leak ? raw + cells : raw;
                 n_slow++;
-                for (int ch = 0; ch < C; ch++) {
-                    const float v = x[(size_t)s * ldx + ch];
+                auto merge_global = [&](int ch, float v) {
                     if (AGGR == 0)
                         atomicMax(reinterpret_cast<int *>(ws.xacc + (size_t)rl * C + ch), enc_f(v));
                     else
                         atomicAdd(reinterpret_cast<unsigned long long *>(ws.xacc + (size_t)rl * C + ch),
                                   (unsigned long long)(long long)llrint((double)v * kFeatScale));
+                };
+                if constexpr (SAMP) {
+                    for (int p = 0; p < PPN; p++) {
+                        const int colp = 4 * p - sm.coff;
+                        float v4[4];
+                        if (colp >= 0 && colp < sm.Cf) {
+                            sample_at<4, true>(sc, sm.feat, sm.g, colp, v4);
+                        } else {
+                            const float4 q = *reinterpret_cast<const float4 *>(x + (size_t)s * ldx + 4 * p);
+                            v4[0] = q.x; v4[1] = q.y; v4[2] = q.z; v4[3] = q.w;
+                        }
+#pragma unroll
+                        for (int j = 0; j < 4; j++) merge_global(4 * p + j, v4[j]);
+                    }
+                } else {
+                    for (int ch = 0; ch < C; ch++) merge_global(ch, x[(size_t)s * ldx + ch]);
                 }
                 ws.occupied[rl] = 1;
                 atomicAdd(&w_cnt[rl], 1);
@@ -267,32 +329,55 @@
         }
         l_sv[wv * 64 + lane] = (short)vloc;
         __builtin_amdgcn_wave_barrier();
+        if constexpr (SAMP) {
+#pragma unroll
+            for (int u = 0; u < U; u++) {
+                Piece pc;
+                piece_begin(64 * u + lane, pc);
+                piece_end(pc, u);
+            }
+        }
+        auto merge_piece = [&](int tgt, const float (&v)[VEC]) {
+            if (tgt >= 0) {
+#pragma unroll
+                for (int j = 0; j < VEC; j++) {
+                    if (AGGR == 0)
+                        atomicMax(&l_acc[tgt + j], enc_f(v[j]));
+                    else
+                        atomicAdd(reinterpret_cast<unsigned long long *>(l_acc) + tgt + j,
+                                  (unsigned long long)(long long)llrint((double)v[j] * kFeatScale));
+                }
+            }
+        };
+        auto target = [&](int wh) {
+            if (wh >= 0) {
+                const int v = l_sv[wv * 64 + (wh >> 16)];
+                if (v >= 0) return v * C + (wh & 0xffff) * VEC;
+            }
+            return -1;
+        };
         for (int f0 = 0; f0 < n_live * PPN; f0 += 64 * U) {
-            float cur[U][VEC];
-            int tgt[U];
-#pragma unroll
-            for (int u = 0; u < U; u++) {
-                tgt[u] = -1;
-                if (who[u] >= 0) {
-                    const int v = l_sv[wv * 64 + (who[u] >> 16)];
-                    if (v >= 0) tgt[u] = v * C + (who[u] & 0xffff) * VEC;
+            const bool more = f0 + 64 * U < n_live * PPN;
+            if constexpr (SAMP) {
+#pragma unroll
+                for (int u = 0; u < U; u++) {
+                    Piece pc;
+                    if (more) piece_begin(f0 + 64 * U + 64 * u + lane, pc);
+                    merge_piece(target(who[u]), val[u]);
+                    if (more) piece_end(pc, u);
                 }
-#pragma unroll
-                for (int j = 0; j < VEC; j++) cur[u][j] = val[u][j];
-            }
-            if (f0 + 64 * U < n_live * PPN) request(f0 + 64 * U);
-#pragma unroll
-            for (int u = 0; u < U; u++) {
-                if (tgt[u] >= 0) {
-#pragma unroll
-                    for (int j = 0; j < VEC; j++) {
-                        if (AGGR == 0)
-                            atomicMax(&l_acc[tgt[u] + j], enc_f(cur[u][j]));
-                        else
-                            atomicAdd(reinterpret_cast<unsigned long long *>(l_acc) + tgt[u] + j,
-                                      (unsigned long long)(long long)llrint((double)cur[u][j] * kFeatScale));
-                    }
+            } else {
+                float cur[U][VEC];
+                int tgt[U];
+#pragma unroll
+                for (int u = 0; u < U; u++) {
+                    tgt[u] = target(who[u]);
+#pragma unroll
+                    for (int j = 0; j < VEC; j++) cur[u][j] = val[u][j];
                 }
+                if (more) request(f0 + 64 * U);
+#pragma unroll
+                for (int u = 0; u < U; u++) merge_piece(tgt[u], cur[u]);
             }
         }
         __builtin_amdgcn_wave_barrier();
@@ -344,12 +429,26 @@
         const int2 *__restrict__ slot_it, const int32_t *__restrict__ slot_xyb, const float *__restrict__ x, int ldx,   \
         const float *__restrict__ pos, PoolWs ws, const int16_t *__restrict__ nbr_code,                                \
         const int32_t *__restrict__ nbr_src, const int32_t *__restrict__ deg, int K, int r) {                          \
-        pool_l0_slots_body<AGGR, VEC, ORD>(d, W, H, n_cap, VW, n_ptr, xlo, ylo, start, row_keys, slot_it, slot_xyb, x, \
-                                           ldx, pos, ws, nbr_code, nbr_src, deg, K, r);                                \
+        pool_l0_slots_body<AGGR, VEC, ORD, false>(d, W, H, n_cap, VW, n_ptr, xlo, ylo, start, row_keys, slot_it,       \
+                                                  slot_xyb, x, ldx, pos, ws, nbr_code, nbr_src, deg, K, r, L0Sample{}); \
     }
 DAGR_POOL_L0_SLOTS_KERNEL(k_pool_l0_slots, false)
 DAGR_POOL_L0_SLOTS_KERNEL(k_pool_l0_slots_ord, true)
 #undef DAGR_POOL_L0_SLOTS_KERNEL
+#define DAGR_POOL_L0_SAMPLED_KERNEL(NAME, ORD)                                                                        \
+    template <int AGGR>                                                                                                \
+    __global__ __launch_bounds__(kPoolL0Block) void NAME(                                                              \
+        dagr_pool_desc d, int W, int H, int n_cap, int VW, const int32_t *__restrict__ n_ptr,                          \
+        const int32_t *__restrict__ xlo, const int32_t *__restrict__ ylo, const int32_t *__restrict__ start, int row_keys, \
+        const int2 *__restrict__ slot_it, const int32_t *__restrict__ slot_xyb, const float *__restrict__ x, int ldx,   \
+        const float *__restrict__ pos, PoolWs ws, const int16_t *__restrict__ nbr_code,                                \
+        const int32_t *__restrict__ nbr_src, const int32_t *__restrict__ deg, int K, int r, L0Sample sm) {             \
+        pool_l0_slots_body<AGGR, 4, ORD, true>(d, W, H, n_cap, VW, n_ptr, xlo, ylo, start, row_keys, slot_it, slot_xyb, x, \
+                                               ldx, pos, ws, nbr_code, nbr_src, deg, K, r, sm);                        \
+    }
+DAGR_POOL_L0_SAMPLED_KERNEL(k_pool_l0_slots_sampled, false)
+DAGR_POOL_L0_SAMPLED_KERNEL(k_pool_l0_slots_sampled_ord, true)
+#undef DAGR_POOL_L0_SAMPLED_KERNEL
 
 __global__ __launch_bounds__(kBlock) void k_pool_l0_event_cluster(dagr_pool_desc d, int N,
                                                                  const float *__restrict__ pos,
@@ -878,7 +977,7 @@
 int launch_pool_l0_slots(const dagr_pool_desc *desc, const dagr_graph_desc *gdesc, void *graph_ws, const int32_t *xlo,
                          const int32_t *ylo, const float *x, int ldx, const float *pos, const PoolWs &ws,
                          const int16_t *nbr_code, const int32_t *nbr_src, const int32_t *deg, int64_t n_cap,
-                         hipStream_t stream) {
+                         hipStream_t stream, const L0Sample *sm = nullptr) {
     PixelIndex ix;
     graph_ws_index(gdesc, graph_ws, &ix);
     const int32_t *start = ix.start; const int2 *slot_it = ix.slot_it;
@@ -887,6 +986,14 @@
     const int row_keys = ix.W;
     const int C = desc->channels, W = gdesc->width, H = gdesc->height, K = gdesc->max_neighbors;
     const bool vec4 = C % 4 == 0 && ldx % 4 == 0 && ((uintptr_t)x & 15) == 0;
+    if (sm) {
+        DAGR_CHECK_ARG(sm->feat && sm->batch && sm->g.B >= 1 && sm->g.h >= 1 && sm->g.w >= 1 && W > 1 && H > 1,
+                       "sampled level-0 pooling: bad feature map");
+        DAGR_CHECK_ARG(vec4 && sm->Cf > 0 && sm->Cf % 4 == 0 && sm->g.C == sm->Cf && sm->coff >= 0 && sm->coff % 4 == 0 &&
+                           sm->coff + sm->Cf <= C && ((uintptr_t)sm->feat & 15) == 0,
+                       "sampled level-0 pooling: rows, map channels and column offset must be multiples of 4 floats, 16-byte "
+                       "aligned, and the sampled columns inside the pooled row");
+    }
     const bool ord = desc->keep_order != 0;
     const size_t per_slot = (size_t)C * (desc->aggr == 0 ? 4 : 8) + 36 + (ord ? 4 : 0);
     const size_t budget = (size_t)60 * 1024 - (size_t)(W + H) * 2 - 2048 - 1024;
@@ -898,15 +1005,23 @@
     const int gmult = C > 32 ? 2 : 1;
     const unsigned grid = (unsigned)std::max<int64_t>(1, std::min<int64_t>((int64_t)gmult * device_cu_count(),
                                                                           ceil_div(n_cap, kPoolL0Block)));
+#define DAGR_POOL_L0_LAUNCH_SAMPLED(KERNEL, AG)                                                                        \
+    KERNEL<AG><<<grid, kPoolL0Block, lds, stream>>>(*desc, W, H, (int)n_cap, VW, n_ptr, xlo, ylo, start, row_keys, slot_it, \
+                                                    slot_xyb, x, ldx, pos, ws, nbr_code, nbr_src, deg, K, gdesc->radius, *sm)
 #define DAGR_POOL_L0_LAUNCH(AG, VEC)                                                                                  \
     if (ord) DAGR_POOL_L0_LAUNCH_ORD(k_pool_l0_slots_ord, AG, VEC); else DAGR_POOL_L0_LAUNCH_ORD(k_pool_l0_slots, AG, VEC)
 #define DAGR_POOL_L0_LAUNCH_ORD(KERNEL, AG, VEC)                                                                      \
     KERNEL<AG, VEC><<<grid, kPoolL0Block, lds, stream>>>(*desc, W, H, (int)n_cap, VW, n_ptr, xlo, ylo, start, row_keys, slot_it, \
                                                                    slot_xyb, x, ldx, pos, ws, nbr_code, nbr_src, deg, K, \
                                                                    gdesc->radius)
-    if (desc->aggr == 0) { if (vec4) DAGR_POOL_L0_LAUNCH(0, 4); else DAGR_POOL_L0_LAUNCH(0, 1); }
-    else                 { if (vec4) DAGR_POOL_L0_LAUNCH(1, 4); else DAGR_POOL_L0_LAUNCH(1, 1); }
+    if (sm) {
+        if (desc->aggr == 0) { if (ord) DAGR_POOL_L0_LAUNCH_SAMPLED(k_pool_l0_slots_sampled_ord, 0); else DAGR_POOL_L0_LAUNCH_SAMPLED(k_pool_l0_slots_sampled, 0); }
+        else                 { if (ord) DAGR_POOL_L0_LAUNCH_SAMPLED(k_pool_l0_slots_sampled_ord, 1); else DAGR_POOL_L0_LAUNCH_SAMPLED(k_pool_l0_slots_sampled, 1); }
+    }
+    else if (desc->aggr == 0) { if (vec4) DAGR_POOL_L0_LAUNCH(0, 4); else DAGR_POOL_L0_LAUNCH(0, 1); }
+    else                      { if (vec4) DAGR_POOL_L0_LAUNCH(1, 4); else DAGR_POOL_L0_LAUNCH(1, 1); }
 #undef DAGR_POOL_L0_LAUNCH
+#undef DAGR_POOL_L0_LAUNCH_SAMPLED
 #undef DAGR_POOL_L0_LAUNCH_ORD
     DAGR_CHECK_LAUNCH();
     return DAGR_OK;
@@ -989,13 +1104,13 @@
     return DAGR_OK;
 }
 
-int dagr_pool_l0(const dagr_pool_desc *desc, void *pool_ws, const dagr_graph_desc *gdesc, void *graph_ws,
-                 const int32_t *xlo, const int32_t *ylo, const float *x, int32_t ldx, const float *pos,
-                 const int32_t *batch_nodes, const void *batch, int32_t batch_is_int64, int64_t N,
-                 const int32_t *nbr_src, const int16_t *nbr_code, const int32_t *deg,
-                 int32_t *cluster_scratch, float *x_out, int32_t ldo, int32_t xoff, float *pos_out,
-                 int32_t *batch_out, int32_t *n_out, int32_t *rowptr_out, int32_t *col_out, int32_t *code_out,
-                 int32_t *e_out, int32_t e_cap, void *stream_) {
+static int pool_l0_impl(const dagr_pool_desc *desc, void *pool_ws, const dagr_graph_desc *gdesc, void *graph_ws,
+                        const int32_t *xlo, const int32_t *ylo, const float *x, int32_t ldx, const float *pos,
+                        const int32_t *batch_nodes, const void *batch, int32_t batch_is_int64, int64_t N,
+                        const int32_t *nbr_src, const int16_t *nbr_code, const int32_t *deg,
+                        int32_t *cluster_scratch, float *x_out, int32_t ldo, int32_t xoff, float *pos_out,
+                        int32_t *batch_out, int32_t *n_out, int32_t *rowptr_out, int32_t *col_out, int32_t *code_out,
+                        int32_t *e_out, int32_t e_cap, const L0Sample *sm, void *stream_) {
     int rc = validate_pool(desc);
     if (rc != DAGR_OK) return rc;
     DAGR_CHECK_ARG(pool_ws && gdesc && graph_ws, "NULL workspace/desc");
@@ -1015,7 +1130,7 @@
     if (N > 0) {
         DAGR_CHECK_ARG(xlo && ylo && x && pos && batch_nodes && batch && nbr_src && deg && cluster_scratch, "NULL input");
         rc = launch_pool_l0_slots(desc, gdesc, graph_ws, xlo, ylo, x, ldx, pos, ws, fast_edges ? nbr_code : nullptr, nbr_src,
-                                  deg, N, stream);
+                                  deg, N, stream, sm);
         if (rc != DAGR_OK) return rc;
     }
     if (fast_edges) {
@@ -1047,10 +1162,37 @@
                      e_out, e_cap, stream);
 }
 
-int dagr_pool_l0_accumulate(const dagr_pool_desc *desc, void *pool_ws, const dagr_graph_desc *gdesc, void *graph_ws,
-                            const int32_t *xlo, const int32_t *ylo, const float *x, int32_t ldx, const float *pos,
-                            int64_t N, const int32_t *nbr_src, const int16_t *nbr_code, const int32_t *deg,
-                            void *stream_) {
+int dagr_pool_l0(const dagr_pool_desc *desc, void *pool_ws, const dagr_graph_desc *gdesc, void *graph_ws,
+                 const int32_t *xlo, const int32_t *ylo, const float *x, int32_t ldx, const float *pos,
+                 const int32_t *batch_nodes, const void *batch, int32_t batch_is_int64, int64_t N,
+                 const int32_t *nbr_src, const int16_t *nbr_code, const int32_t *deg,
+                 int32_t *cluster_scratch, float *x_out, int32_t ldo, int32_t xoff, float *pos_out,
+                 int32_t *batch_out, int32_t *n_out, int32_t *rowptr_out, int32_t *col_out, int32_t *code_out,
+                 int32_t *e_out, int32_t e_cap, void *stream_) {
+    return pool_l0_impl(desc, pool_ws, gdesc, graph_ws, xlo, ylo, x, ldx, pos, batch_nodes, batch, batch_is_int64, N, nbr_src,
+                        nbr_code, deg, cluster_scratch, x_out, ldo, xoff, pos_out, batch_out, n_out, rowptr_out, col_out,
+                        code_out, e_out, e_cap, nullptr, stream_);
+}
+
+int dagr_pool_l0_sampled(const dagr_pool_desc *desc, void *pool_ws, const dagr_graph_desc *gdesc, void *graph_ws,
+                         const int32_t *xlo, const int32_t *ylo, const float *x, int32_t ldx, const float *pos,
+                         const int32_t *batch_nodes, const void *batch, int32_t batch_is_int64, int64_t N,
+                         const int32_t *nbr_src, const int16_t *nbr_code, const int32_t *deg,
+                         int32_t *cluster_scratch, float *x_out, int32_t ldo, int32_t xoff, float *pos_out,
+                         int32_t *batch_out, int32_t *n_out, int32_t *rowptr_out, int32_t *col_out, int32_t *code_out,
+                         int32_t *e_out, int32_t e_cap, const float *feat_nhwc, int32_t fB, int32_t fh, int32_t fw,
+                         int32_t Cf, int32_t coff, void *stream_) {
+    DAGR_CHECK_ARG(gdesc && fB >= 1 && fh >= 1 && fw >= 1 && Cf >= 1, "bad feature map");
+    const L0Sample sm{feat_nhwc, batch_nodes, sample_geom(fB, fh, fw, Cf, gdesc->width, gdesc->height), coff, Cf};
+    return pool_l0_impl(desc, pool_ws, gdesc, graph_ws, xlo, ylo, x, ldx, pos, batch_nodes, batch, batch_is_int64, N, nbr_src,
+                        nbr_code, deg, cluster_scratch, x_out, ldo, xoff, pos_out, batch_out, n_out, rowptr_out, col_out,
+                        code_out, e_out, e_cap, &sm, stream_);
+}
+
+static int pool_l0_accumulate_impl(const dagr_pool_desc *desc, void *pool_ws, const dagr_graph_desc *gdesc, void *graph_ws,
+                                   const int32_t *xlo, const int32_t *ylo, const float *x, int32_t ldx, const float *pos,
+                                   int64_t N, const int32_t *nbr_src, const int16_t *nbr_code, const int32_t *deg,
+                                   const L0Sample *sm, void *stream_) {
     int rc = validate_pool(desc);
     if (rc != DAGR_OK) return rc;
     DAGR_CHECK_ARG(pool_ws && gdesc && graph_ws && xlo && ylo && x && pos && nbr_src && deg && N > 0, "bad arguments");
@@ -1062,7 +1204,26 @@
     const bool fast_edges = nbr_code != nullptr && K <= 16 && gdesc->radius <= 2 * std::min(cell_w, cell_h) &&
                             gdesc->width <= 4096;
     return launch_pool_l0_slots(desc, gdesc, graph_ws, xlo, ylo, x, ldx, pos, ws, fast_edges ? nbr_code : nullptr, nbr_src,
-                                deg, N, (hipStream_t)stream_);
+                                deg, N, (hipStream_t)stream_, sm);
+}
+
+int dagr_pool_l0_accumulate(const dagr_pool_desc *desc, void *pool_ws, const dagr_graph_desc *gdesc, void *graph_ws,
+                            const int32_t *xlo, const int32_t *ylo, const float *x, int32_t ldx, const float *pos,
+                            int64_t N, const int32_t *nbr_src, const int16_t *nbr_code, const int32_t *deg,
+                            void *stream_) {
+    return pool_l0_accumulate_impl(desc, pool_ws, gdesc, graph_ws, xlo, ylo, x, ldx, pos, N, nbr_src, nbr_code, deg, nullptr,
+                                   stream_);
+}
+
+int dagr_pool_l0_accumulate_sampled(const dagr_pool_desc *desc, void *pool_ws, const dagr_graph_desc *gdesc, void *graph_ws,
+                                    const int32_t *xlo, const int32_t *ylo, const float *x, int32_t ldx, const float *pos,
+                                    const int32_t *batch_nodes, int64_t N, const int32_t *nbr_src, const int16_t *nbr_code,
+                                    const int32_t *deg, const float *feat_nhwc, int32_t fB, int32_t fh, int32_t fw,
+                                    int32_t Cf, int32_t coff, void *stream_) {
+    DAGR_CHECK_ARG(gdesc && fB >= 1 && fh >= 1 && fw >= 1 && Cf >= 1, "bad feature map");
+    const L0Sample sm{feat_nhwc, batch_nodes, sample_geom(fB, fh, fw, Cf, gdesc->width, gdesc->height), coff, Cf};
+    return pool_l0_accumulate_impl(desc, pool_ws, gdesc, graph_ws, xlo, ylo, x, ldx, pos, N, nbr_src, nbr_code, deg, &sm,
+                                   stream_);
 }
 
 int dagr_pool_l0_stream(const dagr_pool_desc *desc, void *pool_ws, int32_t rebuild, const dagr_graph_desc *gdesc,
diff --git a/dagr_amd/csrc/sample.hip b/dagr_amd/csrc/sample.hip
--- a/dagr_amd/csrc/sample.hip
+++ b/dagr_amd/csrc/sample.hip
@@ -1,4 +1,5 @@
 #include "common.hpp"
+#include "sample_common.hpp"
 
 namespace dagr {
 namespace {
@@ -7,51 +8,15 @@
 __global__ __launch_bounds__(kBlock) void k_sample_features(const int32_t *__restrict__ n_ptr, int n_max,
                                                            const float *__restrict__ pos,
                                                            const BatchT *__restrict__ batch,
-                                                           const float *__restrict__ feat, int B, int h, int w,
-                                                           int C, float fW, float fH, float fWm1, float fHm1,
-                                                           float fBm1, float *__restrict__ out, int ldo, int coff) {
+                                                           const float *__restrict__ feat, SampleGeom g,
+                                                           float *__restrict__ out, int ldo, int coff) {
     const int n_nodes = n_ptr ? min(*n_ptr, n_max) : n_max;
-    const int CV = C / V;
+    const int CV = g.C / V;
     const int64_t gid = (int64_t)blockIdx.x * kBlock + threadIdx.x;
     const int n = (int)(gid / CV), c = (int)(gid % CV) * V;
     if (n >= n_nodes) return;
-    float gx = pos[3 * (size_t)n] * fW;
-    float gy = pos[3 * (size_t)n + 1] * fH;
-    float gb = (float)batch[n];
-    gx = (2.0f * gx) / fWm1 - 1.0f;
-    gy = (2.0f * gy) / fHm1 - 1.0f;
-    gb = (2.0f * gb) / fBm1 - 1.0f;
-    const float ix = ((gx + 1.0f) / 2.0f) * (float)(w - 1);
-    const float iy = ((gy + 1.0f) / 2.0f) * (float)(h - 1);
-    const float iz = ((gb + 1.0f) / 2.0f) * (float)(B - 1);
-    const float x0f = floorf(ix), y0f = floorf(iy), z0f = floorf(iz);
-    const int x0 = (int)x0f, y0 = (int)y0f, z0 = (int)z0f;
-    const int x1 = x0 + 1, y1 = y0 + 1, z1 = z0 + 1;
-    const float wx0 = (x0f + 1.0f) - ix, wx1 = ix - x0f;
-    const float wy0 = (y0f + 1.0f) - iy, wy1 = iy - y0f;
-    const float wz0 = (z0f + 1.0f) - iz, wz1 = iz - z0f;
     float acc[V];
-#pragma unroll
-    for (int v = 0; v < V; v++) acc[v] = 0.0f;
-    auto tap = [&](int z, int y, int x, float wgt) {
-        if (wgt == 0.0f || z < 0 || z >= B || y < 0 || y >= h || x < 0 || x >= w) return;
-        const float *src = feat + (((size_t)z * h + y) * w + x) * C + c;
-        if (V == 4 && ALIGNED) {
-            const float4 f = *reinterpret_cast<const float4 *>(src);
-            acc[0] += f.x * wgt; acc[1 % V] += f.y * wgt; acc[2 % V] += f.z * wgt; acc[3 % V] += f.w * wgt;
-        } else {
-#pragma unroll
-            for (int v = 0; v < V; v++) acc[v] += src[v] * wgt;
-        }
-    };
-    tap(z0, y0, x0, (wx0 * wy0) * wz0);
-    tap(z0, y0, x1, (wx1 * wy0) * wz0);
-    tap(z0, y1, x0, (wx0 * wy1) * wz0);
-    tap(z0, y1, x1, (wx1 * wy1) * wz0);
-    tap(z1, y0, x0, (wx0 * wy0) * wz1);
-    tap(z1, y0, x1, (wx1 * wy0) * wz1);
-    tap(z1, y1, x0, (wx0 * wy1) * wz1);
-    tap(z1, y1, x1, (wx1 * wy1) * wz1);
+    sample_node<V, ALIGNED>(pos[3 * (size_t)n], pos[3 * (size_t)n + 1], (float)batch[n], feat, g, c, acc);
     float *dst = out + (size_t)n * ldo + coff + c;
     if (V == 4 && ALIGNED) {
         *reinterpret_cast<float4 *>(dst) = make_float4(acc[0], acc[1 % V], acc[2 % V], acc[3 % V]);
@@ -74,14 +39,13 @@
     if (n_max == 0) return DAGR_OK;
     DAGR_CHECK_ARG(pos && batch && feat_nhwc && out, "NULL pointer");
     hipStream_t stream = (hipStream_t)stream_;
-    const float fBm1 = (float)((B > 1 ? B : 2) - 1);
+    const SampleGeom g = sample_geom(B, h, w, C, width, height);
     const bool four = (C % 4 == 0) && ((uintptr_t)feat_nhwc % 16 == 0);
     const bool aligned = four && (ldo % 4 == 0) && (coff % 4 == 0) && ((uintptr_t)out % 16 == 0);
     const unsigned grid = (unsigned)ceil_div((int64_t)n_max * (four ? C / 4 : C), kBlock);
 #define DAGR_SAMPLE(BT, V, A)                                                                                           \
-    k_sample_features<BT, V, A><<<grid, kBlock, 0, stream>>>(n_ptr, n_max, pos, (const BT *)batch, feat_nhwc, B, h, w, C, \
-                                                             (float)width, (float)height, (float)(width - 1),          \
-                                                             (float)(height - 1), fBm1, out, ldo, coff)
+    k_sample_features<BT, V, A><<<grid, kBlock, 0, stream>>>(n_ptr, n_max, pos, (const BT *)batch, feat_nhwc, g, out, ldo, \
+                                                             coff)
 #define DAGR_SAMPLE_BT(BT)                                 \
     do {                                                   \
         if (aligned) DAGR_SAMPLE(BT, 4, true);             \
diff --git a/dagr_amd/csrc/sample_common.hpp b/dagr_amd/csrc/sample_common.hpp
--- /dev/null
+++ b/dagr_amd/csrc/sample_common.hpp
@@ -0,0 +1,122 @@
+#pragma once
+#include "common.hpp"
+
+namespace dagr {
+namespace {
+
+struct SampleGeom {
+    int B, h, w, C;
+    float fW, fH, fWm1, fHm1, fBm1;
+};
+
+inline SampleGeom sample_geom(int B, int h, int w, int C, int width, int height) {
+    SampleGeom g;
+    g.B = B; g.h = h; g.w = w; g.C = C;
+    g.fW = (float)width; g.fH = (float)height;
+    g.fWm1 = (float)(width - 1); g.fHm1 = (float)(height - 1);
+    g.fBm1 = (float)((B > 1 ? B : 2) - 1);
+    return g;
+}
+
+struct SampleCoord {
+    float ix, iy, iz;
+};
+
+__device__ __forceinline__ SampleCoord sample_coord(float px, float py, float fb, const SampleGeom &g) {
+    float gx = px * g.fW;
+    float gy = py * g.fH;
+    float gb = fb;
+    gx = (2.0f * gx) / g.fWm1 - 1.0f;
+    gy = (2.0f * gy) / g.fHm1 - 1.0f;
+    gb = (2.0f * gb) / g.fBm1 - 1.0f;
+    SampleCoord sc;
+    sc.ix = ((gx + 1.0f) / 2.0f) * (float)(g.w - 1);
+    sc.iy = ((gy + 1.0f) / 2.0f) * (float)(g.h - 1);
+    sc.iz = ((gb + 1.0f) / 2.0f) * (float)(g.B - 1);
+    return sc;
+}
+
+struct SampleCell {
+    int x0, y0, z0;
+    float wx[2], wy[2], wz[2];
+};
+__device__ __forceinline__ SampleCell sample_cell(const SampleCoord &sc) {
+    const float x0f = floorf(sc.ix), y0f = floorf(sc.iy), z0f = floorf(sc.iz);
+    SampleCell q;
+    q.x0 = (int)x0f; q.y0 = (int)y0f; q.z0 = (int)z0f;
+    q.wx[0] = (x0f + 1.0f) - sc.ix; q.wx[1] = sc.ix - x0f;
+    q.wy[0] = (y0f + 1.0f) - sc.iy; q.wy[1] = sc.iy - y0f;
+    q.wz[0] = (z0f + 1.0f) - sc.iz; q.wz[1] = sc.iz - z0f;
+    return q;
+}
+__device__ __forceinline__ float sample_tap_weight(const SampleCell &q, int half, int k) {
+    return (q.wx[k & 1] * q.wy[k >> 1]) * q.wz[half];
+}
+
+template <int V, bool ALIGNED>
+__device__ __forceinline__ unsigned sample_plane_load(const SampleCoord &sc, const float *__restrict__ feat,
+                                                      const SampleGeom &g, int c, int half, bool enable,
+                                                      float (&f)[4][V], const float *other = nullptr) {
+    const SampleCell q = sample_cell(sc);
+    const int z = q.z0 + half;
+    unsigned on = 0u;
+    const float *src[4];
+#pragma unroll
+    for (int k = 0; k < 4; k++) {
+        const int x = q.x0 + (k & 1), y = q.y0 + (k >> 1);
+        const float wgt = sample_tap_weight(q, half, k);
+        const bool hit = enable && !(wgt == 0.0f || z < 0 || z >= g.B || y < 0 || y >= g.h || x < 0 || x >= g.w);
+        if (hit) on |= 1u << k;
+        src[k] = feat + (hit ? (((size_t)z * g.h + y) * g.w + x) * g.C + c : (size_t)c);
+    }
+    if (other && !enable) src[0] = other;
+    if (on || (other && !enable)) {
+#pragma unroll
+        for (int k = 0; k < 4; k++) {
+            if (V == 4 && ALIGNED) {
+                const float4 t = *reinterpret_cast<const float4 *>(src[k]);
+                f[k][0] = t.x; f[k][1 % V] = t.y; f[k][2 % V] = t.z; f[k][3 % V] = t.w;
+            } else {
+#pragma unroll
+                for (int v = 0; v < V; v++) f[k][v] = src[k][v];
+            }
+        }
+    }
+    return on;
+}
+
+template <int V>
+__device__ __forceinline__ void sample_plane_sum(const SampleCoord &sc, int half, unsigned on, const float (&f)[4][V],
+                                                 float (&acc)[V]) {
+    const SampleCell q = sample_cell(sc);
+#pragma unroll
+    for (int k = 0; k < 4; k++) {
+        if (on & (1u << k)) {
+            const float wgt = sample_tap_weight(q, half, k);
+#pragma unroll
+            for (int v = 0; v < V; v++) acc[v] = __fadd_rn(acc[v], __fmul_rn(f[k][v], wgt));
+        }
+    }
+}
+
+template <int V, bool ALIGNED>
+__device__ __forceinline__ void sample_at(const SampleCoord &sc, const float *__restrict__ feat, const SampleGeom &g, int c,
+                                          float (&acc)[V]) {
+#pragma unroll
+    for (int v = 0; v < V; v++) acc[v] = 0.0f;
+#pragma unroll
+    for (int half = 0; half < 2; half++) {
+        float f[4][V];
+        const unsigned on = sample_plane_load<V, ALIGNED>(sc, feat, g, c, half, true, f);
+        sample_plane_sum<V>(sc, half, on, f, acc);
+    }
+}
+
+template <int V, bool ALIGNED>
+__device__ __forceinline__ void sample_node(float px, float py, float fb, const float *__restrict__ feat,
+                                            const SampleGeom &g, int c, float (&acc)[V]) {
+    sample_at<V, ALIGNED>(sample_coord(px, py, fb, g), feat, g, c, acc);
+}
+
+}
+}
diff --git a/dagr_amd/engine.py b/dagr_amd/engine.py
--- a/dagr_amd/engine.py
+++ b/dagr_amd/engine.py
@@ -313,6 +313,7 @@
         self._app = None
         self._n_rows = 0
         self._N = 0
+        self._hp0_sampled = False
         self._prepare(bb, head)
         self.max_events = 0
         self._alloc_events(int(max_events))
@@ -540,6 +541,8 @@
         a["batch_ev"][:n0] = self._batch.to(torch.int32)
         self._n_rows = n0
         self._async_on = True
+        if self.use_image and not self._hp0_sampled:
+            self.stage_l0_sample1()
         self._pool1_stream(rebuild=True, first=n0, n=0)
 
     def _pool1_stream(self, rebuild, first, n):
@@ -673,18 +676,22 @@
     def _nptr(self):
         return self.graph.node_count_ptr() if self._dev_mode else None
 
-    def _sample(self, n_ptr, n_max, pos, batch, b64, fmap, out, coff):
+    def _feat_nhwc(self, fmap):
         if self._feat_ready is not None:
             ready = self._feat_ready.get(id(fmap))
             if ready is None:
                 raise RuntimeError("pipelined window: a sampled feature map has no ready-event (the image branch did not "
                                    "announce it) -- reading it would race with the image stream")
             torch.cuda.current_stream(self.device).wait_event(ready)
-        Bf, C, h, w = fmap.shape
         nhwc = fmap.permute(0, 2, 3, 1)
         if not nhwc.is_contiguous():
             nhwc = nhwc.contiguous()
         self._keep.append(nhwc)
+        return nhwc
+
+    def _sample(self, n_ptr, n_max, pos, batch, b64, fmap, out, coff):
+        nhwc = self._feat_nhwc(fmap)
+        Bf, h, w, C = nhwc.shape
         _lib.check(self.L.dagr_sample_features(n_ptr, n_max, _lib.ptr(pos), _lib.ptr(batch), b64, _lib.ptr(nhwc), Bf, h,
                                                w, C, self.W, self.H, _lib.ptr(out), out.shape[1], coff,
                                                _lib.cur_stream(self.device)), "sample_features")
@@ -829,26 +836,41 @@
     def stage_l0_conv2(self, sample=True):
         P = _lib.ptr
         self._conv_l0(self.l0_conv2, P(self.h1), 16, P(self._x0), self.x0_ld, P(self.hp0), self.hp0.shape[1])
+        self._hp0_sampled = False
         if self.use_image and sample:
+            self._hp0_sampled = True
             self._sample(self._nptr(), self._N, self.pos_n, self.batch_n, 0, self._img_feats[1], self.hp0[:self._N], 16)
 
     def stage_l0_sample1(self):
         self._sample(None, self._N, self.pos_n, self.batch_n, 0, self._img_feats[1], self.hp0[:self._N], 16)
-
-    def stage_pool1(self):
+        self._hp0_sampled = True
+
+    def _fuse_l0_sampling(self):
+        if not self.use_image:
+            return False
+        Cf = int(self._img_feats[1].shape[1])
+        return Cf % 4 == 0 and self.hp0.shape[1] % 4 == 0 and self.pool_desc[0].channels == 16 + Cf
+
+    def stage_pool1(self, sampled=False):
         L, P = self.L, _lib.ptr
         g = self.graph
         nbr_src, nbr_code, deg = self._nbr
         l1 = self.levels[0]
         d = self.pool_desc[0]
         b64 = 1 if self._batch.dtype == torch.int64 else 0
-        _lib.check(L.dagr_pool_l0(ctypes.byref(d), P(self.pool_ws[0]), ctypes.byref(g.desc), P(g.workspace),
-                                  P(self.xlo), P(self.ylo), P(self.hp0), self.hp0.shape[1], P(self.pos_n),
-                                  P(self.batch_n), P(self._batch), b64, self._N, P(nbr_src),
-                                  P(nbr_code) if self.fast_coarse_edges else None, P(deg), P(self.cluster0), P(l1.x),
-                                  l1.x.shape[1], 0, P(l1.pos), P(l1.batch), P(l1.counts), P(l1.rowptr), P(l1.col),
-                                  P(l1.code), ctypes.c_void_p(l1.counts.data_ptr() + 4), l1.e_cap,
-                                  _lib.cur_stream(self.device)), "pool_l0")
+        args = (ctypes.byref(d), P(self.pool_ws[0]), ctypes.byref(g.desc), P(g.workspace),
+                P(self.xlo), P(self.ylo), P(self.hp0), self.hp0.shape[1], P(self.pos_n),
+                P(self.batch_n), P(self._batch), b64, self._N, P(nbr_src),
+                P(nbr_code) if self.fast_coarse_edges else None, P(deg), P(self.cluster0), P(l1.x),
+                l1.x.shape[1], 0, P(l1.pos), P(l1.batch), P(l1.counts), P(l1.rowptr), P(l1.col),
+                P(l1.code), ctypes.c_void_p(l1.counts.data_ptr() + 4), l1.e_cap)
+        if sampled:
+            nhwc = self._feat_nhwc(self._img_feats[1])
+            Bf, h, w, Cf = nhwc.shape
+            _lib.check(L.dagr_pool_l0_sampled(*args, P(nhwc), Bf, h, w, Cf, 16, _lib.cur_stream(self.device)),
+                       "pool_l0_sampled")
+        else:
+            _lib.check(L.dagr_pool_l0(*args, _lib.cur_stream(self.device)), "pool_l0")
 
     def pool1_accumulate_again(self):
         L, P = self.L, _lib.ptr
@@ -1125,7 +1147,8 @@
         self.stage_graph(pos.contiguous(), batch.contiguous(), feat)
         self.stage_l0_input(feat)
         self.stage_l0_conv1()
-        self.stage_l0_conv2()
+        fuse0 = trace is None and self._fuse_l0_sampling()
+        self.stage_l0_conv2(sample=not fuse0)
         if trace is not None:
             trace["nbr"] = tuple(t.clone() for t in self._nbr)
             _, ev_slot = self.graph.node_order(self._N)
@@ -1134,7 +1157,7 @@
             if self.use_image:
                 back = [self.x0_cols.index(k) for k in range(len(self.x0_cols))]
                 trace["x0"] = self._x0[ev_slot][:, back].clone()
-        self.stage_pool1()
+        self.stage_pool1(sampled=fuse0)
         if trace is None and self.tail_graph and not self.use_image:
             return self._replay_tail(static_out)
         out = self._tail_and_head(trace)
@@ -1180,8 +1203,9 @@
                 self.stage_graph(self.in_pos, self.in_batch, self.in_feat)
             self.stage_l0_input(self.in_feat)
             self.stage_l0_conv1()
-            self.stage_l0_conv2()
-            self.stage_pool1()
+            fuse0 = self._fuse_l0_sampling()
+            self.stage_l0_conv2(sample=not fuse0)
+            self.stage_pool1(sampled=fuse0)
             out = self._tail_and_head()
             self._post_launch(out)
             return out
diff --git a/include/dagr_hip.h b/include/dagr_hip.h
--- a/include/dagr_hip.h
+++ b/include/dagr_hip.h
@@ -182,6 +182,15 @@
                  int32_t *cluster_scratch , float *x_out, int32_t ldo, int32_t xoff, float *pos_out,
                  int32_t *batch_out, int32_t *n_out, int32_t *rowptr_out, int32_t *col_out, int32_t *code_out,
                  int32_t *e_out, int32_t e_cap, void *stream);
+int dagr_pool_l0_sampled(const dagr_pool_desc *desc, void *pool_ws, const dagr_graph_desc *gdesc, void *graph_ws,
+                         const int32_t *xlo, const int32_t *ylo, const float *x, int32_t ldx,
+                         const float *pos_nodes, const int32_t *batch_nodes ,
+                         const void *batch, int32_t batch_is_int64 , int64_t N,
+                         const int32_t *nbr_src, const int16_t *nbr_code , const int32_t *deg,
+                         int32_t *cluster_scratch , float *x_out, int32_t ldo, int32_t xoff, float *pos_out,
+                         int32_t *batch_out, int32_t *n_out, int32_t *rowptr_out, int32_t *col_out, int32_t *code_out,
+                         int32_t *e_out, int32_t e_cap, const float *feat_nhwc, int32_t fB, int32_t fh, int32_t fw,
+                         int32_t Cf, int32_t coff, void *stream);
 int dagr_async_graph_append(const dagr_graph_desc *desc, void *graph_ws, int64_t n_static, int64_t first_id,
                             int32_t *app_head, int32_t *app_next, int32_t *app_xytb, int64_t capacity,
                             const void *pos , int32_t pos_is_int32,
@@ -207,6 +216,11 @@
 int dagr_pool_l0_accumulate(const dagr_pool_desc *desc, void *pool_ws, const dagr_graph_desc *gdesc, void *graph_ws,
                             const int32_t *xlo, const int32_t *ylo, const float *x, int32_t ldx, const float *pos,
                             int64_t N, const int32_t *nbr_src, const int16_t *nbr_code, const int32_t *deg, void *stream);
+int dagr_pool_l0_accumulate_sampled(const dagr_pool_desc *desc, void *pool_ws, const dagr_graph_desc *gdesc, void *graph_ws,
+                                    const int32_t *xlo, const int32_t *ylo, const float *x, int32_t ldx, const float *pos,
+                                    const int32_t *batch_nodes, int64_t N, const int32_t *nbr_src, const int16_t *nbr_code,
+                                    const int32_t *deg, const float *feat_nhwc, int32_t fB, int32_t fh, int32_t fw,
+                                    int32_t Cf, int32_t coff, void *stream);
 int dagr_pool_l0_stream(const dagr_pool_desc *desc, void *pool_ws, int32_t rebuild, const dagr_graph_desc *gdesc,
                         void *graph_ws, const int32_t *xlo, const int32_t *ylo, const float *x, int32_t ldx, const float *pos,
                         const int32_t *batch_events, int64_t n_window, int64_t first_row, int64_t n_rows,
```
